# jhauret/vibravox

Hardware: AMD Instinct MI355X
Metric: EBEN train-step audio-seconds/sec (gen+disc) (higher is better)
Workload: dtype bf16

## Files before the change

### include/eben_hip.h

```cpp
#ifndef EBEN_HIP_H
#define EBEN_HIP_H

#include <stddef.h>
#include <stdint.h>

#if defined(EBEN_BUILDING)
#define EBEN_API __attribute__((visibility("default")))
#else
#define EBEN_API
#endif

#ifdef __cplusplus
extern "C" {
#endif

#define EBEN_OK 0
#define EBEN_EINVAL (-1)
#define EBEN_EWORKSPACE (-2)
#define EBEN_EUNSUPPORTED (-3)

#define EBEN_PAD_ZERO 0
#define EBEN_PAD_REFLECT 1

#define EBEN_MATH_F32 0
#define EBEN_MATH_BF16 1
#define EBEN_MATH_BF16X2 2
#define EBEN_MATH_BF16X3 3
#define EBEN_MATH_BF16X6 4
#define EBEN_LAYOUT_BL 0x100

typedef struct EbenConv1dDesc {
  int32_t batch;
  int32_t c_in, c_out;
  int32_t l_in, l_out;
  int32_t ksize, stride, dilation, groups;
  int32_t pad_l, pad_r;
  int32_t pad_mode;
  int32_t transposed;
  float in_slope;
  float out_slope;
  int32_t math;
} EbenConv1dDesc;

EBEN_API const char* eben_last_error(void);
#define EBEN_ABI_VERSION 5
EBEN_API int eben_version(void);
EBEN_API int eben_device_info(char* name, size_t name_bytes);

EBEN_API int eben_wn_scale(const float* g, const float* v, int rows, int cols, float* scale, float* norm, void* stream);
EBEN_API int eben_wn_bwd(const float* dw_slabs, int nslab, size_t slab_stride, int rows, int cols, int row_stride,
                const float* g, const float* v, const float* norm, float* dg, float* dv, float* dbias, void* stream);

typedef struct EbenWnScaleItem {
  const float* g; const float* v; float* scale; float* norm;
  int32_t rows, cols;
} EbenWnScaleItem;
typedef struct EbenWnBwdItem {
  const float* slabs;
  const float* g; const float* v; const float* norm;
  float* dg; float* dv; float* dbias;
  int64_t slab_stride;
  int32_t nslab, rows, cols, row_stride;
  int32_t col_perm_k, pad_;
} EbenWnBwdItem;
EBEN_API int eben_wn_scale_multi(const EbenWnScaleItem* items, int n, void* stream);
EBEN_API int eben_wn_bwd_multi(const EbenWnBwdItem* items, int n, void* stream);

EBEN_API size_t eben_conv1d_packed_floats(const EbenConv1dDesc* d, int which);
typedef struct EbenPackJob {
  EbenConv1dDesc desc;
  const float* v; const float* scale;
  float* wp_fwd; float* wp_bwd;
} EbenPackJob;
EBEN_API int eben_conv1d_pack_multi(const EbenPackJob* jobs, int n, void* stream);
EBEN_API int eben_conv1d_kernel_generation(const EbenConv1dDesc* d, int which);
#define EBEN_VARIANT_TAP3 1
#define EBEN_VARIANT_THIN_BL 2
#define EBEN_VARIANT_TAP4 3
EBEN_API int eben_conv1d_variant(const EbenConv1dDesc* d, int which, int mask_on_load, int* out, int n);
EBEN_API int eben_conv1d_pack(const EbenConv1dDesc* d, const float* v, const float* scale, float* wp_fwd, float* wp_bwd, void* stream);
EBEN_API int eben_conv1d_fwd(const EbenConv1dDesc* d, const float* x, const float* wp_fwd, const float* bias,
                    const float* residual, float* y, void* stream);
EBEN_API int eben_conv1d_fwd_res(const EbenConv1dDesc* d, const float* x, const float* wp_fwd, const float* bias,
                        const float* residual, float res_slope, float* y, void* stream);
EBEN_API size_t eben_conv1d_bwd_dx_workspace(const EbenConv1dDesc* d);
EBEN_API size_t eben_conv1d_bwd_dw_workspace(const EbenConv1dDesc* d, int* nslab, int* row_stride);
EBEN_API int eben_conv1d_bwd_dx(const EbenConv1dDesc* d, const float* dy, const float* y, const float* wp_bwd,
                       const float* x, float* dx, int accumulate, void* workspace, size_t ws_bytes, void* stream);
EBEN_API int eben_conv1d_bwd_dx_res(const EbenConv1dDesc* d, const float* dy, const float* y, const float* wp_bwd, const float* x,
                           const float* res_pre, const float* res_post, float* dx, void* workspace, size_t ws_bytes, void* stream);
EBEN_API int eben_conv1d_bwd_dx_ex(const EbenConv1dDesc* d, const float* g, const float* wp_bwd, const float* res, int res_rows,
                          const float* mask, float mask_slope, int seg, const int* seg_map, float* dx, void* stream);
EBEN_API int eben_conv1d_bwd_dx_fm(const EbenConv1dDesc* d, const float* g, const float* wp_bwd, const float* ref, int fm_rows,
                          const float* fm_sums, float fm_gs, const float* mask, float mask_slope, int seg, const int* seg_map,
                          float* dx, void* stream);
EBEN_API int eben_conv1d_bwd_dw(const EbenConv1dDesc* d, const float* dy, const float* y, const float* x, int has_bias,
                       float* slabs, size_t ws_bytes, void* stream);

EBEN_API int eben_bl_from_f32(const float* x, int batch, int channels, int length, void* hi, void* lo , void* stream);
EBEN_API int eben_bl_to_f32(const void* hi, const void* lo , int batch, int channels, int length, float* x, void* stream);
EBEN_API int eben_bl_conv1d_fwd(const EbenConv1dDesc* d, const void* x_hi, const void* x_lo, const float* wp_fwd, const float* bias,
                       void* y_hi, void* y_lo, void* stream);
EBEN_API int eben_bl_conv1d_bwd_dx(const EbenConv1dDesc* d, const void* g_hi, const float* wp_bwd, const void* act_hi, const void* act_lo,
                          float mask_slope, int seg, const int* seg_map, int fm_rows, int ref_row_offset, const float* fm_sums,
                          float fm_gs, void* dx_hi, void* dx_lo , void* stream);

EBEN_API int eben_bl_dx_pr_desc(const EbenConv1dDesc* d, EbenConv1dDesc* primed);
EBEN_API int eben_bl_dx_pr_weights(const EbenConv1dDesc* d, const float* v, const float* scale, float* w_primed, void* stream);
EBEN_API int eben_bl_conv1d_bwd_dx_pr(const EbenConv1dDesc* d, const void* g_hi, const float* wp_primed_fwd, const void* act_hi, const void* act_lo,
                                      float mask_slope, int seg, const int* seg_map, int fm_rows, int ref_row_offset, const float* fm_sums,
                                      float fm_gs, void* dx_hi, void* dx_lo, void* stream);
EBEN_API int eben_bl_conv1d_bwd_dx_c(const EbenConv1dDesc* d, const void* g_hi, const float* wp_bwd, const void* act_hi, const void* act_lo,
                            const void* fm_codes, float mask_slope, int seg, const int* seg_map, int fm_rows, int ref_row_offset,
                            const float* fm_sums, float fm_gs, void* dx_hi, void* dx_lo , void* stream);
EBEN_API int eben_bl_conv1d_bwd_dx_pr_c(const EbenConv1dDesc* d, const void* g_hi, const float* wp_primed_fwd, const void* act_hi, const void* act_lo,
                               const void* fm_codes, float mask_slope, int seg, const int* seg_map, int fm_rows, int ref_row_offset,
                               const float* fm_sums, float fm_gs, void* dx_hi, void* dx_lo , void* stream);
EBEN_API size_t eben_bl_conv1d_bwd_dw_workspace(const EbenConv1dDesc* d, int* nslab, int* row_stride, int* col_perm_k);
EBEN_API int eben_bl_conv1d_bwd_dw(const EbenConv1dDesc* d, const void* dy_hi, const void* x_hi, int has_bias, float* slabs, size_t ws_bytes,
                          void* stream);
EBEN_API int eben_bl_conv1d_bwd_dw_multi(const EbenConv1dDesc* const* descs, const void* const* dy_hi, const void* const* x_hi, int has_bias,
                                float* const* slabs, const size_t* ws_bytes, int n, void* stream);
EBEN_API int eben_bl_conv1d_bwd_dw_variant(const EbenConv1dDesc* d, int* out, int n);
typedef struct EbenBlHeadJob {
  const float* x;
  const float* v; const float* scale;
  const float* bias;
  void* y_hi; void* y_lo;
  int32_t c_in, c_out, l_in, l_out, ksize, dilation, pad, reflect_pad;
  float out_slope; int32_t pad_;
} EbenBlHeadJob;
EBEN_API int eben_bl_head_fwd(const EbenBlHeadJob* jobs, int njobs, int batch, void* stream);
EBEN_API int eben_bl_head_dx(const EbenBlHeadJob* jobs, int njobs, int rows, float* dx, void* stream);
EBEN_API size_t eben_bl_head_dw_workspace(const EbenBlHeadJob* job, int rows, int* nslab, int* row_stride);
EBEN_API int eben_bl_head_dw(const EbenBlHeadJob* job, int rows, float* slabs, size_t ws_bytes, void* stream);
EBEN_API int eben_bl_tail_fwd(const void* x_hi, const void* x_lo, int batch, int channels, int length, int ksize, int pad, const float* v,
                     const float* scale, const float* bias, float out_slope, float* y, void* stream);
EBEN_API int eben_bl_tail_dx(const float* seeds, int rows, int channels, int length, int ksize, int pad, const float* v, const float* scale,
                    const void* act_hi, const void* act_lo, float mask_slope, int seg, const int* seg_map, int fm_rows,
                    int ref_row_offset, const float* fm_sums, float fm_gs, void* g_hi, void* g_lo , void* stream);
EBEN_API size_t eben_bl_tail_dw_workspace(int rows, int channels, int l_out, int ksize, int nbranch, int* nslab, int* row_stride);
EBEN_API int eben_bl_tail_dw(const float* seeds, const void* x_hi, const void* x_lo, int rows, int nbranch, int channels, int length, int ksize, int pad,
                    float* slabs, size_t ws_bytes, void* stream);
EBEN_API size_t eben_bl_fm_sums_workspace(int npairs);
EBEN_API int eben_bl_fm_sums(const void* const* planes, const int64_t* units, int npairs, float* partial_ws, size_t ws_bytes, float* sums,
                    void* stream);
EBEN_API int eben_bl_fm_sums_codes(const void* const* planes, const int64_t* units, void* const* codes, int npairs, float* partial_ws,
                                   size_t ws_bytes, float* sums, void* stream);

EBEN_API size_t eben_ru_packed_floats(int channels);
EBEN_API int eben_ru_pack(int channels, const float* v_dil, const float* scale_dil, const float* v_pw, const float* scale_pw, float* wimg,
                 void* stream);
EBEN_API int eben_ru_fwd(int batch, int channels, int length, int dilation, const float* x, float in_slope, float out_slope,
                const float* wimg, float* y, float* h, float* u, void* stream);
EBEN_API int eben_ru_pack_bwd(int channels, const float* v_dil, const float* scale_dil, const float* v_pw, const float* scale_pw,
                     float* wimg_bwd, void* stream);
EBEN_API int eben_ru_bwd(int batch, int channels, int length, int dilation, const float* gy, const float* u, float out_slope,
                const float* x, float in_slope, const float* post, const float* wimg_bwd, float* gx, float* gh, void* stream);

EBEN_API size_t eben_ru_packed_floats_ex(int channels, int math);
EBEN_API int eben_ru_supported(int channels, int dilation, int math);
EBEN_API int eben_ru_pack_ex(int channels, int math, int which, const float* v_dil, const float* scale_dil, const float* v_pw,
                    const float* scale_pw, float* wimg, void* stream);
typedef struct EbenRuPackJob {
  int32_t channels, math, which, pad_;
  const float* v_dil; const float* scale_dil; const float* v_pw; const float* scale_pw; float* wimg;
} EbenRuPackJob;
EBEN_API int eben_ru_pack_multi(const EbenRuPackJob* jobs, int n, void* stream);
EBEN_API int eben_ru_fwd_ex(int math, int batch, int channels, int length, int dilation, const float* x, float in_slope, float out_slope,
                   const float* wimg, float* y, float* h, float* u, void* stream);
EBEN_API int eben_ru_bwd_ex(int math, int batch, int channels, int length, int dilation, const float* gy, const float* u, float out_slope,
                   const float* x, float in_slope, const float* post, const float* wimg_bwd, float* gx, float* gh, void* stream);

EBEN_API int eben_ru_dw_slabs(int batch, int channels, int length);
EBEN_API int eben_ru_dw(int math, int batch, int channels, int length, int dilation, const float* gy, const float* u, float out_slope,
               const float* h, const float* gh, const float* x, float in_slope, float* slabs_pw, float* slabs_dil, void* stream);

EBEN_API int eben_rubl_supported(int channels, int dilation);
EBEN_API int eben_rubl_fwd(int math, int batch, int channels, int length, int dilation, const float* x, float in_slope, float out_slope,
                           const float* wimg, float* y, void* xb, void* hb, void* umask, void* stream);
EBEN_API int eben_rubl_bwd(int batch, int channels, int length, int dilation, const float* gy, const void* umask, float out_slope, const float* x,
                           float in_slope, const float* post, const float* wimg_bwd, float* gx, void* gzb, void* ghb, void* stream);
EBEN_API int eben_rubl_dw_slabs(int batch, int channels, int length);
EBEN_API int eben_rubl_dw(int batch, int channels, int length, int dilation, const void* gzb, const void* hb, const void* ghb, const void* xb,
                          float* slabs_pw, float* slabs_dil, void* stream);

EBEN_API int eben_fir_decimate(const float* x, const float* w, float* y, int batch, int lx, int ly, int bands, int ntaps,
                      int stride, int off0, void* stream);
EBEN_API int eben_fir_interp_sum(const float* y, const float* w, float* x, int batch, int lx, int ly, int bands, int ntaps,
                        int stride, int off0, void* stream);

EBEN_API int eben_lrelu_fwd(const float* x, float* y, size_t n, float slope, void* stream);
EBEN_API int eben_lrelu_bwd(const float* dy, const float* x_or_y, float* dx, size_t n, float slope, void* stream);
EBEN_API size_t eben_gemm_packed_floats(int math, int groups, int m, int k);
EBEN_API int eben_gemm_pack(int math, int groups, int m, int k, const float* w, float* wp, void* stream);
EBEN_API int eben_gemm_fwd(int math, int groups, int m, int k, long long n, const float* x, const float* wp, float* y, void* stream);
EBEN_API int eben_space_to_depth(const float* x, const float* mask, float mask_slope, float* out, int rows, int L, int S, int off, int Lq,
                        int reflect, void* stream);
EBEN_API int eben_add(const float* a, const float* b, float* out, size_t n, void* stream);
EBEN_API int eben_axpby(const float* a, float alpha, const float* b, float beta, float* out, size_t n, void* stream);
EBEN_API int eben_tanh_lift_fwd(const float* x, const float* lift, float* out, int batch, int channels, int c_lift, int length, void* stream);
EBEN_API int eben_tanh_bwd(const float* dout, const float* out, float* dx, size_t n, void* stream);
EBEN_API int eben_reflect_pad_fwd(const float* x, float* y, int rows, int lx, int pad_l, int pad_r, void* stream);
EBEN_API int eben_reflect_pad_bwd(const float* dy, float* dx, int rows, int lx, int pad_l, int pad_r, void* stream);

EBEN_API int eben_fm_sums(const void* const* ptrs, const int64_t* numel, int npairs, float* partial_ws, size_t ws_bytes,
                 float* sums, void* stream);
EBEN_API size_t eben_fm_sums_workspace(int npairs);
EBEN_API int eben_fm_bwd(const void* const* ptrs, void* const* da_ptrs, const int64_t* numel, int npairs, const float* sums,
                const float* gout, float inv_count, void* stream);
EBEN_API int eben_hinge_fwd(const float* x, size_t n, float target, float* out, void* stream);
EBEN_API size_t eben_last_conv_norms_workspace(int batch);
EBEN_API int eben_last_conv_norms(const void* const* seeds, int n, const float* bands, const float* pre, int batch, int c_in, int c_out, int length,
                                  int ksize, int pad, float* workspace, size_t ws_bytes, float* norms, void* stream);
EBEN_API int eben_balance(const void* const* norms, const void* const* losses, int n, float* old, int init, int ema, float beta,
                 float one_minus_beta, float* lambdas, float* backprop, void* stream);
EBEN_API int eben_weighted_sum(const void* const* tensors, const float* weights, int n, size_t numel, float* out, void* stream);
EBEN_API int eben_disc_losses(const float* fm_sums, int npairs, float inv_count, const float* hinge, int nchains, float* out, void* stream);
EBEN_API int eben_stft_loss_total(const void* const* sums, const float* inv_counts, int n, int rows, float* out, void* stream);
EBEN_API int eben_hinge_fwd_multi(const void* const* xs, const int64_t* numel, const float* targets, int n, float* out, void* stream);
EBEN_API int eben_hinge_bwd(const float* x, size_t n, float target, const float* gout, float scale, float* dx, void* stream);
EBEN_API int eben_hinge_bwd_stacked(const float* enhanced_logits, const float* reference_logits, size_t per, const float* gout, float scale_adv,
                                    float scale_fake, float scale_real, float* seeds, void* stream);
EBEN_API int eben_stft_loss_sums(const float* spec_x, const float* spec_y, int rows, int bins, int bins_pad, int frames,
                        float eps, float* partial_ws, size_t ws_bytes, float* out, void* stream);
EBEN_API size_t eben_stft_loss_sums_workspace(int rows);
EBEN_API int eben_stft_loss_bwd(const float* spec_x, const float* spec_y, int rows, int bins, int bins_pad, int frames,
                       float eps, const float* sums, const float* gout, float scale, float* dspec_x, void* stream);

EBEN_API int eben_overlap_add(const float* frames_buf, float* x, int batch, int lx, int win, int frames, int hop, int pad,
                     int reflect, int accumulate, void* stream);

EBEN_API int eben_stft_frames(const float* sig, float* out, int rows, int t, int win, int hop, int pad, int frames, void* stream);
EBEN_API int eben_stft_frames_folded(const float* sig, float* out, int rows, int t, int win, int hop, int pad, int frames, int split,
                            void* stream);
EBEN_API int eben_split3(const float* in, float* out, int groups, int rows_per_group, long long cols, void* stream);
EBEN_API int eben_overlap_add_folded_tiled(int lx, int win, int hop, int pad);
EBEN_API int eben_overlap_add_folded(const float* frames_buf, float* x, int batch, int lx, int win, int frames, int hop, int pad,
                            int accumulate, long long row_stride, long long j_stride, void* stream);
EBEN_API int eben_stft_loss_sums_ex(const float* spec_x, const float* spec_y, int rows, int bins, int frames, long long row_stride,
                           long long bin_stride, long long im_off, float eps, float* partial_ws, size_t ws_bytes, float* out,
                           void* stream);
EBEN_API int eben_stft_loss_bwd_ex(const float* spec_x, const float* spec_y, int rows, int bins, int frames, long long row_stride,
                          long long bin_stride, long long im_off, float eps, const float* sums, const float* gout, float scale,
                          float* dspec_x, long long out_row_stride, long long out_bin_stride, long long out_im_off, void* stream);
EBEN_API int eben_overlap_add_ex(const float* frames_buf, float* x, int batch, int lx, int win, int frames, int hop, int pad,
                        int reflect, int accumulate, long long row_stride, long long j_stride, void* stream);

EBEN_API size_t eben_stft_terms_workspace(int rows);
EBEN_API int eben_stft_terms_fwd(const float* spec, int rows, int bins, int frames, float eps, int n_out, const int* fb_lo, const int* fb_off,
                                 const float* fb_w, int terms, int l2, float* mags, float* partial_ws, size_t ws_bytes, float* sums,
                                 void* stream);
EBEN_API int eben_stft_terms_bwd(const float* spec, int rows, int bins, int frames, float eps, int n_out, const int* bin_m, const float* bin_w,
                                 const float* mags, int terms, int l2, float w_sc, float w_log, float w_lin, const float* sums,
                                 const float* gout, float scale, float* dspec, void* stream);
EBEN_API int eben_stft_terms_total(const void* const* sums, const float* inv_counts, int n, int rows, int terms, float w_sc, float w_log,
                                   float w_lin, float* out, void* stream);

typedef struct EbenAdamTensor {
  float* param;
  const float* grad;
  float* exp_avg;
  float* exp_avg_sq;
  int64_t numel;
} EbenAdamTensor;
EBEN_API int eben_adam_step(const EbenAdamTensor* table, int ntensors, int64_t max_numel, float lr, float beta1, float beta2,
                   float eps, float weight_decay, int step, float grad_scale, void* stream);

typedef struct EbenCollateItem {
  const float* speech;
  const float* airborne;
  const float* noise;
  int64_t length;
  int64_t noise_start;
  int64_t shift;
} EbenCollateItem;
EBEN_API int eben_noisy_collate(const EbenCollateItem* items, int nitems, int samples, float* body_conducted, float* airborne, void* stream);

EBEN_API int eben_time_mask(float* x, long long rows, int t, int first, int count, void* stream);
EBEN_API int eben_phase_vocoder(const float* spec, float* out, int rows, int bins, int frames, int frames_out, double rate, float hop,
                       void* stream);
EBEN_API int eben_resample(const float* x, const float* kernels, float* out, int rows, int t_in, int t_out, int orig, int nw,
                  int width, void* stream);

EBEN_API int eben_multirate_down(const float* x, const float* tables, const int* widths, float* const* outs, int rows, int t_in,
                                 int scales, void* stream);
EBEN_API int eben_multirate_down_adjoint(const float* g0, const float* const* gs, const float* tables, const int* widths, float* dx,
                                         int rows, int t_in, int scales, void* stream);
EBEN_API int eben_resample_adjoint(const float* g, const float* kernels, float* dx, int rows, int t_in, int t_out, int orig, int nw,
                                   int width, int accumulate, void* stream);

EBEN_API int eben_l2norm(const float* x, size_t n, float* out, void* stream);

EBEN_API int eben_si_sdr(const float* preds, const float* target, int rows, int t, float* out, void* stream);
EBEN_API size_t eben_stoi_workspace(int rows, int t, int fs);
EBEN_API int eben_stoi(const float* clean, const float* processed, int rows, int t, int fs, const float* resample_table, int taps,
              void* workspace, size_t ws_bytes, float* out, void* stream);

#ifdef __cplusplus
}
#endif
#endif
```

### vibravox_amd/_lib.py

```python
from __future__ import annotations

import ctypes
import os
from ctypes import POINTER, c_char_p, c_float, c_int, c_int32, c_int64, c_size_t, c_void_p
from typing import Optional

import torch

_HERE = os.path.dirname(os.path.abspath(__file__))
LIB_PATH = os.path.join(_HERE, "lib", "libeben_hip.so")


class EbenError(RuntimeError):
    pass


class EbenConv1dDesc(ctypes.Structure):
    _fields_ = [
        ("batch", c_int32),
        ("c_in", c_int32),
        ("c_out", c_int32),
        ("l_in", c_int32),
        ("l_out", c_int32),
        ("ksize", c_int32),
        ("stride", c_int32),
        ("dilation", c_int32),
        ("groups", c_int32),
        ("pad_l", c_int32),
        ("pad_r", c_int32),
        ("pad_mode", c_int32),
        ("transposed", c_int32),
        ("in_slope", c_float),
        ("out_slope", c_float),
        ("math", c_int32),
    ]


class EbenPackJob(ctypes.Structure):
    _fields_ = [("desc", EbenConv1dDesc), ("v", c_void_p), ("scale", c_void_p), ("wp_fwd", c_void_p), ("wp_bwd", c_void_p)]


class EbenRuPackJob(ctypes.Structure):
    _fields_ = [("channels", c_int32), ("math", c_int32), ("which", c_int32), ("pad_", c_int32),
                ("v_dil", c_void_p), ("scale_dil", c_void_p), ("v_pw", c_void_p), ("scale_pw", c_void_p), ("wimg", c_void_p)]


class EbenWnScaleItem(ctypes.Structure):
    _fields_ = [("g", c_void_p), ("v", c_void_p), ("scale", c_void_p), ("norm", c_void_p), ("rows", c_int32), ("cols", c_int32)]


class EbenWnBwdItem(ctypes.Structure):
    _fields_ = [("slabs", c_void_p), ("g", c_void_p), ("v", c_void_p), ("norm", c_void_p), ("dg", c_void_p), ("dv", c_void_p),
                ("dbias", c_void_p), ("slab_stride", c_int64), ("nslab", c_int32), ("rows", c_int32), ("cols", c_int32),
                ("row_stride", c_int32), ("col_perm_k", c_int32), ("pad_", c_int32)]


class EbenBlHeadJob(ctypes.Structure):
    _fields_ = [("x", c_void_p), ("v", c_void_p), ("scale", c_void_p), ("bias", c_void_p), ("y_hi", c_void_p), ("y_lo", c_void_p),
                ("c_in", c_int32), ("c_out", c_int32), ("l_in", c_int32), ("l_out", c_int32), ("ksize", c_int32), ("dilation", c_int32),
                ("pad", c_int32), ("reflect_pad", c_int32), ("out_slope", c_float), ("pad_", c_int32)]


class EbenAdamTensor(ctypes.Structure):
    _fields_ = [
        ("param", c_void_p),
        ("grad", c_void_p),
        ("exp_avg", c_void_p),
        ("exp_avg_sq", c_void_p),
        ("numel", c_int64),
    ]


class EbenCollateItem(ctypes.Structure):
    _fields_ = [("speech", c_void_p), ("airborne", c_void_p), ("noise", c_void_p), ("length", c_int64), ("noise_start", c_int64),
                ("shift", c_int64)]


_P = c_void_p
_D = POINTER(EbenConv1dDesc)

SIGNATURES = {
    "eben_last_error": (c_char_p, []),
    "eben_version": (c_int, []),
    "eben_device_info": (c_int, [ctypes.c_char_p, c_size_t]),
    "eben_wn_scale": (c_int, [_P, _P, c_int, c_int, _P, _P, _P]),
    "eben_wn_bwd": (c_int, [_P, c_int, c_size_t, c_int, c_int, c_int, _P, _P, _P, _P, _P, _P, _P]),
    "eben_wn_scale_multi": (c_int, [POINTER(EbenWnScaleItem), c_int, _P]),
    "eben_wn_bwd_multi": (c_int, [POINTER(EbenWnBwdItem), c_int, _P]),
    "eben_conv1d_packed_floats": (c_size_t, [_D, c_int]),
    "eben_conv1d_kernel_generation": (c_int, [_D, c_int]),
    "eben_conv1d_variant": (c_int, [_D, c_int, c_int, POINTER(c_int), c_int]),
    "eben_conv1d_pack": (c_int, [_D, _P, _P, _P, _P, _P]),
    "eben_conv1d_pack_multi": (c_int, [POINTER(EbenPackJob), c_int, _P]),
    "eben_conv1d_fwd": (c_int, [_D, _P, _P, _P, _P, _P, _P]),
    "eben_conv1d_fwd_res": (c_int, [_D, _P, _P, _P, _P, c_float, _P, _P]),
    "eben_conv1d_bwd_dx_res": (c_int, [_D, _P, _P, _P, _P, _P, _P, _P, _P, c_size_t, _P]),
    "eben_conv1d_bwd_dx_workspace": (c_size_t, [_D]),
    "eben_conv1d_bwd_dw_workspace": (c_size_t, [_D, POINTER(c_int), POINTER(c_int)]),
    "eben_conv1d_bwd_dx": (c_int, [_D, _P, _P, _P, _P, _P, c_int, _P, c_size_t, _P]),
    "eben_conv1d_bwd_dx_ex": (c_int, [_D, _P, _P, _P, c_int, _P, c_float, c_int, POINTER(c_int), _P, _P]),
    "eben_conv1d_bwd_dx_fm": (c_int, [_D, _P, _P, _P, c_int, _P, c_float, _P, c_float, c_int, POINTER(c_int), _P, _P]),
    "eben_conv1d_bwd_dw": (c_int, [_D, _P, _P, _P, c_int, _P, c_size_t, _P]),
    "eben_bl_from_f32": (c_int, [_P, c_int, c_int, c_int, _P, _P, _P]),
    "eben_bl_to_f32": (c_int, [_P, _P, c_int, c_int, c_int, _P, _P]),
    "eben_bl_conv1d_fwd": (c_int, [_D, _P, _P, _P, _P, _P, _P, _P]),
    "eben_bl_conv1d_bwd_dx": (c_int, [_D, _P, _P, _P, _P, c_float, c_int, POINTER(c_int), c_int, c_int, _P, c_float, _P, _P, _P]),
    "eben_bl_dx_pr_desc": (c_int, [_D, _D]),
    "eben_bl_dx_pr_weights": (c_int, [_D, _P, _P, _P, _P]),
    "eben_bl_conv1d_bwd_dx_pr": (c_int, [_D, _P, _P, _P, _P, c_float, c_int, POINTER(c_int), c_int, c_int, _P, c_float, _P, _P, _P]),
    "eben_bl_conv1d_bwd_dx_c": (c_int, [_D, _P, _P, _P, _P, _P, c_float, c_int, POINTER(c_int), c_int, c_int, _P, c_float, _P, _P, _P]),
    "eben_bl_conv1d_bwd_dx_pr_c": (c_int, [_D, _P, _P, _P, _P, _P, c_float, c_int, POINTER(c_int), c_int, c_int, _P, c_float, _P, _P, _P]),
    "eben_bl_conv1d_bwd_dw_workspace": (c_size_t, [_D, POINTER(c_int), POINTER(c_int), POINTER(c_int)]),
    "eben_bl_conv1d_bwd_dw": (c_int, [_D, _P, _P, c_int, _P, c_size_t, _P]),
    "eben_bl_conv1d_bwd_dw_multi": (c_int, [POINTER(_D), POINTER(_P), POINTER(_P), c_int, POINTER(_P), POINTER(c_size_t), c_int, _P]),
    "eben_bl_conv1d_bwd_dw_variant": (c_int, [_D, POINTER(c_int), c_int]),
    "eben_bl_head_fwd": (c_int, [POINTER(EbenBlHeadJob), c_int, c_int, _P]),
    "eben_bl_head_dx": (c_int, [POINTER(EbenBlHeadJob), c_int, c_int, _P, _P]),
    "eben_bl_head_dw_workspace": (c_size_t, [POINTER(EbenBlHeadJob), c_int, POINTER(c_int), POINTER(c_int)]),
    "eben_bl_head_dw": (c_int, [POINTER(EbenBlHeadJob), c_int, _P, c_size_t, _P]),
    "eben_bl_tail_fwd": (c_int, [_P, _P, c_int, c_int, c_int, c_int, c_int, _P, _P, _P, c_float, _P, _P]),
    "eben_bl_tail_dx": (c_int, [_P, c_int, c_int, c_int, c_int, c_int, _P, _P, _P, _P, c_float, c_int, POINTER(c_int), c_int, c_int, _P, c_float,
                                _P, _P, _P]),
    "eben_bl_tail_dw_workspace": (c_size_t, [c_int, c_int, c_int, c_int, c_int, POINTER(c_int), POINTER(c_int)]),
    "eben_bl_tail_dw": (c_int, [_P, _P, _P, c_int, c_int, c_int, c_int, c_int, c_int, _P, c_size_t, _P]),
    "eben_bl_fm_sums_workspace": (c_size_t, [c_int]),
    "eben_bl_fm_sums": (c_int, [POINTER(c_void_p), POINTER(c_int64), c_int, _P, c_size_t, _P, _P]),
    "eben_bl_fm_sums_codes": (c_int, [POINTER(c_void_p), POINTER(c_int64), POINTER(c_void_p), c_int, _P, c_size_t, _P, _P]),
    "eben_ru_packed_floats": (c_size_t, [c_int]),
    "eben_ru_pack": (c_int, [c_int, _P, _P, _P, _P, _P, _P]),
    "eben_ru_fwd": (c_int, [c_int, c_int, c_int, c_int, _P, c_float, c_float, _P, _P, _P, _P, _P]),
    "eben_ru_pack_bwd": (c_int, [c_int, _P, _P, _P, _P, _P, _P]),
    "eben_ru_bwd": (c_int, [c_int, c_int, c_int, c_int, _P, _P, c_float, _P, c_float, _P, _P, _P, _P, _P]),
    "eben_ru_packed_floats_ex": (c_size_t, [c_int, c_int]),
    "eben_ru_supported": (c_int, [c_int, c_int, c_int]),
    "eben_ru_pack_ex": (c_int, [c_int, c_int, c_int, _P, _P, _P, _P, _P, _P]),
    "eben_ru_pack_multi": (c_int, [POINTER(EbenRuPackJob), c_int, _P]),
    "eben_ru_fwd_ex": (c_int, [c_int, c_int, c_int, c_int, c_int, _P, c_float, c_float, _P, _P, _P, _P, _P]),
    "eben_ru_bwd_ex": (c_int, [c_int, c_int, c_int, c_int, c_int, _P, _P, c_float, _P, c_float, _P, _P, _P, _P, _P]),
    "eben_ru_dw_slabs": (c_int, [c_int, c_int, c_int]),
    "eben_ru_dw": (c_int, [c_int, c_int, c_int, c_int, c_int, _P, _P, c_float, _P, _P, _P, c_float, _P, _P, _P]),
    "eben_rubl_supported": (c_int, [c_int, c_int]),
    "eben_rubl_fwd": (c_int, [c_int, c_int, c_int, c_int, c_int, _P, c_float, c_float, _P, _P, _P, _P, _P, _P]),
    "eben_rubl_bwd": (c_int, [c_int, c_int, c_int, c_int, _P, _P, c_float, _P, c_float, _P, _P, _P, _P, _P, _P]),
    "eben_rubl_dw_slabs": (c_int, [c_int, c_int, c_int]),
    "eben_rubl_dw": (c_int, [c_int, c_int, c_int, c_int, _P, _P, _P, _P, _P, _P, _P]),
    "eben_fir_decimate": (c_int, [_P, _P, _P, c_int, c_int, c_int, c_int, c_int, c_int, c_int, _P]),
    "eben_fir_interp_sum": (c_int, [_P, _P, _P, c_int, c_int, c_int, c_int, c_int, c_int, c_int, _P]),
    "eben_lrelu_fwd": (c_int, [_P, _P, c_size_t, c_float, _P]),
    "eben_lrelu_bwd": (c_int, [_P, _P, _P, c_size_t, c_float, _P]),
    "eben_space_to_depth": (c_int, [_P, _P, c_float, _P, c_int, c_int, c_int, c_int, c_int, c_int, _P]),
    "eben_gemm_packed_floats": (c_size_t, [c_int, c_int, c_int, c_int]),
    "eben_gemm_pack": (c_int, [c_int, c_int, c_int, c_int, _P, _P, _P]),
    "eben_gemm_fwd": (c_int, [c_int, c_int, c_int, c_int, ctypes.c_longlong, _P, _P, _P, _P]),
    "eben_add": (c_int, [_P, _P, _P, c_size_t, _P]),
    "eben_axpby": (c_int, [_P, c_float, _P, c_float, _P, c_size_t, _P]),
    "eben_tanh_lift_fwd": (c_int, [_P, _P, _P, c_int, c_int, c_int, c_int, _P]),
    "eben_tanh_bwd": (c_int, [_P, _P, _P, c_size_t, _P]),
    "eben_reflect_pad_fwd": (c_int, [_P, _P, c_int, c_int, c_int, c_int, _P]),
    "eben_reflect_pad_bwd": (c_int, [_P, _P, c_int, c_int, c_int, c_int, _P]),
    "eben_fm_sums": (c_int, [POINTER(c_void_p), POINTER(c_int64), c_int, _P, c_size_t, _P, _P]),
    "eben_fm_sums_workspace": (c_size_t, [c_int]),
    "eben_fm_bwd": (c_int, [POINTER(c_void_p), POINTER(c_void_p), POINTER(c_int64), c_int, _P, _P, c_float, _P]),
    "eben_hinge_fwd": (c_int, [_P, c_size_t, c_float, _P, _P]),
    "eben_hinge_fwd_multi": (c_int, [POINTER(c_void_p), POINTER(c_int64), POINTER(c_float), c_int, _P, _P]),
    "eben_disc_losses": (c_int, [_P, c_int, c_float, _P, c_int, _P, _P]),
    "eben_stft_loss_total": (c_int, [POINTER(c_void_p), POINTER(c_float), c_int, c_int, _P, _P]),
    "eben_last_conv_norms_workspace": (c_size_t, [c_int]),
    "eben_last_conv_norms": (c_int, [POINTER(c_void_p), c_int, _P, _P, c_int, c_int, c_int, c_int, c_int, c_int, _P, c_size_t, _P, _P]),
    "eben_balance": (c_int, [POINTER(c_void_p), POINTER(c_void_p), c_int, _P, c_int, c_int, c_float, c_float, _P, _P, _P]),
    "eben_weighted_sum": (c_int, [POINTER(c_void_p), _P, c_int, c_size_t, _P, _P]),
    "eben_hinge_bwd": (c_int, [_P, c_size_t, c_float, _P, c_float, _P, _P]),
    "eben_hinge_bwd_stacked": (c_int, [_P, _P, c_size_t, _P, c_float, c_float, c_float, _P, _P]),
    "eben_stft_loss_sums": (c_int, [_P, _P, c_int, c_int, c_int, c_int, c_float, _P, c_size_t, _P, _P]),
    "eben_stft_loss_sums_workspace": (c_size_t, [c_int]),
    "eben_stft_loss_bwd": (c_int, [_P, _P, c_int, c_int, c_int, c_int, c_float, _P, _P, c_float, _P, _P]),
    "eben_overlap_add": (c_int, [_P, _P, c_int, c_int, c_int, c_int, c_int, c_int, c_int, c_int, _P]),
    "eben_time_mask": (c_int, [_P, c_int64, c_int, c_int, c_int, _P]),
    "eben_phase_vocoder": (c_int, [_P, _P, c_int, c_int, c_int, c_int, ctypes.c_double, c_float, _P]),
    "eben_resample": (c_int, [_P, _P, _P, c_int, c_int, c_int, c_int, c_int, c_int, _P]),
    "eben_stft_frames": (c_int, [_P, _P, c_int, c_int, c_int, c_int, c_int, c_int, _P]),
    "eben_stft_frames_folded": (c_int, [_P, _P, c_int, c_int, c_int, c_int, c_int, c_int, c_int, _P]),
    "eben_split3": (c_int, [_P, _P, c_int, c_int, c_int64, _P]),
    "eben_overlap_add_folded_tiled": (c_int, [c_int, c_int, c_int, c_int]),
    "eben_overlap_add_folded": (c_int, [_P, _P, c_int, c_int, c_int, c_int, c_int, c_int, c_int, c_int64, c_int64, _P]),
    "eben_stft_loss_sums_ex": (c_int, [_P, _P, c_int, c_int, c_int, c_int64, c_int64, c_int64, c_float, _P, c_size_t, _P, _P]),
    "eben_stft_loss_bwd_ex": (c_int, [_P, _P, c_int, c_int, c_int, c_int64, c_int64, c_int64, c_float, _P, _P, c_float, _P, c_int64, c_int64,
                                      c_int64, _P]),
    "eben_overlap_add_ex": (c_int, [_P, _P, c_int, c_int, c_int, c_int, c_int, c_int, c_int, c_int, c_int64, c_int64, _P]),
    "eben_stft_terms_workspace": (c_size_t, [c_int]),
    "eben_stft_terms_fwd": (c_int, [_P, c_int, c_int, c_int, c_float, c_int, _P, _P, _P, c_int, c_int, _P, _P, c_size_t, _P, _P]),
    "eben_stft_terms_bwd": (c_int, [_P, c_int, c_int, c_int, c_float, c_int, _P, _P, _P, c_int, c_int, c_float, c_float, c_float, _P, _P,
                                    c_float, _P, _P]),
    "eben_stft_terms_total": (c_int, [POINTER(c_void_p), POINTER(c_float), c_int, c_int, c_int, c_float, c_float, c_float, _P, _P]),
    "eben_adam_step": (c_int, [POINTER(EbenAdamTensor), c_int, c_int64, c_float, c_float, c_float, c_float, c_float, c_int, c_float, _P]),
    "eben_noisy_collate": (c_int, [POINTER(EbenCollateItem), c_int, c_int, _P, _P, _P]),
    "eben_l2norm": (c_int, [_P, c_size_t, _P, _P]),
    "eben_si_sdr": (c_int, [_P, _P, c_int, c_int, _P, _P]),
    "eben_stoi_workspace": (c_size_t, [c_int, c_int, c_int]),
    "eben_stoi": (c_int, [_P, _P, c_int, c_int, c_int, _P, c_int, _P, c_size_t, _P, _P]),
    "eben_multirate_down": (c_int, [_P, _P, POINTER(c_int), POINTER(c_void_p), c_int, c_int, c_int, _P]),
    "eben_multirate_down_adjoint": (c_int, [_P, POINTER(c_void_p), _P, POINTER(c_int), _P, c_int, c_int, c_int, _P]),
    "eben_resample_adjoint": (c_int, [_P, _P, _P, c_int, c_int, c_int, c_int, c_int, c_int, c_int, _P]),
}

_lib: Optional[ctypes.CDLL] = None


ABI_VERSION = 5


def load(path: Optional[str] = None) -> ctypes.CDLL:
    global _lib
    if _lib is not None and path is None:
        return _lib
    p = path or os.environ.get("EBEN_HIP_LIB", LIB_PATH)
    if not os.path.exists(p):
        raise EbenError(
            f"{p} not found: build it with `python -c 'import __graft_entry__ as g; g.build()'` "
            f"or `vibravox_amd/csrc/build.sh` (there is no CPU fallback)."
        )
    lib = ctypes.CDLL(p)
    for name, (res, args) in SIGNATURES.items():
        fn = getattr(lib, name)
        fn.restype = res
        fn.argtypes = args
    have = lib.eben_version()
    if have != ABI_VERSION:
        raise EbenError(f"{p} reports ABI version {have}, this package binds version {ABI_VERSION} (include/eben_hip.h EBEN_ABI_VERSION): rebuild it "
                        f"with vibravox_amd/csrc/build.sh")
    if path is None:
        _lib = lib
    return lib


def check(rc: int, what: str = "") -> None:
    if rc != 0:
        msg = load().eben_last_error()
        raise EbenError(f"{what or 'libeben_hip'} failed (code {rc}): {msg.decode() if msg else '?'}")


def ptr(t: Optional[torch.Tensor]) -> Optional[int]:
    if t is None:
        return None
    if not t.is_cuda:
        raise EbenError(
            f"vibravox_amd ops run only on an MI355X HIP device (got a tensor on '{t.device}'); "
            "there is no CPU path -- the CPU oracle lives under oracle/ and is test-only."
        )
    if t.dtype is not torch.float32 or not t.is_contiguous():
        raise EbenError(f"expected a contiguous float32 tensor, got {t.dtype} contiguous={t.is_contiguous()}")
    return t.data_ptr()


def stream() -> int:
    return torch._C._cuda_getCurrentRawStream(torch._C._cuda_getDevice())
```

### vibravox_amd/csrc/common.h

```cpp
#pragma once
#include <hip/hip_runtime.h>

#include <atomic>

#include <cstdarg>
#include <cstdio>
#include <cstring>

#include "eben_hip.h"

namespace eben {

char* tls_error_buffer();
inline int fail(int code, const char* fmt, ...) {
  va_list ap;
  va_start(ap, fmt);
  vsnprintf(tls_error_buffer(), 512, fmt, ap);
  va_end(ap);
  return code;
}
inline int hip_fail(hipError_t e, const char* what) {
  snprintf(tls_error_buffer(), 512, "%s: %s", what, hipGetErrorString(e));
  return (int)e;
}

struct LdsAttrOnce { std::atomic<unsigned long long> devices{0ull}; };
inline int current_device_ordinal() {
  int dev = 0;
  if (hipGetDevice(&dev) != hipSuccess || dev < 0) dev = 0;
  return dev;
}
inline hipError_t lds_attr_once(LdsAttrOnce& once, const void* kern) {
  const unsigned long long bit = 1ull << (current_device_ordinal() & 63);
  if (once.devices.load(std::memory_order_acquire) & bit) return hipSuccess;
  const hipError_t e = hipFuncSetAttribute(kern, hipFuncAttributeMaxDynamicSharedMemorySize, 160 * 1024);
  if (e == hipSuccess) once.devices.fetch_or(bit, std::memory_order_release);
  return e;
}
inline int device_cus() {
  static std::atomic<int> cache[64];
  const int dev = current_device_ordinal() & 63;
  int n = cache[dev].load(std::memory_order_relaxed);
  if (n <= 0) {
    if (hipDeviceGetAttribute(&n, hipDeviceAttributeMultiprocessorCount, dev) != hipSuccess || n <= 0) n = 256;
    cache[dev].store(n, std::memory_order_relaxed);
  }
  return n;
}
#define EBEN_CHECK_LAUNCH(what)                         \
  do {                                                  \
    hipError_t e__ = hipGetLastError();                 \
    if (e__ != hipSuccess) return hip_fail(e__, what);  \
  } while (0)
#define EBEN_REQUIRE(cond, ...) \
  do {                          \
    if (!(cond)) return fail(EBEN_EINVAL, __VA_ARGS__); \
  } while (0)

inline hipStream_t as_stream(void* s) { return reinterpret_cast<hipStream_t>(s); }

inline int ceil_div(int a, int b) { return (a + b - 1) / b; }
inline int round_up(int a, int b) { return ceil_div(a, b) * b; }
inline size_t ceil_div_z(size_t a, size_t b) { return (a + b - 1) / b; }

__device__ __forceinline__ float lrelu(float v, float slope) { return v > 0.f ? v : v * slope; }
__device__ __forceinline__ float dlrelu(float ref, float slope) { return ref > 0.f ? 1.f : slope; }

__device__ __forceinline__ unsigned xcd_remap(unsigned bid, unsigned nblocks) {
  const unsigned nx = 8;
  const unsigned q = nblocks / nx, r = nblocks % nx;
  const unsigned xcd = bid % nx, idx = bid / nx;
  const unsigned start = xcd < r ? xcd * (q + 1) : r * (q + 1) + (xcd - r) * q;
  return start + idx;
}

__device__ __forceinline__ float wave_sum(float v) {
  float a = v, b = v;
  asm volatile("s_nop 1\n\tv_permlane32_swap_b32 %0, %1" : "+v"(a), "+v"(b));
  v = a + b;
  a = v; b = v;
  asm volatile("s_nop 1\n\tv_permlane16_swap_b32 %0, %1" : "+v"(a), "+v"(b));
  v = a + b;
#define EBEN_ROW_ROR_ADD(N)                                                                                                   \
  v += __builtin_bit_cast(float, __builtin_amdgcn_update_dpp(0, __builtin_bit_cast(int, v), 0x120 + (N), 0xf, 0xf, false));
  EBEN_ROW_ROR_ADD(8)
  EBEN_ROW_ROR_ADD(4)
  EBEN_ROW_ROR_ADD(2)
  EBEN_ROW_ROR_ADD(1)
#undef EBEN_ROW_ROR_ADD
  return v;
}
__device__ __forceinline__ float wave_sum_shfl(float v) {
#pragma unroll
  for (int o = 32; o > 0; o >>= 1) v += __shfl_xor(v, o, 64);
  return v;
}

__device__ __forceinline__ float block_sum_256(float v, float* red ) {
  v = wave_sum(v);
  const int lane = threadIdx.x & 63, w = threadIdx.x >> 6;
  __syncthreads();
  if (lane == 0) red[w] = v;
  __syncthreads();
  return red[0] + red[1] + red[2] + red[3];
}

typedef float f32x4 __attribute__((ext_vector_type(4)));

struct Canon {
  int B, Cin, Cout, Lin, Lout, k, s, d, g, pl, pr, reflect;
  int bf16;
  int xsplit_dir;
  int np;
  int bl;
};
int canon_from_desc(const EbenConv1dDesc* d, Canon* c);

struct TapIO {
  const float* x; const float* xmask; int in_mode; float in_slope;
  const float* wp; const float* bias; const float* res; float res_slope;
  const float* emask; float emask_slope; float out_slope; float* y; int accumulate;
  int res_rows; int em_seg; int em_map[4];
  const float* fm_sums; float fm_gs;
  const void* xh; const void* xl; void* yh; void* yl; const void* eh; const void* el; int bl_ref_off;
  const void* ec;
  int pr_S, pr_cbg, pr_Ly, pr_CBy, pr_order;
};

struct PhaseGeom { int J, off0, minoff, nt, oo, k0; };
__host__ __device__ inline PhaseGeom phase_geom(int mode, int ph, int J0, int off0_gs, int nt_gs, int dstep, int OS,
                                                int ps_pad, int ps_k, int ps_d, int ps_kstep, int Ly) {
  PhaseGeom q;
  q.J = J0; q.off0 = off0_gs; q.nt = nt_gs; q.oo = 0; q.k0 = 0;
  if (mode == 1) {
    int k0 = -1;
    for (int c = 0; c < ps_kstep; ++c) {
      int v = (ph + ps_pad - c * ps_d) % OS;
      if (v < 0) v += OS;
      if (v == 0) { k0 = c; break; }
    }
    if (k0 >= 0 && k0 < ps_k) {
      q.J = (ps_k - 1 - k0) / ps_kstep + 1;
      q.off0 = (ph + ps_pad - k0 * ps_d) / OS;
    } else {
      q.J = 0;
      q.off0 = 0;
    }
    q.k0 = k0;
    q.nt = ph < Ly ? (Ly - ph + OS - 1) / OS : 0;
    q.oo = ph;
  }
  q.minoff = (dstep >= 0 || q.J == 0) ? q.off0 : q.off0 + (q.J - 1) * dstep;
  return q;
}

int tap2_applicable(const Canon& c, int dir);
size_t tap2_packed_floats(const Canon& c, int dir);
int tap2_pack(const Canon& c, int dir, const float* w, const float* scale, float* wp, hipStream_t st);
int tap2_launch(const Canon& c, int dir, const TapIO& io, int reflect, hipStream_t st);

int tap3_applicable(const Canon& c, int dir);
int tap3_is_big(const Canon& c, int dir);
size_t tap3_packed_floats(const Canon& c, int dir);
int tap3_pack(const Canon& c, int dir, const float* w, const float* scale, float* wp, hipStream_t st);
int tap3_pack_multi(const Canon* cs, const int* dirs, const float* const* ws, const float* const* scales, float* const* wps, int n, hipStream_t st);
int tap3_launch(const Canon& c, int dir, const TapIO& io, int reflect, hipStream_t st);

int gc_applicable(const Canon& c, int dir);
size_t gc_packed_floats(const Canon& c, int dir);
int gc_pack(const Canon& c, int dir, const float* w, const float* scale, float* wp, hipStream_t st);
int gc_launch(const Canon& c, int dir, const TapIO& io, hipStream_t st);

int thin_applicable(const Canon& c, int dir);
size_t thin_packed_floats(const Canon& c, int dir);
int thin_pack(const Canon& c, int dir, const float* w, const float* scale, float* wp, hipStream_t st);
int thin_launch(const Canon& c, int dir, const TapIO& io, int reflect, hipStream_t st);
int tap_generation(const Canon& c, int dir);

struct Dw2Args {
  const float* a; const float* amask; int a_mode; float a_slope;
  const float* x; const float* xmask; int x_mode; float x_slope;
  float* ap;
  float* slabs;
  int B, G, Cg, Mg, Ca, Cx, La, Lx;
  int S, d, off0, J, Ng, has_bias, row_stride, reflect;
  int nsplit, nct, nchunks, nnt, nmt, XSTR, nch_max;
  long long slab_stride;
};

int dw2_applicable(const Canon& c);
size_t dw2_workspace(const Canon& c, int* nslab, int* row_stride);
int dw2_launch(const Canon& c, Dw2Args a, float* workspace, size_t ws_bytes, hipStream_t st);


int dw3_applicable(const Canon& c);
size_t dw3_workspace(const Canon& c, int* nslab, int* row_stride);
int dw3_launch(const Canon& c, const float* a, const float* amask, float a_slope, const float* x, float x_slope, int has_bias, float* workspace,
               size_t ws_bytes, hipStream_t st);

}
```

### vibravox_amd/csrc/gen_conv.hip

```cpp
#include "common.h"

#include <cstdlib>
#include <type_traits>

namespace eben {

typedef float f32x16 __attribute__((ext_vector_type(16)));
typedef float f32x2 __attribute__((ext_vector_type(2)));
typedef __bf16 bf16x8 __attribute__((ext_vector_type(8)));
typedef __bf16 bf16x2 __attribute__((ext_vector_type(2)));
typedef unsigned u32x4 __attribute__((ext_vector_type(4)));

struct GcArgs {
  const float* x; float* y; const u32x4* wp; const float* bias; const float* res;
  int B, CX, LX, CY, LY, NU, S;
  int rpc_shift, off0, KSP, nkg;
  int nrt, nrg, ncb, nh;
  int reflect;
  float in_slope, out_slope, res_slope;
  long long w_rt, w_half;
  unsigned xq, xr;
};

__device__ __forceinline__ unsigned gc_pack2(float a, float b) {
  const f32x2 v = {a, b};
  return __builtin_bit_cast(unsigned, __builtin_convertvector(v, bf16x2));
}

template <int NP>
__device__ __forceinline__ void gc_split(const float (&v)[8], u32x4 (&pc)[NP]) {
  float t[8];
#pragma unroll
  for (int e = 0; e < 8; ++e) t[e] = v[e];
#pragma unroll
  for (int q = 0; q < NP; ++q) {
    u32x4 o;
    o[0] = gc_pack2(t[0], t[1]); o[1] = gc_pack2(t[2], t[3]); o[2] = gc_pack2(t[4], t[5]); o[3] = gc_pack2(t[6], t[7]);
    pc[q] = o;
    if (q + 1 < NP) {
#pragma unroll
      for (int e = 0; e < 4; ++e) {
        t[2 * e] -= __builtin_bit_cast(float, o[e] << 16);
        t[2 * e + 1] -= __builtin_bit_cast(float, o[e] & 0xffff0000u);
      }
    }
  }
}

#ifndef EBEN_GC_DBG
#define EBEN_GC_DBG 0
#endif

template <int FORM, int RT, int CT, int NP>
__global__ __launch_bounds__(256, 2) void gc_kernel(const GcArgs P) {
  constexpr int KC = (RT == 2 && CT == 2) ? 2 : 8 / RT;
  constexpr int RTU = KC * NP * 64;
  constexpr int SLOT = RT * RTU;
  __shared__ __attribute__((aligned(16))) u32x4 Ws[2 * SLOT];

  const int tid = threadIdx.x;
  const int lane = tid & 63;
  const int wave = __builtin_amdgcn_readfirstlane(tid >> 6);
  const int n = lane & 31, hk = lane >> 5;

  unsigned id;
  {
    const unsigned bid = blockIdx.x, xcd = bid & 7u, idx = bid >> 3;
    id = (xcd < P.xr ? xcd * (P.xq + 1) : P.xr * (P.xq + 1) + (xcd - P.xr) * P.xq) + idx;
  }
  const int rg = __builtin_amdgcn_readfirstlane((int)(id % (unsigned)P.nrg)); id /= (unsigned)P.nrg;
  const int h = __builtin_amdgcn_readfirstlane((int)(id % (unsigned)P.nh)); id /= (unsigned)P.nh;
  const int cb = __builtin_amdgcn_readfirstlane((int)(id % (unsigned)P.ncb));
  const int b = __builtin_amdgcn_readfirstlane((int)(id / (unsigned)P.ncb));

  const float* xb = P.x + (long long)b * P.CX * P.LX;
  const u32x4* wsrc = P.wp + (long long)h * P.w_half + (long long)(rg * RT) * P.w_rt;
  const int nch = P.KSP / KC;

  constexpr int WPT = SLOT / 256;
  typedef const __attribute__((address_space(1))) char* gptr_t;
  static_assert(SLOT % 256 == 0, "a slot is a whole number of block-wide pieces");
  u32x4 wreg[WPT];
  auto load_w = [&](int ch) {
    if (EBEN_GC_DBG & 4) return;
#pragma unroll
    for (int p = 0; p < WPT; ++p) {
      if constexpr (RTU % 256 == 0) {
        const u32x4* base = wsrc + (long long)((p * 256) / RTU) * P.w_rt + (long long)ch * RTU + (p * 256) % RTU;
        unsigned long long a = reinterpret_cast<unsigned long long>(base);
        asm volatile("" : "+s"(a));
        wreg[p] = *reinterpret_cast<const __attribute__((address_space(1))) u32x4*>(reinterpret_cast<gptr_t>(a) + (unsigned)tid * 16u);
      } else {
        const int idx = p * 256 + tid;
        const unsigned off = (unsigned)((idx / RTU) * (int)P.w_rt + idx % RTU) * 16u;
        unsigned long long a = reinterpret_cast<unsigned long long>(wsrc + (long long)ch * RTU);
        asm volatile("" : "+s"(a));
        wreg[p] = *reinterpret_cast<const __attribute__((address_space(1))) u32x4*>(reinterpret_cast<gptr_t>(a) + off);
      }
    }
  };
  auto store_w = [&](int ch) {
    if (EBEN_GC_DBG & 4) return;
#pragma unroll
    for (int p = 0; p < WPT; ++p) Ws[(ch & 1) * SLOT + p * 256 + tid] = wreg[p];
  };

  const int u0w = (cb * 4 + wave) * (32 * CT);
  int ucol[CT];
  bool fast[CT];
#pragma unroll
  for (int ct = 0; ct < CT; ++ct) {
    const int u0 = u0w + ct * 32;
    const int u = u0 + n;
    ucol[ct] = u < P.NU ? u : P.NU - 1;
    bool f = u0 + 31 < P.NU;
    if (FORM == 0) f = f && P.S * u0 + P.off0 >= 0 && P.S * (u0 + 31) + P.off0 + (8 << P.rpc_shift) <= P.LX;
    if (FORM == 1) f = f && P.S * u0 + P.off0 >= 0 && P.S * (u0 + 31) + P.off0 + 4 <= P.LX;
    if (FORM == 2) f = f && (h == 0 ? u0 >= 1 : u0 + 32 < P.LX);
    fast[ct] = f;
  }
  const bool act_in = P.in_slope != 1.f;
  const int ks_real = P.nkg >> 1;
  const int RKS = FORM == 0 ? (P.rpc_shift ? 1 : 2) : FORM == 1 ? 4 : 8;
  int loff[CT];
#pragma unroll
  for (int ct = 0; ct < CT; ++ct) {
    const int u = ucol[ct];
    if (FORM == 0) loff[ct] = (P.rpc_shift ? 8 * hk : hk * P.LX) + P.S * u + P.off0;
    else if (FORM == 1) loff[ct] = 2 * hk * P.LX + P.S * u + P.off0;
    else loff[ct] = 4 * hk * P.LX + u - 1 + h;
  }
  auto row_ptr = [&](int ks) -> gptr_t {
    const int kc = ks < ks_real ? ks : ks_real - 1;
    const float* rp = xb + (long long)(kc * RKS) * P.LX;
    unsigned long long a = reinterpret_cast<unsigned long long>(rp);
    asm volatile("" : "+s"(a));
    return reinterpret_cast<gptr_t>(a);
  };
  struct Slow { int off[8]; unsigned ok; };
  auto slow_init = [&](int ct, Slow& sl) {
    const int u = ucol[ct];
    sl.ok = 0;
#pragma unroll
    for (int e = 0; e < 8; ++e) {
      int crow, pos;
      if (FORM == 0) { crow = P.rpc_shift ? 0 : hk; pos = P.S * u + P.off0 + (P.rpc_shift ? 8 * hk : 0) + e; }
      else if (FORM == 1) { crow = 2 * hk + (e >> 2); pos = P.S * u + P.off0 + (e & 3); }
      else { crow = 4 * hk + (e >> 1); pos = u - 1 + h + (e & 1); }
      if (P.reflect) {
        pos = pos < 0 ? -pos : pos;
        pos = pos >= P.LX ? 2 * (P.LX - 1) - pos : pos;
      }
      const bool ok = pos >= 0 && pos < P.LX;
      sl.off[e] = crow * P.LX + (ok ? pos : 0);
      sl.ok |= (unsigned)ok << e;
    }
  };
  auto gather = [&](auto fast_tag, int ks, int ct, const Slow& sl, float (&v)[8]) {
    constexpr bool FAST = decltype(fast_tag)::value;
    if (EBEN_GC_DBG & 2) {
#pragma unroll
      for (int e = 0; e < 8; ++e) v[e] = 1.f;
      return;
    }
    const gptr_t rp = row_ptr(ks);
    typedef float f4u __attribute__((ext_vector_type(4), aligned(4)));
    typedef float f2u __attribute__((ext_vector_type(2), aligned(4)));
    typedef const __attribute__((address_space(1))) f4u* g4_t;
    typedef const __attribute__((address_space(1))) f2u* g2_t;
    typedef const __attribute__((address_space(1))) float* g1_t;
    if constexpr (FAST) {
      const unsigned o = (unsigned)loff[ct] * 4u;
      if (FORM == 0) {
        const f4u a0 = *reinterpret_cast<g4_t>(rp + o), a1 = *reinterpret_cast<g4_t>(rp + 16 + o);
#pragma unroll
        for (int e = 0; e < 4; ++e) { v[e] = a0[e]; v[4 + e] = a1[e]; }
      } else if (FORM == 1) {
        const f4u a0 = *reinterpret_cast<g4_t>(rp + o), a1 = *reinterpret_cast<g4_t>(rp + (long long)P.LX * 4 + o);
#pragma unroll
        for (int e = 0; e < 4; ++e) { v[e] = a0[e]; v[4 + e] = a1[e]; }
      } else {
#pragma unroll
        for (int r = 0; r < 4; ++r) {
          const f2u a = *reinterpret_cast<g2_t>(rp + (long long)r * P.LX * 4 + o);
          v[2 * r] = a[0]; v[2 * r + 1] = a[1];
        }
      }
    } else {
#pragma unroll
      for (int e = 0; e < 8; ++e) v[e] = *reinterpret_cast<g1_t>(rp + (unsigned)sl.off[e] * 4u);
    }
  };
  auto slow_mask = [&](const Slow& sl, float (&v)[8]) {
#pragma unroll
    for (int e = 0; e < 8; ++e) v[e] = (sl.ok >> e) & 1u ? v[e] : 0.f;
  };
  auto activate = [&](auto act_tag, float (&v)[8]) {
    if constexpr (decltype(act_tag)::value) {
#pragma unroll
      for (int e = 0; e < 8; ++e) v[e] = lrelu(v[e], P.in_slope);
    }
  };

  f32x16 acc[CT][RT];
#pragma unroll
  for (int ct = 0; ct < CT; ++ct)
#pragma unroll
    for (int i = 0; i < RT; ++i)
#pragma unroll
      for (int r = 0; r < 16; ++r) acc[ct][i][r] = 0.f;

  auto run = [&](auto fast_tag, auto act_tag) {
    constexpr bool FAST = decltype(fast_tag)::value;
    float v[KC][CT][8];
    Slow sl[CT];
    if constexpr (!FAST) {
#pragma unroll
      for (int ct = 0; ct < CT; ++ct) slow_init(ct, sl[ct]);
    }
    auto pieces = [&](int j, u32x4 (&out)[CT][NP]) {
#pragma unroll
      for (int ct = 0; ct < CT; ++ct) {
        if constexpr (!FAST) slow_mask(sl[ct], v[j][ct]);
        activate(act_tag, v[j][ct]);
        gc_split<NP>(v[j][ct], out[ct]);
      }
    };
    load_w(0);
#pragma unroll
    for (int ksl = 0; ksl < KC; ++ksl)
#pragma unroll
      for (int ct = 0; ct < CT; ++ct) gather(fast_tag, ksl, ct, sl[ct], v[ksl][ct]);
    store_w(0);
    u32x4 bq[CT][NP];
    pieces(0, bq);
#pragma unroll
    for (int ct = 0; ct < CT; ++ct) gather(fast_tag, KC, ct, sl[ct], v[0][ct]);
    __syncthreads();
    auto chunk = [&](int ch, auto more_tag) {
      constexpr bool MORE = decltype(more_tag)::value;
      if constexpr (MORE) load_w(ch + 1);
      const u32x4* wb = Ws + (ch & 1) * SLOT + lane;
#pragma unroll
      for (int ksl = 0; ksl < KC; ++ksl) {
        constexpr int VPM = (44 * CT + 6 * RT * CT - 1) / (6 * RT * CT);
        const int nx = (ksl + 1) % KC;
        const bool has_next = MORE || ksl + 1 < KC;
        u32x4 aq[NP][RT];
#pragma unroll
        for (int q = 0; q < NP; ++q)
#pragma unroll
          for (int i = 0; i < RT; ++i) aq[q][i] = wb[i * RTU + (ksl * NP + q) * 64];
        u32x4 bqn[CT][NP];
        if (has_next) pieces(nx, bqn);
        if constexpr (MORE) {
#pragma unroll
          for (int ct = 0; ct < CT; ++ct) gather(fast_tag, ch * KC + ksl + 1 + KC, ct, sl[ct], v[nx][ct]);
        }
#pragma unroll
        for (int lvl = NP - 1; lvl >= 0; --lvl)
#pragma unroll
          for (int qw = 0; qw < NP; ++qw) {
            const int qx = lvl - qw;
            if (qx < 0 || qx >= NP) continue;
#pragma unroll
            for (int ct = 0; ct < CT; ++ct)
#pragma unroll
              for (int i = 0; i < RT; ++i) {
                if (EBEN_GC_DBG & 1) acc[ct][i][0] += __builtin_bit_cast(float, aq[qw][i][0] ^ bq[ct][qx][1]);
                else acc[ct][i] = __builtin_amdgcn_mfma_f32_32x32x16_bf16(__builtin_bit_cast(bf16x8, aq[qw][i]), __builtin_bit_cast(bf16x8, bq[ct][qx]), acc[ct][i], 0, 0, 0);
              }
          }
        if (has_next) {
#pragma unroll
          for (int ct = 0; ct < CT; ++ct)
#pragma unroll
            for (int q = 0; q < NP; ++q) bq[ct][q] = bqn[ct][q];
        }
        if (!(EBEN_GC_DBG & 16)) {
          __builtin_amdgcn_sched_group_barrier(0x100, NP * RT, 0);
          __builtin_amdgcn_sched_group_barrier(0x002, VPM, 0);
#pragma unroll
          for (int m = 0; m < 6 * RT * CT; ++m) {
            __builtin_amdgcn_sched_group_barrier(0x008, 1, 0);
            __builtin_amdgcn_sched_group_barrier(0x002, VPM, 0);
          }
        }
        __builtin_amdgcn_sched_barrier(0);
      }
      if constexpr (MORE) {
        store_w(ch + 1);
        __syncthreads();
      }
    };
    for (int ch = 0; ch + 1 < nch; ++ch) chunk(ch, std::true_type{});
    chunk(nch - 1, std::false_type{});
  };
  bool allfast = true;
#pragma unroll
  for (int ct = 0; ct < CT; ++ct) allfast = allfast && fast[ct];
  if (allfast) {
    if (act_in) run(std::true_type{}, std::true_type{});
    else run(std::true_type{}, std::false_type{});
  } else {
    if (act_in) run(std::false_type{}, std::true_type{});
    else run(std::false_type{}, std::false_type{});
  }

  if (EBEN_GC_DBG & 8) {
    float s = 0.f;
#pragma unroll
    for (int ct = 0; ct < CT; ++ct)
#pragma unroll
      for (int i = 0; i < RT; ++i)
#pragma unroll
        for (int r = 0; r < 16; ++r) s += acc[ct][i][r];
    if (s == 1.2345f) P.y[0] = s;
    return;
  }
  float* yb = P.y + (long long)b * P.CY * P.LY;
  const float* rb = P.res ? P.res + (long long)b * P.CY * P.LY : nullptr;
#pragma unroll
  for (int ct = 0; ct < CT; ++ct) {
    const int u = u0w + ct * 32 + n;
    if (u >= P.NU) continue;
#pragma unroll
    for (int i = 0; i < RT; ++i) {
      const int mt = (rg * RT + i) * 32;
#pragma unroll
      for (int r4 = 0; r4 < 4; ++r4) {
        const int m = mt + 8 * r4 + 4 * hk;
        float o[4];
#pragma unroll
        for (int r = 0; r < 4; ++r) o[r] = acc[ct][i][4 * r4 + r];
        if (FORM != 2) {
#pragma unroll
          for (int r = 0; r < 4; ++r) {
            const float t = o[r] + (P.bias ? P.bias[m + r] : 0.f);
            const long long yi = (long long)(m + r) * P.LY + u;
            yb[yi] = lrelu(t, P.out_slope) + (rb ? lrelu(rb[yi], P.res_slope) : 0.f);
          }
        } else if (P.S == 8) {
          const int co = m >> 2;
          const float bv = P.bias ? P.bias[co] : 0.f;
          f32x4 t;
#pragma unroll
          for (int r = 0; r < 4; ++r) t[r] = lrelu(o[r] + bv, P.out_slope);
          const long long yi = (long long)co * P.LY + 8 * u + 4 * h;
          if (rb) {
            const f32x4 rv = *reinterpret_cast<const f32x4*>(rb + yi);
#pragma unroll
            for (int r = 0; r < 4; ++r) t[r] += lrelu(rv[r], P.res_slope);
          }
          *reinterpret_cast<f32x4*>(yb + yi) = t;
        } else if (P.S == 4) {
#pragma unroll
          for (int c2 = 0; c2 < 2; ++c2) {
            const int co = (m >> 1) + c2;
            const float bv = P.bias ? P.bias[co] : 0.f;
            f32x2 t;
            t[0] = lrelu(o[2 * c2] + bv, P.out_slope); t[1] = lrelu(o[2 * c2 + 1] + bv, P.out_slope);
            const long long yi = (long long)co * P.LY + 4 * u + 2 * h;
            if (rb) { t[0] += lrelu(rb[yi], P.res_slope); t[1] += lrelu(rb[yi + 1], P.res_slope); }
            *reinterpret_cast<f32x2*>(yb + yi) = t;
          }
        } else {
#pragma unroll
          for (int r = 0; r < 4; ++r) {
            const float t = o[r] + (P.bias ? P.bias[m + r] : 0.f);
            const long long yi = (long long)(m + r) * P.LY + 2 * u + h;
            yb[yi] = lrelu(t, P.out_slope) + (rb ? lrelu(rb[yi], P.res_slope) : 0.f);
          }
        }
      }
    }
  }
}

struct GcPackArgs {
  const float* w; const float* scale; u32x4* wp;
  int form, CX, CY, k, S, pad, rpc_shift, nkg, KSP, nrt, nh, np;
  long long total;
};

__global__ __launch_bounds__(256) void gc_pack_kernel(const GcPackArgs P) {
  const long long i = (long long)blockIdx.x * 256 + threadIdx.x;
  if (i >= P.total) return;
  const int lane = (int)(i & 63);
  long long r = i >> 6;
  const int q = (int)(r % P.np); r /= P.np;
  const int ks = (int)(r % P.KSP); r /= P.KSP;
  const int rt = (int)(r % P.nrt);
  const int h = (int)(r / P.nrt);
  const int mr = rt * 32 + (lane & 31);
  const int kg = 2 * ks + (lane >> 5);
  float v[8];
#pragma unroll
  for (int e = 0; e < 8; ++e) {
    float t = 0.f;
    if (kg < P.nkg) {
      if (P.form != 2) {
        const int chan = P.form == 0 ? kg >> P.rpc_shift : 2 * kg + (e >> 2);
        const int j = P.form == 0 ? 8 * (kg & ((1 << P.rpc_shift) - 1)) + e : (e & 3);
        if (j < P.k && chan < P.CX && mr < P.CY)
          t = P.w[((long long)mr * P.CX + chan) * P.k + j] * (P.scale ? P.scale[mr] : 1.f);
      } else {
        const int chan = 4 * kg + (e >> 1);
        const int hs = P.S >> 1;
        const int co = mr / hs, p = h * hs + mr % hs;
        const int du = h == 0 ? 1 - (e & 1) : -(e & 1);
        const int j = P.S * du + p + P.pad;
        if (j >= 0 && j < P.k && chan < P.CX && co < P.CY)
          t = P.w[((long long)chan * P.CY + co) * P.k + j] * (P.scale ? P.scale[chan] : 1.f);
      }
    }
    v[e] = t;
  }
  u32x4 o;
  for (int qq = 0;; ++qq) {
    o[0] = gc_pack2(v[0], v[1]); o[1] = gc_pack2(v[2], v[3]); o[2] = gc_pack2(v[4], v[5]); o[3] = gc_pack2(v[6], v[7]);
    if (qq == q) break;
#pragma unroll
    for (int u = 0; u < 4; ++u) {
      v[2 * u] -= __builtin_bit_cast(float, o[u] << 16);
      v[2 * u + 1] -= __builtin_bit_cast(float, o[u] & 0xffff0000u);
    }
  }
  P.wp[i] = o;
}

static int gc_env(const char* name, int dflt) {
  const char* s = getenv(name);
  return s ? atoi(s) : dflt;
}

struct GcPlan {
  int ok, form, np;
  int CX, LX, CY, LY, NU, S, k, pad, rpc_shift, nkg, KSP, rows, nrt, nh;
  int RT, CT, nrg, ncb;
};

static void gc_plan(const Canon& c, int dir, GcPlan* p) {
  static const int enabled = gc_env("EBEN_GC", 1);
  memset(p, 0, sizeof(*p));
  if (!enabled || c.bl || (c.np != 3 && c.np != 2) || c.g != 1 || c.d != 1 || c.xsplit_dir >= 0) return;
  p->np = c.np;
  p->S = c.s; p->k = c.k;
  if (dir == 0) {
    const bool enc = c.k == 2 * c.s && (c.s == 2 || c.s == 4 || c.s == 8);
    const bool lat = c.s == 1 && c.k >= 5 && c.k <= 8;
    if (!(enc || lat) || c.Cin % 16 || c.Cout % 32) return;
    if (c.reflect && (c.pl > c.Lin - 1 || c.pr > c.Lin - 1)) return;
    p->form = c.k <= 4 ? 1 : 0;
    p->CX = c.Cin; p->LX = c.Lin; p->CY = c.Cout; p->LY = c.Lout; p->NU = c.Lout;
    p->pad = c.pl;
    p->rpc_shift = c.k > 8 ? 1 : 0;
    p->nkg = p->form == 0 ? c.Cin << p->rpc_shift : c.Cin / 2;
    p->rows = c.Cout; p->nh = 1;
  } else {
    if (c.s != 2 && c.s != 4 && c.s != 8) return;
    if (c.k != 2 * c.s || c.pl != c.s / 2 || c.Lin != c.s * c.Lout) return;
    if (c.Cout % 16 || (c.Cin * (c.s / 2)) % 32) return;
    p->form = 2;
    p->CX = c.Cout; p->LX = c.Lout; p->CY = c.Cin; p->LY = c.Lin; p->NU = c.Lout;
    p->pad = c.pl;
    p->nkg = c.Cout / 4;
    p->rows = c.Cin * (c.s / 2); p->nh = 2;
  }
  p->KSP = round_up(ceil_div(p->nkg, 2), 8);
  p->nrt = p->rows / 32;
  static const int env_rt = gc_env("EBEN_GC_RT", 0), env_ct = gc_env("EBEN_GC_CT", 0);
  double best = 1e30;
  const int prod = p->np == 3 ? 6 : p->np == 2 ? 3 : 1;
  for (int rt : {2, 1}) {
    if (p->nrt % rt) continue;
    for (int ct : {2, 1}) {
      if (rt == 1 && ct == 2) continue;
      if ((env_rt && rt != env_rt && p->nrt % env_rt == 0) || (env_ct && ct != env_ct)) continue;
      const int ncb = ceil_div(p->NU, 128 * ct);
      const long long waves = 4ll * p->nh * (p->nrt / rt) * c.B * ncb;
      const double per_wave = (double)p->KSP * ct * (32.0 * prod * rt > 240.0 ? 32.0 * prod * rt : 240.0) + 2500.0 + 600.0 * rt * ct;
      const double t = (double)((waves + 1023) / 1024) * per_wave * (ct == 2 ? 1.05 : 1.0);
      if (t < best * 0.98) { best = t; p->RT = rt; p->CT = ct; }
    }
  }
  if (!p->RT) return;
  p->nrg = p->nrt / p->RT;
  p->ncb = ceil_div(p->NU, 128 * p->CT);
  p->ok = 1;
}

int gc_applicable(const Canon& c, int dir) {
  GcPlan p;
  gc_plan(c, dir, &p);
  return p.ok;
}

size_t gc_packed_floats(const Canon& c, int dir) {
  GcPlan p;
  gc_plan(c, dir, &p);
  return p.ok ? (size_t)p.nh * p.nrt * p.KSP * p.np * 64 * 4 : 0;
}

int gc_pack(const Canon& c, int dir, const float* w, const float* scale, float* wp, hipStream_t st) {
  GcPlan p;
  gc_plan(c, dir, &p);
  if (!p.ok) return fail(EBEN_EUNSUPPORTED, "gc_pack on a layer the direct-operand conv does not cover");
  GcPackArgs a{};
  a.w = w; a.scale = scale; a.wp = reinterpret_cast<u32x4*>(wp);
  a.form = p.form; a.CX = p.CX; a.CY = p.CY; a.k = p.k; a.S = p.S; a.pad = p.pad; a.rpc_shift = p.rpc_shift; a.nkg = p.nkg; a.KSP = p.KSP;
  a.nrt = p.nrt; a.nh = p.nh; a.np = p.np;
  a.total = (long long)p.nh * p.nrt * p.KSP * p.np * 64;
  hipLaunchKernelGGL(gc_pack_kernel, dim3((unsigned)((a.total + 255) / 256)), dim3(256), 0, st, a);
  EBEN_CHECK_LAUNCH("gc_pack_kernel");
  return EBEN_OK;
}

template <int FORM, int NP>
static void gc_launch_shape(const GcPlan& p, const GcArgs& a, unsigned grid, hipStream_t st) {
  if (p.RT == 2 && p.CT == 2) hipLaunchKernelGGL((gc_kernel<FORM, 2, 2, NP>), dim3(grid), dim3(256), 0, st, a);
  else if (p.RT == 2) hipLaunchKernelGGL((gc_kernel<FORM, 2, 1, NP>), dim3(grid), dim3(256), 0, st, a);
  else hipLaunchKernelGGL((gc_kernel<FORM, 1, 1, NP>), dim3(grid), dim3(256), 0, st, a);
}

int gc_launch(const Canon& c, int dir, const TapIO& io, hipStream_t st) {
  GcPlan p;
  gc_plan(c, dir, &p);
  if (!p.ok) return fail(EBEN_EUNSUPPORTED, "gc_launch on a layer the direct-operand conv does not cover");
  if (io.emask || io.in_mode || io.accumulate || io.res_rows || io.fm_sums) return fail(EBEN_EUNSUPPORTED, "direct-operand conv: forward launches only");
  GcArgs a{};
  a.x = io.x; a.y = io.y; a.wp = reinterpret_cast<const u32x4*>(io.wp); a.bias = io.bias; a.res = io.res;
  a.B = c.B; a.CX = p.CX; a.LX = p.LX; a.CY = p.CY; a.LY = p.LY; a.NU = p.NU; a.S = p.S;
  a.rpc_shift = p.rpc_shift; a.off0 = -p.pad; a.KSP = p.KSP; a.nkg = p.nkg;
  a.nrt = p.nrt; a.nrg = p.nrg; a.ncb = p.ncb; a.nh = p.nh;
  a.reflect = dir == 0 ? c.reflect : 0;
  a.in_slope = io.in_slope; a.out_slope = io.out_slope; a.res_slope = io.res_slope;
  a.w_rt = (long long)p.KSP * p.np * 64; a.w_half = a.w_rt * p.nrt;
  const unsigned grid = (unsigned)(p.nh * p.nrg * c.B * p.ncb);
  a.xq = grid / 8; a.xr = grid % 8;
  if (p.np == 2) {
    if (p.form == 0) gc_launch_shape<0, 2>(p, a, grid, st);
    else if (p.form == 1) gc_launch_shape<1, 2>(p, a, grid, st);
    else gc_launch_shape<2, 2>(p, a, grid, st);
  } else if (p.form == 0) gc_launch_shape<0, 3>(p, a, grid, st);
  else if (p.form == 1) gc_launch_shape<1, 3>(p, a, grid, st);
  else gc_launch_shape<2, 3>(p, a, grid, st);
  EBEN_CHECK_LAUNCH("gc_kernel");
  return EBEN_OK;
}

}
```

### vibravox_amd/csrc/ru_split.hip

```cpp
#include "common.h"

#include <cstdlib>

namespace eben {

#ifndef EBEN_RU_DBG
#define EBEN_RU_DBG 0
#endif

typedef float f32x16 __attribute__((ext_vector_type(16)));
typedef float f32x2 __attribute__((ext_vector_type(2)));
typedef __bf16 bf16x8 __attribute__((ext_vector_type(8)));
typedef __bf16 bf16x2 __attribute__((ext_vector_type(2)));
typedef unsigned u32x4 __attribute__((ext_vector_type(4)));

__device__ __forceinline__ unsigned rs_pack_bf16(float a, float b) {
  const f32x2 v = {a, b};
  return __builtin_bit_cast(unsigned, __builtin_convertvector(v, bf16x2));
}

template <int NP>
__device__ __forceinline__ void rs_split8(const float (&v)[8], u32x4 (&p)[NP]) {
  float r[8];
#pragma unroll
  for (int e = 0; e < 8; ++e) r[e] = v[e];
#pragma unroll
  for (int q = 0; q < NP; ++q) {
    u32x4 o;
#pragma unroll
    for (int e = 0; e < 4; ++e) o[e] = rs_pack_bf16(r[2 * e], r[2 * e + 1]);
    p[q] = o;
    if (q + 1 < NP) {
#pragma unroll
      for (int e = 0; e < 4; ++e) {
        r[2 * e] -= __builtin_bit_cast(float, o[e] << 16);
        r[2 * e + 1] -= __builtin_bit_cast(float, o[e] & 0xffff0000u);
      }
    }
  }
}

template <int NP, int CT>
__device__ __forceinline__ void rs_mma(const u32x4 (&a)[NP][CT], const u32x4 (&b)[NP], f32x16 (&acc)[CT]) {
#pragma unroll
  for (int lvl = NP - 1; lvl >= 0; --lvl)
#pragma unroll
    for (int q = 0; q <= lvl; ++q)
#pragma unroll
      for (int i = 0; i < CT; ++i) {
        if (EBEN_RU_DBG & 8) acc[i][0] += __builtin_bit_cast(float, a[q][i][0] ^ b[lvl - q][i & 3]);
        else acc[i] = __builtin_amdgcn_mfma_f32_32x32x16_bf16(__builtin_bit_cast(bf16x8, a[q][i]), __builtin_bit_cast(bf16x8, b[lvl - q]), acc[i], 0, 0, 0);
      }
}

constexpr int RS_DMAX = 9;

struct Ru3Args {
  const float* x; const u32x4* wimg; float* y; float* h; float* u;
  u32x4* xb; u32x4* hb; unsigned char* um;
  int B, L, d, ntt, vec;
  float in_slope, out_slope;
};

template <int CT, int NW, int NP, int KSC, bool BL = false>
__global__ __launch_bounds__(NW * 64, (NW == 4 && CT < 4) ? 2 : 1) void ru3_fwd_kernel(const Ru3Args P) {
  constexpr int NT = NW * 64, BN = NW * 32, C = 32 * CT;
  constexpr int XS = BN + 2 * RS_DMAX + 6;
  constexpr int KB = C / 16;
  constexpr int KS1 = 3 * KB, KS2 = KB;
  constexpr int U = NP * CT * 64;
  constexpr int WCHU = KSC * U;
  constexpr int NCH1 = KS1 / KSC, NCH2 = KS2 / KSC, NCHK = NCH1 + NCH2;
  static_assert(KS1 % KSC == 0 && KS2 % KSC == 0, "a chunk never straddles the two stages");
  static_assert(XS % 4 == 0 && WCHU % 64 == 0, "tile rows are float4-aligned, chunks are whole wave pieces");

  extern __shared__ __attribute__((aligned(16))) u32x4 rs_smem[];
  u32x4* Ws = rs_smem;
  float* Xs = reinterpret_cast<float*>(rs_smem + 2 * WCHU);

  const int tid = threadIdx.x, lane = tid & 63;
  const int wn = __builtin_amdgcn_readfirstlane(tid >> 6);
  const int tt = __builtin_amdgcn_readfirstlane(blockIdx.x % P.ntt);
  const int b = __builtin_amdgcn_readfirstlane(blockIdx.x / P.ntt);
  const int t0 = tt * BN, d = P.d, L = P.L;
  const int q0 = t0 - d;
  const int qa = q0 >= 0 ? (q0 & ~3) : q0;
  const int xshift = q0 - qa;
  const float* xrow = P.x + (long long)b * C * L;

  auto issue_w = [&](int ch) {
    const u32x4* src = P.wimg + (long long)ch * WCHU;
    u32x4* dst = Ws + (ch & 1) * WCHU;
#pragma unroll
    for (int p = 0; p * NT < WCHU; ++p) {
      const int idx = p * NT + tid;
      if (idx < WCHU)
        __builtin_amdgcn_global_load_lds((const __attribute__((address_space(1))) void*)(src + idx),
                                         (__attribute__((address_space(3))) void*)(dst + (idx & ~63)), 16, 0, 0);
    }
  };
  issue_w(0);

  const bool interior = P.vec && q0 >= 0 && qa + XS <= L;
  if (interior) {
    constexpr int x4 = XS >> 2, tot4 = C * x4;
    for (int base = 0; base < ((EBEN_RU_DBG & 4) ? 4 * NT : tot4); base += 4 * NT) {
      f32x4 v[4];
      int sl[4];
#pragma unroll
      for (int e = 0; e < 4; ++e) {
        const int i = base + tid + e * NT;
        const int c = i / x4;
        const int k4 = i - c * x4;
        const bool ok = i < tot4;
        v[e] = *reinterpret_cast<const f32x4*>(xrow + (ok ? (long long)c * L + qa + 4 * k4 : 0));
        sl[e] = ok ? c * XS + 4 * k4 : -1;
      }
#pragma unroll
      for (int e = 0; e < 4; ++e) {
        f32x4 t;
#pragma unroll
        for (int k = 0; k < 4; ++k) t[k] = lrelu(v[e][k], P.in_slope);
        if (sl[e] >= 0) *reinterpret_cast<f32x4*>(Xs + sl[e]) = t;
      }
    }
  } else {
    constexpr int tot = C * XS;
    for (int base = 0; base < tot; base += 8 * NT) {
      float v[8];
      int sl[8], ok[8];
#pragma unroll
      for (int e = 0; e < 8; ++e) {
        const int i = base + tid + e * NT;
        const int c = i / XS;
        const int p = i - c * XS;
        int q = qa + p;
        q = q < 0 ? -q : q;
        q = q >= L ? 2 * (L - 1) - q : q;
        ok[e] = (int)(i < tot) & (int)(q >= 0) & (int)(q < L);
        v[e] = xrow[ok[e] ? (long long)c * L + q : 0];
        sl[e] = i < tot ? c * XS + p : -1;
      }
#pragma unroll
      for (int e = 0; e < 8; ++e)
        if (sl[e] >= 0) Xs[sl[e]] = ok[e] ? lrelu(v[e], P.in_slope) : 0.f;
    }
  }
  __syncthreads();

  f32x16 acc1[CT], acc2[CT];
#pragma unroll
  for (int i = 0; i < CT; ++i)
#pragma unroll
    for (int r = 0; r < 16; ++r) { acc1[i][r] = 0.f; acc2[i][r] = 0.f; }

  const int col = wn * 32 + (lane & 31);
  const float* xb = Xs + (lane >> 5) * 8 * XS + xshift + col;
  const int t = t0 + col;
  const bool live = t < L;
  const long long ubase = (long long)b * (C / 8) * L + t;

#pragma nounroll
  for (int ch = 0; ch < NCH1; ++ch) {
    issue_w(ch + 1);
    const u32x4* wb = Ws + (ch & 1) * WCHU + lane;
#pragma unroll
    for (int kk = 0; kk < KSC; ++kk) {
      const int ks = ch * KSC + kk;
      const int j = ks / KB, cb = ks - j * KB;
      const float* xk = xb + cb * 16 * XS + j * d;
      float v[8];
#pragma unroll
      for (int e = 0; e < 8; ++e) v[e] = xk[e * XS];
      u32x4 a[NP][CT], bq[NP];
#pragma unroll
      for (int q = 0; q < NP; ++q)
#pragma unroll
        for (int i = 0; i < CT; ++i) a[q][i] = wb[kk * U + (q * CT + i) * 64];
      rs_split8<NP>(v, bq);
      if constexpr (BL) {
        if (j == 1 && live && (!(EBEN_RU_DBG & 2) || bq[0][0] == 0x12345u)) P.xb[ubase + (long long)(2 * cb + (lane >> 5)) * L] = bq[0];
      }
      rs_mma<NP, CT>(a, bq, acc1);
    }
    __syncthreads();
  }

  const long long lbase = (long long)b * C * L + t;
  if constexpr (BL) {
    if (live) {
      uint2* __restrict__ hu = reinterpret_cast<uint2*>(P.hb + ubase) + (lane >> 5);
#pragma unroll
      for (int i = 0; i < CT; ++i)
#pragma unroll
        for (int q = 0; q < 4; ++q) {
          uint2 v;
          v.x = rs_pack_bf16(acc1[i][4 * q], acc1[i][4 * q + 1]);
          v.y = rs_pack_bf16(acc1[i][4 * q + 2], acc1[i][4 * q + 3]);
          if (!(EBEN_RU_DBG & 2) || v.x == 0x12345u) hu[(long long)(4 * i + q) * L * 2] = v;
        }
    }
  } else if (P.h != nullptr && live) {
    float* __restrict__ hb = P.h + lbase;
#pragma unroll
    for (int i = 0; i < CT; ++i)
#pragma unroll
      for (int r = 0; r < 16; ++r) {
        const unsigned m = i * 32 + (r & 3) + 8 * (r >> 2) + 4 * (lane >> 5);
        hb[m * (unsigned)L] = acc1[i][r];
      }
  }

#pragma unroll
  for (int c2 = 0; c2 < NCH2; ++c2) {
    const int ch = NCH1 + c2;
    if (ch + 1 < NCHK) issue_w(ch + 1);
    const u32x4* wb = Ws + (ch & 1) * WCHU + lane;
#pragma unroll
    for (int kk = 0; kk < KSC; ++kk) {
      const int ks2 = c2 * KSC + kk;
      const int isrc = ks2 >> 1, s = ks2 & 1;
      float v[8];
#pragma unroll
      for (int e = 0; e < 8; ++e) v[e] = acc1[isrc][8 * s + e];
      u32x4 a[NP][CT], bq[NP];
#pragma unroll
      for (int q = 0; q < NP; ++q)
#pragma unroll
        for (int i = 0; i < CT; ++i) a[q][i] = wb[kk * U + (q * CT + i) * 64];
      rs_split8<NP>(v, bq);
      rs_mma<NP, CT>(a, bq, acc2);
    }
    if (c2 + 1 < NCH2) __syncthreads();
  }

  if constexpr (BL) {
    unsigned nlo = 0, nhi = 0;
#pragma unroll
    for (int i = 0; i < CT; ++i)
#pragma unroll
      for (int q = 0; q < 4; ++q) {
        unsigned nib = 0;
#pragma unroll
        for (int e = 0; e < 4; ++e) nib |= (acc2[i][4 * q + e] > 0.f ? 1u : 0u) << e;
        if (i < 2) nlo |= nib << (4 * (4 * i + q));
        else nhi |= nib << (4 * (4 * (i - 2) + q));
      }
    const unsigned olo = __shfl_xor(nlo, 32, 64), ohi = CT > 2 ? __shfl_xor(nhi, 32, 64) : 0u;
    const int hf = lane >> 5;
    const unsigned l0 = hf ? olo : nlo, l1 = hf ? nlo : olo, h0 = hf ? ohi : nhi, h1 = hf ? nhi : ohi;
    if (live) {
      unsigned char* __restrict__ ub8 = P.um + ubase;
#pragma unroll
      for (int g = 0; g < 4 * CT; g += 2) {
        const int gg = g + hf;
        const unsigned w0 = gg < 8 ? l0 : h0, w1 = gg < 8 ? l1 : h1;
        const int sh = 4 * (gg & 7);
        ub8[(long long)gg * L] = (unsigned char)(((w0 >> sh) & 15u) | (((w1 >> sh) & 15u) << 4));
      }
    }
  }

  if (!live) return;
  const float* xc = Xs + xshift + d + col;
  float* __restrict__ yb = P.y + lbase;
  float* __restrict__ ub = P.u + lbase;
  const bool keep_u = !BL && P.u != nullptr;
#pragma unroll
  for (int i = 0; i < CT; ++i)
#pragma unroll
    for (int r = 0; r < 16; ++r) {
      const unsigned m = i * 32 + (r & 3) + 8 * (r >> 2) + 4 * (lane >> 5);
      const unsigned off = m * (unsigned)L;
      const float uu = lrelu(acc2[i][r], P.out_slope);
      if (keep_u) ub[off] = uu;
      if (!(EBEN_RU_DBG & 1) || uu == 12345.f) yb[off] = xc[m * XS] + uu;
    }
}

__device__ __forceinline__ void ru3_pack_fwd_body(const float* __restrict__ vd, const float* __restrict__ sd, const float* __restrict__ vp,
                                                  const float* __restrict__ sp, u32x4* __restrict__ img, int CT, int NP, unsigned bid, unsigned nblk) {
  const int C = 32 * CT, KB = C / 16;
  const int total = 4 * KB * CT * 64;
  for (int t = bid * 256 + threadIdx.x; t < total; t += nblk * 256) {
    const int lane = t & 63;
    const int i = (t >> 6) % CT;
    const int ks = t / (64 * CT);
    const int m = 32 * i + (lane & 31), kh = lane >> 5;
    float w[8];
    if (ks < 3 * KB) {
      const int j = ks / KB, cb = ks - j * KB;
#pragma unroll
      for (int e = 0; e < 8; ++e) w[e] = vd[((long long)m * C + cb * 16 + 8 * kh + e) * 3 + j] * (sd ? sd[m] : 1.f);
    } else {
      const int ks2 = ks - 3 * KB, isrc = ks2 >> 1, s = ks2 & 1;
#pragma unroll
      for (int e = 0; e < 8; ++e) {
        const int chn = 32 * isrc + (e & 3) + 8 * (2 * s + (e >> 2)) + 4 * kh;
        w[e] = vp[(long long)m * C + chn] * (sp ? sp[m] : 1.f);
      }
    }
    float r[8];
#pragma unroll
    for (int e = 0; e < 8; ++e) r[e] = w[e];
    for (int q = 0; q < NP; ++q) {
      u32x4 o;
#pragma unroll
      for (int e = 0; e < 4; ++e) o[e] = rs_pack_bf16(r[2 * e], r[2 * e + 1]);
      img[((long long)(ks * NP + q) * CT + i) * 64 + lane] = o;
#pragma unroll
      for (int e = 0; e < 4; ++e) {
        r[2 * e] -= __builtin_bit_cast(float, o[e] << 16);
        r[2 * e + 1] -= __builtin_bit_cast(float, o[e] & 0xffff0000u);
      }
    }
  }
}

struct Ru3BwdArgs {
  const float* gy; const float* u; const u32x4* wimg; const float* xmask; const float* post; float* gx; float* gh;
  int B, L, d, ntt, BO, vec;
  float out_slope, in_slope;
};

template <int CT, int NW, int NP, int G>
__global__ __launch_bounds__(NW * 64, (NW == 4 && CT < 4) ? 2 : 1) void ru3_bwd_kernel(const Ru3BwdArgs P) {
  constexpr int NT = NW * 64, WN = NW * 32, C = 32 * CT;
  constexpr int GS = WN + 4;
  constexpr int U = NP * CT * 64;
  constexpr int EU = 2 * U;
  constexpr int WCHU = G * EU;
  static_assert(CT % G == 0, "an entry group never straddles a stage");

  extern __shared__ __attribute__((aligned(16))) u32x4 rs_smem[];
  u32x4* Ws = rs_smem;
  float* Gs = reinterpret_cast<float*>(rs_smem + 2 * WCHU);

  const int tid = threadIdx.x, lane = tid & 63;
  const int wn = __builtin_amdgcn_readfirstlane(tid >> 6);
  const int tt = __builtin_amdgcn_readfirstlane(blockIdx.x % P.ntt);
  const int b = __builtin_amdgcn_readfirstlane(blockIdx.x / P.ntt);
  const int d = P.d, L = P.L, BO = P.BO;
  const int t0 = tt * BO;
  const int w0 = t0 - d;
  const int wa = w0 >= 0 ? (w0 & ~3) : w0;
  const int xshift = w0 - wa;
  const long long rowbase = (long long)b * C * L;

  const bool fold_l = t0 <= d && L > 1;
  const bool fold_r = t0 + BO > L - 1 - d && t0 <= L - 2;
  const int NS = 4 * CT + (fold_l ? CT : 0) + (fold_r ? CT : 0);
  const int NSG = NS / G;
  auto img_entry = [&](int sq) -> int {
    if (sq < 4 * CT) return sq;
    sq -= 4 * CT;
    if (fold_l) { if (sq < CT) return CT + 2 * CT + sq; sq -= CT; }
    return CT + sq;
  };
  auto issue_w = [&](int sg) {
    u32x4* dst = Ws + (sg & 1) * WCHU;
#pragma unroll
    for (int g = 0; g < G; ++g) {
      const u32x4* src = P.wimg + (long long)img_entry(sg * G + g) * EU;
#pragma unroll
      for (int p = 0; p * NT < EU; ++p) {
        const int idx = p * NT + tid;
        if (idx < EU)
          __builtin_amdgcn_global_load_lds((const __attribute__((address_space(1))) void*)(src + idx),
                                           (__attribute__((address_space(3))) void*)(dst + g * EU + (idx & ~63)), 16, 0, 0);
      }
    }
  };
  issue_w(0);

  const float* gyr = P.gy + rowbase;
  const float* ur = P.u + rowbase;
  const bool interior = P.vec && w0 >= 0 && wa + GS <= L;
  if (interior) {
    constexpr int x4 = GS >> 2, tot4 = C * x4;
    for (int base = 0; base < tot4; base += 4 * NT) {
      f32x4 v[4], m[4];
      int sl[4];
#pragma unroll
      for (int e = 0; e < 4; ++e) {
        const int i = base + tid + e * NT;
        const int c = i / x4;
        const int k4 = i - c * x4;
        const bool ok = i < tot4;
        const long long o = ok ? (long long)c * L + wa + 4 * k4 : 0;
        v[e] = *reinterpret_cast<const f32x4*>(gyr + o);
        m[e] = *reinterpret_cast<const f32x4*>(ur + o);
        sl[e] = ok ? c * GS + 4 * k4 : -1;
      }
#pragma unroll
      for (int e = 0; e < 4; ++e) {
        f32x4 t;
#pragma unroll
        for (int k = 0; k < 4; ++k) t[k] = v[e][k] * dlrelu(m[e][k], P.out_slope);
        if (sl[e] >= 0) *reinterpret_cast<f32x4*>(Gs + sl[e]) = t;
      }
    }
  } else {
    constexpr int tot = C * GS;
    for (int base = 0; base < tot; base += 8 * NT) {
      float v[8], m[8];
      int sl[8], ok[8];
#pragma unroll
      for (int e = 0; e < 8; ++e) {
        const int i = base + tid + e * NT;
        const int c = i / GS;
        const int p = i - c * GS;
        const int q = wa + p;
        ok[e] = (int)(i < tot) & (int)(q >= 0) & (int)(q < L);
        const long long o = ok[e] ? (long long)c * L + q : 0;
        v[e] = gyr[o];
        m[e] = ur[o];
        sl[e] = i < tot ? c * GS + p : -1;
      }
#pragma unroll
      for (int e = 0; e < 8; ++e)
        if (sl[e] >= 0) Gs[sl[e]] = ok[e] ? v[e] * dlrelu(m[e], P.out_slope) : 0.f;
    }
  }
  __syncthreads();

  f32x16 acc1[CT], acc2[CT];
#pragma unroll
  for (int i = 0; i < CT; ++i)
#pragma unroll
    for (int r = 0; r < 16; ++r) { acc1[i][r] = 0.f; acc2[i][r] = 0.f; }

  const int wc = wn * 32 + (lane & 31);
  const float* gbA = Gs + (lane >> 5) * 8 * GS + xshift + wc;
  const float* gbB = Gs + (lane >> 5) * 8 * GS + xshift + (wc < BO ? wc : BO - 1);

  auto entry = [&](const u32x4* wslot, int cb, const float* gb, int off, f32x16 (&acc)[CT], bool sel) {
#pragma unroll
    for (int kk = 0; kk < 2; ++kk) {
      const float* xk = gb + (cb * 32 + kk * 16) * GS + off;
      float v[8];
#pragma unroll
      for (int e = 0; e < 8; ++e) v[e] = sel ? xk[e * GS] : 0.f;
      u32x4 a[NP][CT], bq[NP];
#pragma unroll
      for (int q = 0; q < NP; ++q)
#pragma unroll
        for (int i = 0; i < CT; ++i) a[q][i] = wslot[kk * U + (q * CT + i) * 64];
      rs_split8<NP>(v, bq);
      rs_mma<NP, CT>(a, bq, acc);
    }
  };

  int sg = 0;
#pragma nounroll
  for (int c0 = 0; c0 < CT; c0 += G, ++sg) {
    issue_w(sg + 1);
    const u32x4* wb = Ws + (sg & 1) * WCHU + lane;
#pragma unroll
    for (int g = 0; g < G; ++g) entry(wb + g * EU, c0 + g, gbA, 0, acc1, true);
    if (c0 + G >= CT) {
      const int q = w0 + wc;
      const bool own = wc >= d && wc < d + BO && q < L;
      float* __restrict__ ghb = P.gh + rowbase + (own ? q : 0);
#pragma unroll
      for (int i = 0; i < CT; ++i)
#pragma unroll
        for (int r = 0; r < 16; ++r) {
          const int m = i * 32 + (r & 3) + 8 * (r >> 2) + 4 * (lane >> 5);
          const float v = (q >= 0 && q < L) ? acc1[i][r] : 0.f;
          Gs[m * GS + xshift + wc] = v;
          if (own) ghb[(unsigned)m * (unsigned)L] = v;
        }
    }
    __syncthreads();
  }
#pragma nounroll
  for (int jj = 0; jj < 3; ++jj)
#pragma nounroll
    for (int c0 = 0; c0 < CT; c0 += G, ++sg) {
      if (sg + 1 < NSG) issue_w(sg + 1);
      const u32x4* wb = Ws + (sg & 1) * WCHU + lane;
#pragma unroll
      for (int g = 0; g < G; ++g) entry(wb + g * EU, c0 + g, gbB, jj * d, acc2, true);
      __syncthreads();
    }
  const int t = t0 + wc;
  if (fold_l) {
    const bool in = t >= 1 && t <= d && wc < BO;
    const int off = in ? (d - t - w0) - wc : 0;
#pragma nounroll
    for (int c0 = 0; c0 < CT; c0 += G, ++sg) {
      if (sg + 1 < NSG) issue_w(sg + 1);
      const u32x4* wb = Ws + (sg & 1) * WCHU + lane;
#pragma unroll
      for (int g = 0; g < G; ++g) entry(wb + g * EU, c0 + g, gbA, off, acc2, in);
      __syncthreads();
    }
  }
  if (fold_r) {
    const bool in = t >= L - 1 - d && t <= L - 2 && wc < BO;
    const int off = in ? (2 * (L - 1) - t - d - w0) - wc : 0;
#pragma nounroll
    for (int c0 = 0; c0 < CT; c0 += G, ++sg) {
      if (sg + 1 < NSG) issue_w(sg + 1);
      const u32x4* wb = Ws + (sg & 1) * WCHU + lane;
#pragma unroll
      for (int g = 0; g < G; ++g) entry(wb + g * EU, c0 + g, gbA, off, acc2, in);
      __syncthreads();
    }
  }

  if (wc >= BO || t >= L) return;
  const float* __restrict__ gyb = P.gy + rowbase + t;
  const float* __restrict__ xmb = P.xmask + rowbase + t;
  const float* __restrict__ pob = P.post + rowbase + t;
  float* __restrict__ gxb = P.gx + rowbase + t;
#pragma unroll
  for (int i = 0; i < CT; ++i) {
    float gv[16], xv[16], pv[16];
    unsigned off[16];
#pragma unroll
    for (int r = 0; r < 16; ++r) {
      off[r] = (unsigned)(i * 32 + (r & 3) + 8 * (r >> 2) + 4 * (lane >> 5)) * (unsigned)L;
      gv[r] = gyb[off[r]];
    }
    if (P.xmask) {
#pragma unroll
      for (int r = 0; r < 16; ++r) xv[r] = xmb[off[r]];
    }
    if (P.post) {
#pragma unroll
      for (int r = 0; r < 16; ++r) pv[r] = pob[off[r]];
    }
#pragma unroll
    for (int r = 0; r < 16; ++r) {
      float v = acc2[i][r] + gv[r];
      if (P.xmask) v *= dlrelu(xv[r], P.in_slope);
      if (P.post) v += pv[r];
      gxb[off[r]] = v;
    }
  }
}

__device__ __forceinline__ void ru3_pack_bwd_body(const float* __restrict__ vd, const float* __restrict__ sd, const float* __restrict__ vp,
                                                  const float* __restrict__ sp, u32x4* __restrict__ img, int CT, int NP, unsigned bid, unsigned nblk) {
  const int C = 32 * CT;
  const int total = 4 * CT * 2 * CT * 64;
  for (int t = bid * 256 + threadIdx.x; t < total; t += nblk * 256) {
    const int lane = t & 63;
    const int i = (t >> 6) % CT;
    const int kk = (t / (64 * CT)) & 1;
    const int en = t / (128 * CT);
    const int row = 32 * i + (lane & 31), kh = lane >> 5;
    float w[8];
#pragma unroll
    for (int e = 0; e < 8; ++e) {
      if (en < CT) {
        const int m = en * 32 + kk * 16 + 8 * kh + e;
        w[e] = vp[(long long)m * C + row] * (sp ? sp[m] : 1.f);
      } else {
        const int jj = (en - CT) / CT, cb = (en - CT) - jj * CT;
        const int m = cb * 32 + kk * 16 + 8 * kh + e;
        w[e] = vd[((long long)m * C + row) * 3 + (2 - jj)] * (sd ? sd[m] : 1.f);
      }
    }
    float r[8];
#pragma unroll
    for (int e = 0; e < 8; ++e) r[e] = w[e];
    for (int q = 0; q < NP; ++q) {
      u32x4 o;
#pragma unroll
      for (int e = 0; e < 4; ++e) o[e] = rs_pack_bf16(r[2 * e], r[2 * e + 1]);
      img[(((long long)(en * 2 + kk) * NP + q) * CT + i) * 64 + lane] = o;
#pragma unroll
      for (int e = 0; e < 4; ++e) {
        r[2 * e] -= __builtin_bit_cast(float, o[e] << 16);
        r[2 * e + 1] -= __builtin_bit_cast(float, o[e] & 0xffff0000u);
      }
    }
  }
}

__global__ __launch_bounds__(256) void ru3_pack_fwd_kernel(const float* vd, const float* sd, const float* vp, const float* sp, u32x4* img, int CT, int NP) {
  ru3_pack_fwd_body(vd, sd, vp, sp, img, CT, NP, blockIdx.x, gridDim.x);
}
__global__ __launch_bounds__(256) void ru3_pack_bwd_kernel(const float* vd, const float* sd, const float* vp, const float* sp, u32x4* img, int CT, int NP) {
  ru3_pack_bwd_body(vd, sd, vp, sp, img, CT, NP, blockIdx.x, gridDim.x);
}

constexpr int RU_PACK_MULTI = 48;
struct RuPackTable {
  int n;
  unsigned short first[RU_PACK_MULTI + 1];
  struct { const float* vd; const float* sd; const float* vp; const float* sp; u32x4* img; short CT, NP, which, pad; } job[RU_PACK_MULTI];
};
__global__ __launch_bounds__(256) void ru3_pack_multi_kernel(const RuPackTable T) {
  int j = 0;
#pragma unroll 1
  while (j + 1 < T.n && blockIdx.x >= T.first[j + 1]) ++j;
  const unsigned bid = blockIdx.x - T.first[j], nblk = T.first[j + 1] - T.first[j];
  if (T.job[j].which == 0) ru3_pack_fwd_body(T.job[j].vd, T.job[j].sd, T.job[j].vp, T.job[j].sp, T.job[j].img, T.job[j].CT, T.job[j].NP, bid, nblk);
  else ru3_pack_bwd_body(T.job[j].vd, T.job[j].sd, T.job[j].vp, T.job[j].sp, T.job[j].img, T.job[j].CT, T.job[j].NP, bid, nblk);
}

static int rs_pieces(int math) {
  switch (math) {
    case EBEN_MATH_BF16: return 1;
    case EBEN_MATH_BF16X3: return 2;
    case EBEN_MATH_BF16X6: return 3;
    default: return 0;
  }
}

template <int CT, int NW, int NP, int KSC, bool BL = false>
static int launch_ru3_fwd(const Ru3Args& a, hipStream_t st) {
  static LdsAttrOnce attr_once;
  auto kern = ru3_fwd_kernel<CT, NW, NP, KSC, BL>;
  constexpr int XS = NW * 32 + 2 * RS_DMAX + 6;
  const size_t lds = (size_t)2 * KSC * NP * CT * 64 * 16 + sizeof(float) * 32 * CT * XS;
  {
    const hipError_t e = lds_attr_once(attr_once, reinterpret_cast<const void*>(kern));
    if (e != hipSuccess) return hip_fail(e, "hipFuncSetAttribute(ru3_fwd)");
  }
  hipLaunchKernelGGL(kern, dim3(a.B * a.ntt), dim3(NW * 64), lds, st, a);
  EBEN_CHECK_LAUNCH("ru3_fwd_kernel");
  return EBEN_OK;
}

template <int CT, int NW, int NP, int G>
static int launch_ru3_bwd(const Ru3BwdArgs& a, hipStream_t st) {
  static LdsAttrOnce attr_once;
  auto kern = ru3_bwd_kernel<CT, NW, NP, G>;
  constexpr int GS = NW * 32 + 4;
  const size_t lds = (size_t)2 * G * 2 * NP * CT * 64 * 16 + sizeof(float) * 32 * CT * GS;
  {
    const hipError_t e = lds_attr_once(attr_once, reinterpret_cast<const void*>(kern));
    if (e != hipSuccess) return hip_fail(e, "hipFuncSetAttribute(ru3_bwd)");
  }
  hipLaunchKernelGGL(kern, dim3(a.B * a.ntt), dim3(NW * 64), lds, st, a);
  EBEN_CHECK_LAUNCH("ru3_bwd_kernel");
  return EBEN_OK;
}

static int rs_waves(int channels) {
  static const int w128 = getenv("EBEN_RU3_W128") ? atoi(getenv("EBEN_RU3_W128")) : 4;
  return channels == 128 ? (w128 == 4 ? 4 : 2) : 4;
}

int ru3_supported(int channels, int dilation, int math) {
  return (channels == 32 || channels == 64 || channels == 128) && dilation >= 1 && dilation <= RS_DMAX && rs_pieces(math) > 0;
}

size_t ru3_packed_floats(int channels, int math) {
  const int np = rs_pieces(math);
  if (np == 0 || (channels != 32 && channels != 64 && channels != 128)) return 0;
  return (size_t)2 * np * channels * channels;
}

int ru3_pack(int channels, int math, int which, const float* vd, const float* sd, const float* vp, const float* sp, float* wimg, hipStream_t st) {
  const int np = rs_pieces(math), CT = channels / 32;
  const int total = which == 0 ? 8 * CT * CT * 64 : 4 * CT * 2 * CT * 64;
  if (which == 0)
    hipLaunchKernelGGL(ru3_pack_fwd_kernel, dim3(ceil_div(total, 256)), dim3(256), 0, st, vd, sd, vp, sp, reinterpret_cast<u32x4*>(wimg), CT, np);
  else
    hipLaunchKernelGGL(ru3_pack_bwd_kernel, dim3(ceil_div(total, 256)), dim3(256), 0, st, vd, sd, vp, sp, reinterpret_cast<u32x4*>(wimg), CT, np);
  EBEN_CHECK_LAUNCH("ru3_pack_kernel");
  return EBEN_OK;
}

int ru3_fwd(int math, int batch, int channels, int length, int dilation, const float* x, float in_slope, float out_slope, const float* wimg,
            float* y, float* h, float* u, hipStream_t st) {
  Ru3Args a;
  a.x = x; a.wimg = reinterpret_cast<const u32x4*>(wimg); a.y = y; a.h = h; a.u = u;
  a.xb = nullptr; a.hb = nullptr; a.um = nullptr;
  a.B = batch; a.L = length; a.d = dilation;
  const int bn = rs_waves(channels) * 32;
  a.ntt = ceil_div(length, bn);
  a.in_slope = in_slope; a.out_slope = out_slope;
  a.vec = ((reinterpret_cast<uintptr_t>(x) & 15) == 0 && (length & 3) == 0) ? 1 : 0;
  if ((long long)a.B * a.ntt > 0x7fffffffLL) return fail(EBEN_EINVAL, "ResidualUnit grid too large");
  const int np = rs_pieces(math);
#define EBEN_RU3_FWD(NPV)                                                 \
  switch (channels / 32) {                                                \
    case 1: return launch_ru3_fwd<1, 4, NPV, 2>(a, st);                   \
    case 2: return launch_ru3_fwd<2, 4, NPV, 2>(a, st);                   \
    default: return rs_waves(128) == 4 ? launch_ru3_fwd<4, 4, NPV, 2>(a, st) : launch_ru3_fwd<4, 2, NPV, 1>(a, st); \
  }
  switch (np) {
    case 1: EBEN_RU3_FWD(1)
    case 2: EBEN_RU3_FWD(2)
    default: EBEN_RU3_FWD(3)
  }
#undef EBEN_RU3_FWD
}

int ru3_fwd_bl(int math, int batch, int channels, int length, int dilation, const float* x, float in_slope, float out_slope, const float* wimg,
               float* y, void* xb, void* hb, void* um, hipStream_t st) {
  Ru3Args a;
  a.x = x; a.wimg = reinterpret_cast<const u32x4*>(wimg); a.y = y; a.h = nullptr; a.u = nullptr;
  a.xb = static_cast<u32x4*>(xb); a.hb = static_cast<u32x4*>(hb); a.um = static_cast<unsigned char*>(um);
  a.B = batch; a.L = length; a.d = dilation;
  a.ntt = ceil_div(length, 128);
  a.in_slope = in_slope; a.out_slope = out_slope;
  a.vec = ((reinterpret_cast<uintptr_t>(x) & 15) == 0 && (length & 3) == 0) ? 1 : 0;
  if ((long long)a.B * a.ntt > 0x7fffffffLL) return fail(EBEN_EINVAL, "ResidualUnit grid too large");
  const int np = rs_pieces(math);
  if (np != 3 && np != 2) return fail(EBEN_EUNSUPPORTED, "eben_rubl_fwd: the forward computes in EBEN_MATH_BF16X6 or EBEN_MATH_BF16X3 (got %d)", math);
  if (np == 2) {
    switch (channels / 32) {
      case 1: return launch_ru3_fwd<1, 4, 2, 2, true>(a, st);
      case 2: return launch_ru3_fwd<2, 4, 2, 2, true>(a, st);
      default: return launch_ru3_fwd<4, 4, 2, 2, true>(a, st);
    }
  }
  switch (channels / 32) {
    case 1: return launch_ru3_fwd<1, 4, 3, 2, true>(a, st);
    case 2: return launch_ru3_fwd<2, 4, 3, 2, true>(a, st);
    default: return launch_ru3_fwd<4, 4, 3, 2, true>(a, st);
  }
}

int ru3_bwd(int math, int batch, int channels, int length, int dilation, const float* gy, const float* u, float out_slope, const float* x,
            float in_slope, const float* post, const float* wimg, float* gx, float* gh, hipStream_t st) {
  Ru3BwdArgs a;
  a.gy = gy; a.u = u; a.wimg = reinterpret_cast<const u32x4*>(wimg); a.xmask = in_slope != 1.f ? x : nullptr; a.post = post; a.gx = gx; a.gh = gh;
  a.B = batch; a.L = length; a.d = dilation;
  const int nw = rs_waves(channels);
  const int wn = nw * 32;
  a.BO = wn - 2 * dilation; a.ntt = ceil_div(length, a.BO);
  a.out_slope = out_slope; a.in_slope = in_slope;
  a.vec = (((reinterpret_cast<uintptr_t>(gy) | reinterpret_cast<uintptr_t>(u)) & 15) == 0 && (length & 3) == 0) ? 1 : 0;
  if ((long long)a.B * a.ntt > 0x7fffffffLL) return fail(EBEN_EINVAL, "ResidualUnit grid too large");
  const int np = rs_pieces(math);
  switch (np) {
    case 1:
      switch (channels / 32) {
        case 1: return launch_ru3_bwd<1, 4, 1, 1>(a, st);
        case 2: return launch_ru3_bwd<2, 4, 1, 2>(a, st);
        default: return nw == 4 ? launch_ru3_bwd<4, 4, 1, 2>(a, st) : launch_ru3_bwd<4, 2, 1, 2>(a, st);
      }
    case 2:
      switch (channels / 32) {
        case 1: return launch_ru3_bwd<1, 4, 2, 1>(a, st);
        case 2: return launch_ru3_bwd<2, 4, 2, 2>(a, st);
        default: return rs_waves(128) == 4 ? launch_ru3_bwd<4, 4, 2, 1>(a, st) : launch_ru3_bwd<4, 2, 2, 1>(a, st);
      }
    default:
      switch (channels / 32) {
        case 1: return launch_ru3_bwd<1, 4, 3, 1>(a, st);
        case 2: return launch_ru3_bwd<2, 4, 3, 1>(a, st);
        default: return rs_waves(128) == 4 ? launch_ru3_bwd<4, 4, 3, 1>(a, st) : launch_ru3_bwd<4, 2, 3, 1>(a, st);
      }
  }
}

}

using namespace eben;

extern "C" size_t eben_ru_packed_floats_ex(int channels, int math) {
  if (math == EBEN_MATH_F32) return eben_ru_packed_floats(channels);
  return ru3_packed_floats(channels, math);
}

extern "C" int eben_ru_supported(int channels, int dilation, int math) {
  if (math == EBEN_MATH_F32) return (channels == 32 || channels == 64 || channels == 128) && dilation >= 1 && dilation <= 16;
  return ru3_supported(channels, dilation, math);
}

extern "C" int eben_ru_pack_ex(int channels, int math, int which, const float* v_dil, const float* scale_dil, const float* v_pw,
                               const float* scale_pw, float* wimg, void* stream) {
  EBEN_REQUIRE(which == 0 || which == 1, "ru_pack_ex: which = 0 (forward image) or 1 (backward image)");
  if (math == EBEN_MATH_F32)
    return which == 0 ? eben_ru_pack(channels, v_dil, scale_dil, v_pw, scale_pw, wimg, stream)
                      : eben_ru_pack_bwd(channels, v_dil, scale_dil, v_pw, scale_pw, wimg, stream);
  EBEN_REQUIRE(ru3_supported(channels, 1, math), "fused ResidualUnit: 32, 64 or 128 channels and a known math mode (got %d, %d)", channels, math);
  EBEN_REQUIRE(v_dil && v_pw && wimg, "null pointer in ru_pack_ex");
  return ru3_pack(channels, math, which, v_dil, scale_dil, v_pw, scale_pw, wimg, as_stream(stream));
}

extern "C" int eben_ru_pack_multi(const EbenRuPackJob* jobs, int n, void* stream) {
  EBEN_REQUIRE(n >= 0 && (n == 0 || jobs != nullptr), "bad ru pack job list");
  for (int base = 0; base < n; base += RU_PACK_MULTI) {
    RuPackTable T;
    T.n = n - base < RU_PACK_MULTI ? n - base : RU_PACK_MULTI;
    T.first[0] = 0;
    for (int j = 0; j < T.n; ++j) {
      const EbenRuPackJob& jb = jobs[base + j];
      EBEN_REQUIRE(jb.math != EBEN_MATH_F32, "ru_pack_multi: the split-operand images only (pack the fp32 MFMA images with eben_ru_pack)");
      EBEN_REQUIRE(ru3_supported(jb.channels, 1, jb.math) && (jb.which == 0 || jb.which == 1) && jb.v_dil && jb.v_pw && jb.wimg, "bad ru pack job %d", base + j);
      const int CT = jb.channels / 32;
      T.job[j].vd = jb.v_dil; T.job[j].sd = jb.scale_dil; T.job[j].vp = jb.v_pw; T.job[j].sp = jb.scale_pw;
      T.job[j].img = reinterpret_cast<u32x4*>(jb.wimg);
      T.job[j].CT = (short)CT; T.job[j].NP = (short)rs_pieces(jb.math); T.job[j].which = (short)jb.which; T.job[j].pad = 0;
      T.first[j + 1] = (unsigned short)(T.first[j] + ceil_div(8 * CT * CT * 64, 256));
    }
    hipLaunchKernelGGL(ru3_pack_multi_kernel, dim3(T.first[T.n]), dim3(256), 0, as_stream(stream), T);
    EBEN_CHECK_LAUNCH("ru3_pack_multi_kernel");
  }
  return EBEN_OK;
}

extern "C" int eben_ru_fwd_ex(int math, int batch, int channels, int length, int dilation, const float* x, float in_slope, float out_slope,
                              const float* wimg, float* y, float* h, float* u, void* stream) {
  if (math == EBEN_MATH_F32) return eben_ru_fwd(batch, channels, length, dilation, x, in_slope, out_slope, wimg, y, h, u, stream);
  EBEN_REQUIRE(ru3_supported(channels, dilation, math), "fused ResidualUnit (split bf16): 32 / 64 / 128 channels, dilation 1..%d (got %d, %d)",
               RS_DMAX, channels, dilation);
  EBEN_REQUIRE(batch > 0 && length > 0 && dilation < length, "bad ResidualUnit geometry");
  EBEN_REQUIRE(x && wimg && y, "null pointer in ru_fwd_ex");
  return ru3_fwd(math, batch, channels, length, dilation, x, in_slope, out_slope, wimg, y, h, u, as_stream(stream));
}

extern "C" int eben_ru_bwd_ex(int math, int batch, int channels, int length, int dilation, const float* gy, const float* u, float out_slope,
                              const float* x, float in_slope, const float* post, const float* wimg_bwd, float* gx, float* gh, void* stream) {
  if (math == EBEN_MATH_F32) return eben_ru_bwd(batch, channels, length, dilation, gy, u, out_slope, x, in_slope, post, wimg_bwd, gx, gh, stream);
  EBEN_REQUIRE(ru3_supported(channels, dilation, math), "fused ResidualUnit (split bf16): 32 / 64 / 128 channels, dilation 1..%d (got %d, %d)",
               RS_DMAX, channels, dilation);
  EBEN_REQUIRE(batch > 0 && length > 0 && dilation < length, "bad ResidualUnit geometry");
  EBEN_REQUIRE(gy && u && wimg_bwd && gx && gh, "null pointer in ru_bwd_ex");
  EBEN_REQUIRE(in_slope == 1.f || x, "x is required to differentiate the fused input activation");
  return ru3_bwd(math, batch, channels, length, dilation, gy, u, out_slope, x, in_slope, post, wimg_bwd, gx, gh, as_stream(stream));
}

extern "C" int eben_rubl_fwd(int math, int batch, int channels, int length, int dilation, const float* x, float in_slope, float out_slope,
                             const float* wimg, float* y, void* xb, void* hb, void* umask, void* stream) {
  EBEN_REQUIRE(ru3_supported(channels, dilation, math), "fused ResidualUnit (split bf16): 32 / 64 / 128 channels, dilation 1..%d (got %d, %d)",
               RS_DMAX, channels, dilation);
  EBEN_REQUIRE(batch > 0 && length > 0 && dilation < length, "bad ResidualUnit geometry");
  EBEN_REQUIRE(x && wimg && y && xb && hb && umask, "null pointer in rubl_fwd");
  return ru3_fwd_bl(math, batch, channels, length, dilation, x, in_slope, out_slope, wimg, y, xb, hb, umask, as_stream(stream));
}
```

### vibravox_amd/csrc/tapconv.hip

```cpp
#include "common.h"
#include "tap3.h"

#include <cstdlib>

namespace eben {

struct TapArgs {
  const float* x;
  const float* xmask;
  const float* wp;
  const float* bias;
  const float* res;
  const float* emask;
  float* y;
  int B, G, Cg, Mg, Mp, Cx, Cy, Lx, Ly;
  int S, OS, dstep, J, KCpad, CI_T, ncc;
  int mode;
  int off0, nt;
  int ps_pad, ps_k, ps_d, ps_kstep;
  int reflect, in_mode;
  float in_slope, out_slope, res_slope, emask_slope;
  int accumulate;
  int res_rows, em_seg, em_map[4];
  int PLEN, CSTRIDE;
// ... 283 lines not shown

struct TapPlan {
  int mode;
  int Cg, Mg, G, CI_T, ncc, J, KCpad, Mp, cfg, BM, BN;
  int S, OS, dstep, kstep, nph, PLEN, CSTRIDE;
  int Lx, Ly, Cx, Cy, off0, nt, ps_pad;
  int ntt, nmt;
  size_t lds_bytes;
  long long phase_stride;
  size_t packed_floats;
};

constexpr int kTapBM = 16, kTapBN = 256;

static void make_plan(const Canon& c, int dir, TapPlan* p) {
  p->mode = dir;
  p->G = c.g;
  if (dir == 0) {
    p->Cg = c.Cin / c.g; p->Mg = c.Cout / c.g;
    p->S = c.s; p->OS = 1; p->dstep = c.d; p->kstep = 1; p->nph = 1; p->J = c.k;
    p->Lx = c.Lin; p->Ly = c.Lout; p->Cx = c.Cin; p->Cy = c.Cout;
    p->off0 = -c.pl; p->nt = c.Lout; p->ps_pad = 0;
  } else {
    p->Cg = c.Cout / c.g; p->Mg = c.Cin / c.g;
    p->S = 1; p->OS = c.s;
    p->kstep = c.s / gcd_i(c.s, c.d);
    p->dstep = -(c.d * p->kstep) / c.s;
    p->nph = c.s;
    p->J = ceil_div(c.k, p->kstep);
    p->Lx = c.Lout; p->Cx = c.Cout; p->Cy = c.Cin;
    p->Ly = c.reflect ? c.Lin + c.pl + c.pr : c.Lin;
    p->ps_pad = c.reflect ? 0 : c.pl;
    p->off0 = 0; p->nt = ceil_div(p->Ly, c.s);
  }
  p->cfg = 3;
  p->BM = kTapBM; p->BN = kTapBN;
  p->Mp = round_up(p->Mg, p->BM);
  p->nmt = p->Mp / p->BM;
  p->ntt = ceil_div(p->nt, p->BN);
  const int adstep = p->dstep >= 0 ? p->dstep : -p->dstep;
  const int KT = 4096 / p->BM;
  {
    const int maxd = ((p->J - 1) * adstep) / p->S + 1;
    p->PLEN = p->BN + maxd + 1;
    p->CSTRIDE = round_up(p->S * p->PLEN, 32) + 16;
  }
  static const int env_cap = getenv("EBEN_TAP_CI_CAP") ? atoi(getenv("EBEN_TAP_CI_CAP")) : 0;
  static const int env_kb = getenv("EBEN_TAP_X_KB") ? atoi(getenv("EBEN_TAP_X_KB")) : 0;
  int cap = (int)(((env_kb > 0 ? env_kb : 24) * 1024) / (4 * (size_t)p->CSTRIDE));
  if (cap > (env_cap > 0 ? env_cap : 16)) cap = env_cap > 0 ? env_cap : 16;
  if (cap < 1) cap = 1;
  int ci;
  if (p->Cg <= cap) ci = p->Cg;
  else {
    const int nch = ceil_div(p->Cg, cap);
    ci = ceil_div(p->Cg, nch);
  }
  for (;;) {
    p->CI_T = ci;
    p->KCpad = round_up(p->J * ci, 4);
    p->lds_bytes = 4ull * ((size_t)round_up(p->KCpad, KT) + (size_t)KT * (p->BM + 16) + (size_t)ci * p->CSTRIDE);
    if (p->lds_bytes <= 160 * 1024 || ci == 1) break;
    ci = ci / 2 > 0 ? ci / 2 : 1;
  }
  p->ncc = ceil_div(p->Cg, p->CI_T);
  p->phase_stride = (long long)p->G * p->ncc * p->KCpad * p->Mp;
  p->packed_floats = (size_t)p->phase_stride * p->nph;
}

struct PackArgs {
  const float* w;
  const float* scale;
  float* wp;
  int G, Cg, Mg, Mp, CI_T, ncc, KCpad, J, nph;
  int mode, k, s, d, kstep, ps_pad, Cin_g, Cout_g;
  long long phase_stride;
};

__global__ __launch_bounds__(256) void pack_kernel(const PackArgs P) {
  const long long total = P.phase_stride * P.nph;
  for (long long i = (long long)blockIdx.x * 256 + threadIdx.x; i < total; i += (long long)gridDim.x * 256) {
    long long r = i;
    const int m = r % P.Mp; r /= P.Mp;
    const int f = r % P.KCpad; r /= P.KCpad;
    const int cc = r % P.ncc; r /= P.ncc;
    const int g = r % P.G;
    const int ph = r / P.G;
    const int j = f / P.CI_T, cl = f - j * P.CI_T;
    const int chan = cc * P.CI_T + cl;
    float v = 0.f;
    if (m < P.Mg && chan < P.Cg && j < P.J) {
      if (P.mode == 0) {
        const int co = g * P.Cout_g + m;
        v = P.w[((long long)co * P.Cin_g + chan) * P.k + j];
        if (P.scale) v *= P.scale[co];
      } else {
        int k0 = -1;
        for (int c = 0; c < P.kstep; ++c) {
          int q = (ph + P.ps_pad - c * P.d) % P.s;
          if (q < 0) q += P.s;
          if (q == 0) { k0 = c; break; }
        }
        const int kk = k0 + j * P.kstep;
        if (k0 >= 0 && kk < P.k) {
          const int co = g * P.Cout_g + chan;
          v = P.w[((long long)co * P.Cin_g + m) * P.k + kk];
          if (P.scale) v *= P.scale[co];
        }
      }
    }
    P.wp[i] = v;
  }
}

static int launch_pack(const Canon& c, const TapPlan& p, const float* w, const float* scale, float* wp, hipStream_t st) {
  PackArgs a;
  a.w = w; a.scale = scale; a.wp = wp;
  a.G = p.G; a.Cg = p.Cg; a.Mg = p.Mg; a.Mp = p.Mp; a.CI_T = p.CI_T; a.ncc = p.ncc; a.KCpad = p.KCpad; a.J = p.J; a.nph = p.nph;
  a.mode = p.mode; a.k = c.k; a.s = c.s; a.d = c.d; a.kstep = p.kstep; a.ps_pad = p.ps_pad;
  a.Cin_g = c.Cin / c.g; a.Cout_g = c.Cout / c.g;
  a.phase_stride = p.phase_stride;
  const long long total = p.phase_stride * p.nph;
  int blocks = (int)((total + 255) / 256);
  if (blocks > 8192) blocks = 8192;
  if (blocks < 1) blocks = 1;
  hipLaunchKernelGGL(pack_kernel, dim3(blocks), dim3(256), 0, st, a);
  EBEN_CHECK_LAUNCH("pack_kernel");
  return EBEN_OK;
}

template <int WM, int WN, int FM, int FN>
static int launch_cfg(const TapArgs& a, int nblocks, size_t lds, hipStream_t st) {
  static LdsAttrOnce attr_once;
  auto kern = tapconv_kernel<WM, WN, FM, FN>;
  {
    const hipError_t e = lds_attr_once(attr_once, reinterpret_cast<const void*>(kern));
    if (e != hipSuccess) return hip_fail(e, "hipFuncSetAttribute(tapconv)");
  }
  hipLaunchKernelGGL(kern, dim3(nblocks), dim3(WM * WN * 64), lds, st, a);
  EBEN_CHECK_LAUNCH("tapconv_kernel");
  return EBEN_OK;
}

static int launch_tap(const Canon& c, const TapPlan& p, const TapIO& io, int reflect, hipStream_t st) {
  if (p.lds_bytes > 160 * 1024) return fail(EBEN_EUNSUPPORTED, "tapconv tile needs %zu B of LDS", p.lds_bytes);
  TapArgs a;
  a.x = io.x; a.xmask = io.xmask; a.wp = io.wp; a.bias = io.bias; a.res = io.res; a.emask = io.emask; a.y = io.y;
  a.B = c.B; a.G = p.G; a.Cg = p.Cg; a.Mg = p.Mg; a.Mp = p.Mp; a.Cx = p.Cx; a.Cy = p.Cy; a.Lx = p.Lx; a.Ly = p.Ly;
  a.S = p.S; a.OS = p.OS; a.dstep = p.dstep; a.J = p.J; a.KCpad = p.KCpad; a.CI_T = p.CI_T; a.ncc = p.ncc;
  a.mode = p.mode; a.off0 = p.off0; a.nt = p.nt;
  a.ps_pad = p.ps_pad; a.ps_k = c.k; a.ps_d = c.d; a.ps_kstep = p.kstep;
  a.reflect = reflect; a.in_mode = io.in_mode;
  a.in_slope = io.in_slope; a.out_slope = io.out_slope; a.res_slope = io.res_slope; a.emask_slope = io.emask_slope;
  a.accumulate = io.accumulate;
  a.res_rows = io.res_rows; a.em_seg = io.em_seg;
  for (int i = 0; i < 4; ++i) a.em_map[i] = io.em_map[i];
  a.PLEN = p.PLEN; a.CSTRIDE = p.CSTRIDE;
  a.s_magic = p.S > 1 ? (unsigned)((0x100000000ull + p.S - 1) / p.S) : 0u;
  a.ntt = p.ntt; a.nmt = p.nmt; a.nph = p.nph;
  a.phase_stride = p.phase_stride;
  const long long nb = (long long)p.ntt * c.B * p.nph * p.nmt * p.G;
  if (nb <= 0 || nb > 0x7fffffffLL) return fail(EBEN_EINVAL, "tapconv grid of %lld blocks", nb);
  return launch_cfg<1, 4, 1, 4>(a, (int)nb, p.lds_bytes, st);
}

__global__ __launch_bounds__(1024) void conv_m1_fwd_kernel(const float* __restrict__ x, const float* __restrict__ wp,
                                                           const float* __restrict__ bias, float* __restrict__ y, int C, int Lx,
                                                           int Ly, int J, int pad, int dil, int CI_T, int KCpad, int Mp,
                                                           float out_slope) {
  __shared__ float part[16][64];
  const int lane = threadIdx.x & 63, w = threadIdx.x >> 6;
  const int b = blockIdx.y, t = blockIdx.x * 64 + lane;
  const float* xb = x + (long long)b * C * Lx;
  float acc = 0.f;
  if (J == 3) {
    int q[3], ok[3];
#pragma unroll
    for (int j = 0; j < 3; ++j) {
      const int qq = t - pad + j * dil;
      ok[j] = (int)(qq >= 0) & (int)(qq < Lx);
      q[j] = ok[j] ? qq : 0;
    }
    int cc = w / CI_T, cl = w - cc * CI_T;
    for (int c = w; c < C; c += 64) {
      float xv[4][3], wv[4][3];
#pragma unroll
      for (int u = 0; u < 4; ++u) {
        const int cu = c + 16 * u;
        const bool live = cu < C;
        const float* xr = xb + (long long)(live ? cu : w) * Lx;
        const float* wc = wp + ((long long)cc * KCpad + cl) * Mp;
#pragma unroll
        for (int j = 0; j < 3; ++j) {
          xv[u][j] = xr[q[j]];
          wv[u][j] = live ? wc[(long long)j * CI_T * Mp] : 0.f;
          if (!ok[j]) xv[u][j] = 0.f;
        }
        cl += 16;
        while (cl >= CI_T) { cl -= CI_T; ++cc; }
      }
#pragma unroll
      for (int u = 0; u < 4; ++u)
#pragma unroll
        for (int j = 0; j < 3; ++j)
          if (c + 16 * u < C) acc = fmaf(wv[u][j], xv[u][j], acc);
    }
  } else {
    for (int c = w; c < C; c += 16) {
      const int cc = c / CI_T, cl = c - cc * CI_T;
      const float* xr = xb + (long long)c * Lx;
      const float* wc = wp + ((long long)cc * KCpad + cl) * Mp;
      for (int j = 0; j < J; ++j) {
        const int q = t - pad + j * dil;
        const float xv = (q >= 0 && q < Lx) ? xr[q] : 0.f;
        acc = fmaf(wc[(long long)j * CI_T * Mp], xv, acc);
      }
    }
  }
  part[w][lane] = acc;
  __syncthreads();
  if (w == 0 && t < Ly) {
    float s = bias ? bias[0] : 0.f;
#pragma unroll
    for (int i = 0; i < 16; ++i) s += part[i][lane];
    y[(long long)b * Ly + t] = lrelu(s, out_slope);
  }
}

__global__ __launch_bounds__(256) void fold_kernel(const float* __restrict__ D, const float* __restrict__ mask, float* __restrict__ dx,
                                                   long long rows, int L, int pl, int pr, float slope, int accumulate,
                                                   const float* __restrict__ pre, const float* __restrict__ post) {
  const int Lp = L + pl + pr;
  const long long total = rows * L;
  for (long long i = (long long)blockIdx.x * 256 + threadIdx.x; i < total; i += (long long)gridDim.x * 256) {
    const long long row = i / L;
    const int u = (int)(i - row * L);
    const float* d = D + row * Lp;
    float v = d[u + pl];
    if (u >= 1 && u <= pl) v += d[pl - u];
    if (u >= L - 1 - pr && u <= L - 2) v += d[pl + 2 * (L - 1) - u];
    if (pre) v += pre[i];
    if (mask) v *= dlrelu(mask[i], slope);
    if (post) v += post[i];
    if (accumulate) v += dx[i];
    dx[i] = v;
  }
}

}

using namespace eben;

namespace eben {
int tap_generation(const Canon& c, int dir) {
  static const int thin_first = getenv("EBEN_THIN_FIRST") ? atoi(getenv("EBEN_THIN_FIRST")) : 0;
  if (c.bl) return tap3_applicable(c, dir) ? 4 : 0;
  if (c.bf16 && tap3_applicable(c, dir)) return 4;
  const int t2 = tap2_applicable(c, dir), th = thin_applicable(c, dir);
  if (th && (thin_first || !t2)) return 3;
  if (t2) return 2;
  return 1;
}
}

extern "C" size_t eben_conv1d_packed_floats(const EbenConv1dDesc* d, int which) {
  Canon c;
  if (canon_from_desc(d, &c) != EBEN_OK) return 0;
  TapPlan p;
  const int dir = d->transposed ? 1 - which : which;
  if (which == 0 && gc_applicable(c, dir)) return gc_packed_floats(c, dir);
  const int gen = tap_generation(c, dir);
  if (gen == 2) return tap2_packed_floats(c, dir);
  if (gen == 3) return thin_packed_floats(c, dir);
  if (gen == 4) return tap3_packed_floats(c, dir);
  make_plan(c, dir, &p);
  return p.packed_floats;
}

extern "C" int eben_conv1d_kernel_generation(const EbenConv1dDesc* d, int which) {
  Canon c;
  if (canon_from_desc(d, &c) != EBEN_OK) return 0;
  if (which == 0 && gc_applicable(c, d->transposed ? 1 : 0)) return 5;
  const int dir = d->transposed ? 1 - which : which;
  const int gen = tap_generation(c, dir);
  return gen == 4 && tap3_is_big(c, dir) ? 6 : gen;
}

extern "C" int eben_conv1d_variant(const EbenConv1dDesc* d, int which, int mask_on_load, int* out, int n) {
  EBEN_REQUIRE(out && n >= 8 && (which == 0 || which == 1), "eben_conv1d_variant: which 0 / 1 and 8 output slots");
  EBEN_REQUIRE(!mask_on_load || which == 1, "eben_conv1d_variant: the mask is applied on load by input gradients only");
  Canon c;
  const int rc = canon_from_desc(d, &c);
  if (rc) return rc;
  for (int i = 0; i < 8; ++i) out[i] = 0;
  out[0] = eben_conv1d_kernel_generation(d, which);
  if (out[0] != 4 && out[0] != 6) return EBEN_OK;
  const int dir = d->transposed ? 1 - which : which;
  Tap3Call k{};
  k.bl = c.bl; k.in_mode = mask_on_load ? 1 : 0; k.reflect = which == 0 && c.reflect && !d->transposed;
  Tap3Variant v;
  if (const int e = tap3_plan_variant(c, dir, k, &v)) return e;
  out[1] = v.FM; out[2] = v.XRB; out[3] = v.IM; out[4] = v.NPW; out[5] = v.NPX; out[6] = v.BL; out[7] = v.kernel;
  return EBEN_OK;
}

extern "C" int eben_conv1d_pack(const EbenConv1dDesc* d, const float* v, const float* scale, float* wp_fwd, float* wp_bwd, void* stream) {
  Canon c;
  int rc = canon_from_desc(d, &c);
  if (rc) return rc;
  EBEN_REQUIRE(v != nullptr, "null weight");
  for (int which = 0; which < 2; ++which) {
    float* dst = which == 0 ? wp_fwd : wp_bwd;
    if (!dst) continue;
    const int dir = d->transposed ? 1 - which : which;
    if (which == 0 && gc_applicable(c, dir)) {
      if ((rc = gc_pack(c, dir, v, scale, dst, as_stream(stream)))) return rc;
      continue;
    }
    const int gen = tap_generation(c, dir);
    if (gen != 1) {
      rc = gen == 2 ? tap2_pack(c, dir, v, scale, dst, as_stream(stream))
         : gen == 4 ? tap3_pack(c, dir, v, scale, dst, as_stream(stream)) : thin_pack(c, dir, v, scale, dst, as_stream(stream));
      if (rc) return rc;
      continue;
    }
    TapPlan p;
    make_plan(c, dir, &p);
    rc = launch_pack(c, p, v, scale, dst, as_stream(stream));
    if (rc) return rc;
  }
  return EBEN_OK;
}

extern "C" int eben_conv1d_pack_multi(const EbenPackJob* jobs, int n, void* stream) {
  EBEN_REQUIRE(n >= 0 && (n == 0 || jobs != nullptr), "bad pack job list");
  constexpr int CAP = 512;
  static thread_local Canon cs[CAP];
  static thread_local int dirs[CAP];
  static thread_local const float* ws[CAP];
  static thread_local const float* scs[CAP];
  static thread_local float* wps[CAP];
  int m = 0;
  auto flush = [&]() -> int {
    const int rc = m ? tap3_pack_multi(cs, dirs, ws, scs, wps, m, as_stream(stream)) : EBEN_OK;
    m = 0;
    return rc;
  };
  for (int i = 0; i < n; ++i) {
    const EbenPackJob& jb = jobs[i];
    Canon c;
    int rc = canon_from_desc(&jb.desc, &c);
    if (rc) return rc;
    EBEN_REQUIRE(jb.v != nullptr, "null weight");
    for (int which = 0; which < 2; ++which) {
      float* dst = which == 0 ? jb.wp_fwd : jb.wp_bwd;
      if (!dst) continue;
      const int dir = jb.desc.transposed ? 1 - which : which;
      if (!(which == 0 && gc_applicable(c, dir)) && tap_generation(c, dir) == 4) {
        if (m == CAP && (rc = flush())) return rc;
        cs[m] = c; dirs[m] = dir; ws[m] = jb.v; scs[m] = jb.scale; wps[m] = dst;
        ++m;
      } else {
        rc = eben_conv1d_pack(&jb.desc, jb.v, jb.scale, which == 0 ? dst : nullptr, which == 1 ? dst : nullptr, stream);
        if (rc) return rc;
      }
    }
  }
  return flush();
}

static int conv1d_fwd_impl(const EbenConv1dDesc* d, const float* x, const float* wp_fwd, const float* bias,
                           const float* residual, float res_slope, float* y, void* stream) {
  Canon c;
  int rc = canon_from_desc(d, &c);
  if (rc) return rc;
  EBEN_REQUIRE(x && wp_fwd && y, "null pointer in conv1d_fwd");
  TapPlan p;
  make_plan(c, d->transposed ? 1 : 0, &p);
  if (!d->transposed && c.Cout == 1 && c.g == 1 && c.s == 1 && !c.reflect && d->in_slope == 1.f && !residual && tap_generation(c, 0) == 1) {
    hipLaunchKernelGGL(conv_m1_fwd_kernel, dim3(ceil_div(c.Lout, 64), c.B), dim3(1024), 0, as_stream(stream), x, wp_fwd, bias, y,
                       c.Cin, c.Lin, c.Lout, c.k, c.pl, c.d, p.CI_T, p.KCpad, p.Mp, d->out_slope);
    EBEN_CHECK_LAUNCH("conv_m1_fwd_kernel");
    return EBEN_OK;
  }
  TapIO io{};
  io.x = x; io.in_mode = 0; io.in_slope = d->in_slope; io.wp = wp_fwd; io.bias = bias;
  io.res = residual; io.res_slope = res_slope; io.emask = nullptr; io.emask_slope = 1.f;
  io.out_slope = d->out_slope; io.y = y; io.accumulate = 0;
  if (gc_applicable(c, d->transposed ? 1 : 0)) return gc_launch(c, d->transposed ? 1 : 0, io, as_stream(stream));
  const int fgen = tap_generation(c, d->transposed ? 1 : 0);
  if (fgen == 2) return tap2_launch(c, d->transposed ? 1 : 0, io, c.reflect && !d->transposed, as_stream(stream));
  if (fgen == 3) return thin_launch(c, d->transposed ? 1 : 0, io, c.reflect && !d->transposed, as_stream(stream));
  if (fgen == 4) return tap3_launch(c, d->transposed ? 1 : 0, io, c.reflect && !d->transposed, as_stream(stream));
  return launch_tap(c, p, io, c.reflect && !d->transposed, as_stream(stream));
}

extern "C" int eben_conv1d_fwd(const EbenConv1dDesc* d, const float* x, const float* wp_fwd, const float* bias,
                               const float* residual, float* y, void* stream) {
  return conv1d_fwd_impl(d, x, wp_fwd, bias, residual, 1.f, y, stream);
}

extern "C" int eben_conv1d_fwd_res(const EbenConv1dDesc* d, const float* x, const float* wp_fwd, const float* bias,
                                   const float* residual, float res_slope, float* y, void* stream) {
  EBEN_REQUIRE(residual != nullptr, "conv1d_fwd_res without a residual");
  return conv1d_fwd_impl(d, x, wp_fwd, bias, residual, res_slope, y, stream);
}

extern "C" size_t eben_conv1d_bwd_dx_workspace(const EbenConv1dDesc* d) {
  Canon c;
  if (canon_from_desc(d, &c) != EBEN_OK) return 0;
  if (!d->transposed && c.reflect) return sizeof(float) * (size_t)c.B * c.Cin * (c.Lin + c.pl + c.pr);
  return 0;
}

static int conv1d_bwd_dx_impl(const EbenConv1dDesc* d, const float* dy, const float* y, const float* wp_bwd, const float* x,
                              const float* res_pre, const float* res_post, float* dx, int accumulate, void* workspace, size_t ws_bytes,
                              void* stream) {
  Canon c;
  int rc = canon_from_desc(d, &c);
  if (rc) return rc;
  EBEN_REQUIRE(dy && wp_bwd && dx, "null pointer in conv1d_bwd_dx");
  EBEN_REQUIRE(d->out_slope == 1.f || y, "y is required to differentiate the fused output activation");
  EBEN_REQUIRE(d->in_slope == 1.f || x, "x is required to differentiate the fused input activation");
  hipStream_t st = as_stream(stream);
  TapPlan p;
  const int dir = d->transposed ? 0 : 1;
  const int gen = tap_generation(c, dir);
  make_plan(c, dir, &p);
  TapIO io{};
  io.x = dy; io.wp = wp_bwd; io.bias = nullptr; io.res = nullptr; io.res_slope = 1.f; io.out_slope = 1.f;
  if (d->out_slope != 1.f) { io.in_mode = 1; io.xmask = y; io.in_slope = d->out_slope; }
  else { io.in_mode = 0; io.in_slope = 1.f; }
  const bool fold = !d->transposed && c.reflect;
  if (!fold) {
    if (res_post) return fail(EBEN_EUNSUPPORTED, "bwd_dx: an addend behind the input-activation mask needs the reflect-fold pass");
    io.res = res_pre;
    io.emask = d->in_slope != 1.f ? x : nullptr; io.emask_slope = d->in_slope;
    io.y = dx; io.accumulate = accumulate;
    return gen == 2 ? tap2_launch(c, dir, io, 0, st) : gen == 3 ? thin_launch(c, dir, io, 0, st)
         : gen == 4 ? tap3_launch(c, dir, io, 0, st) : launch_tap(c, p, io, 0, st);
  }
  const size_t need = eben_conv1d_bwd_dx_workspace(d);
  if (!workspace || ws_bytes < need) return fail(EBEN_EWORKSPACE, "bwd_dx needs %zu workspace bytes, got %zu", need, ws_bytes);
  io.emask = nullptr; io.emask_slope = 1.f; io.y = static_cast<float*>(workspace); io.accumulate = 0;
  rc = gen == 2 ? tap2_launch(c, dir, io, 0, st) : gen == 3 ? thin_launch(c, dir, io, 0, st)
     : gen == 4 ? tap3_launch(c, dir, io, 0, st) : launch_tap(c, p, io, 0, st);
  if (rc) return rc;
  const long long rows = (long long)c.B * c.Cin;
  long long blocks = (rows * c.Lin + 255) / 256;
  if (blocks > 4096) blocks = 4096;
  hipLaunchKernelGGL(fold_kernel, dim3((unsigned)blocks), dim3(256), 0, st, static_cast<const float*>(workspace),
                     d->in_slope != 1.f ? x : nullptr, dx, rows, c.Lin, c.pl, c.pr, d->in_slope, accumulate, res_pre, res_post);
  EBEN_CHECK_LAUNCH("fold_kernel");
  return EBEN_OK;
}

extern "C" int eben_conv1d_bwd_dx(const EbenConv1dDesc* d, const float* dy, const float* y, const float* wp_bwd,
                                  const float* x, float* dx, int accumulate, void* workspace, size_t ws_bytes, void* stream) {
  return conv1d_bwd_dx_impl(d, dy, y, wp_bwd, x, nullptr, nullptr, dx, accumulate, workspace, ws_bytes, stream);
}

extern "C" int eben_conv1d_bwd_dx_res(const EbenConv1dDesc* d, const float* dy, const float* y, const float* wp_bwd, const float* x,
                                      const float* res_pre, const float* res_post, float* dx, void* workspace, size_t ws_bytes,
                                      void* stream) {
  return conv1d_bwd_dx_impl(d, dy, y, wp_bwd, x, res_pre, res_post, dx, 0, workspace, ws_bytes, stream);
}

static int bwd_dx_batched(const EbenConv1dDesc* d, const float* g, const float* wp_bwd, const float* res, int res_rows, const float* fm_sums,
                          float fm_gs, const float* mask, float mask_slope, int seg, const int* seg_map, float* dx, void* stream);
extern "C" int eben_conv1d_bwd_dx_ex(const EbenConv1dDesc* d, const float* g, const float* wp_bwd, const float* res, int res_rows,
                                     const float* mask, float mask_slope, int seg, const int* seg_map, float* dx, void* stream) {
  return bwd_dx_batched(d, g, wp_bwd, res, res_rows, nullptr, 0.f, mask, mask_slope, seg, seg_map, dx, stream);
}
extern "C" int eben_conv1d_bwd_dx_fm(const EbenConv1dDesc* d, const float* g, const float* wp_bwd, const float* ref, int fm_rows,
                                     const float* fm_sums, float fm_gs, const float* mask, float mask_slope, int seg, const int* seg_map,
                                     float* dx, void* stream) {
  EBEN_REQUIRE(ref && fm_sums && mask && fm_rows > 0, "bad feature-matching arguments in conv1d_bwd_dx_fm");
  return bwd_dx_batched(d, g, wp_bwd, ref, fm_rows, fm_sums, fm_gs, mask, mask_slope, seg, seg_map, dx, stream);
}
static int bwd_dx_batched(const EbenConv1dDesc* d, const float* g, const float* wp_bwd, const float* res, int res_rows, const float* fm_sums,
                          float fm_gs, const float* mask, float mask_slope, int seg, const int* seg_map, float* dx, void* stream) {
  Canon c;
  int rc = canon_from_desc(d, &c);
  if (rc) return rc;
  EBEN_REQUIRE(g && wp_bwd && dx, "null pointer in conv1d_bwd_dx_ex");
  EBEN_REQUIRE(!(c.reflect && !d->transposed), "bwd_dx_ex does not fold reflect padding (pad explicitly)");
  EBEN_REQUIRE(seg >= 0 && (seg == 0 || (seg_map && c.B <= 4 * seg)), "bad batch segment map");
  const int dir = d->transposed ? 0 : 1;
  TapIO io{};
  io.x = g; io.in_mode = 0; io.in_slope = 1.f; io.wp = wp_bwd; io.out_slope = 1.f;
  io.res = res; io.res_slope = 1.f; io.res_rows = res_rows;
  io.emask = mask; io.emask_slope = mask_slope; io.em_seg = mask ? seg : 0;
  for (int i = 0; i < 4; ++i) io.em_map[i] = (seg > 0 && seg_map) ? seg_map[i] : i;
  io.y = dx; io.accumulate = 0;
  const int gen = tap_generation(c, dir);
  io.fm_sums = fm_sums; io.fm_gs = fm_gs;
  if (fm_sums && gen != 3 && gen != 4) return fail(EBEN_EUNSUPPORTED, "conv1d_bwd_dx_fm: kernel generation %d has no feature-matching epilogue", gen);
  hipStream_t st = as_stream(stream);
  if (gen == 2) return tap2_launch(c, dir, io, 0, st);
  if (gen == 3) return thin_launch(c, dir, io, 0, st);
  if (gen == 4) return tap3_launch(c, dir, io, 0, st);
  TapPlan p;
  make_plan(c, dir, &p);
  return launch_tap(c, p, io, 0, st);
}

namespace eben {
struct PrGeom { int ok, S, umin, kq, Lq, fold, cbg, order; };

static int pr_floordiv(int a, int b) { int q = a / b; if ((a % b != 0) && ((a < 0) != (b < 0))) --q; return q; }

static PrGeom pr_geometry(const Canon& c, Canon* cp) {
  PrGeom g{};
  static const int min_s = getenv("EBEN_PR_MIN_STRIDE") ? atoi(getenv("EBEN_PR_MIN_STRIDE")) : 4;
  static const int max_d = getenv("EBEN_PR_MAX_DIL") ? atoi(getenv("EBEN_PR_MAX_DIL")) : 1;
  static const int s2_max_d = getenv("EBEN_PR2_S2_MAX_DIL") ? atoi(getenv("EBEN_PR2_S2_MAX_DIL")) : 2;
  const bool s2 = c.s == 2 && c.d <= s2_max_d;
  if (!c.bl || c.np != 1 || c.reflect || (c.d > max_d && !s2) || c.s < 2 || (c.s < min_s && !s2) || c.s > 8 || (c.k - 1) * c.d + 1 <= c.s || c.pl > (c.k - 1) * c.d) return g;
  const int Cg = c.Cin / c.g;
  if ((c.Cin & 7) || (c.Cout & 7)) return g;
  g.S = c.s;
  g.umin = -pr_floordiv((c.k - 1) * c.d - c.pl, c.s);
  const int umax = pr_floordiv(c.s - 1 + c.pl, c.s);
  g.kq = umax - g.umin + 1;
  g.Lq = ceil_div(c.Lin, c.s);
  g.fold = (Cg & 7) != 0;
  g.cbg = g.fold ? c.Cin / 8 : Cg / 8;
  Canon q = c;
  q.Cin = c.Cout; q.Cout = c.s * c.Cin; q.Lin = c.Lout; q.Lout = g.Lq;
  q.k = g.kq; q.s = 1; q.d = 1; q.g = g.fold ? 1 : c.g;
  q.pl = -g.umin;
  q.pr = g.Lq - c.Lout + g.kq - 1 - q.pl;
  if (q.pl < 0 || q.pr < 0) return g;
  q.reflect = 0; q.xsplit_dir = -1;
  static const int max_rows = getenv("EBEN_PR_MAX_ROWS") ? atoi(getenv("EBEN_PR_MAX_ROWS")) : 64;
  static const int big_pr = getenv("EBEN_PR_BIG") ? atoi(getenv("EBEN_PR_BIG")) : 1;
  static const int small_pr2 = getenv("EBEN_PR2_TAP3") ? atoi(getenv("EBEN_PR2_TAP3")) : 1;
  g.order = (big_pr && c.s == 4 && c.d == 1 && (tap3_is_big(q, 0) || (small_pr2 && (q.Cout / q.g) % 32 == 0))) ? 1 : 0;
  if (s2) {
    if (tap3_is_big(q, 0) || (q.Cout / q.g) % 16 != 0) return g;
    g.order = 1;
  }
  if (q.Cout / q.g > max_rows && !g.order) return g;
  if (!tap3_applicable(q, 0)) return g;
  if (cp) *cp = q;
  g.ok = 1;
  return g;
}

__global__ __launch_bounds__(256) void pr_weights_kernel(const float* __restrict__ v, const float* __restrict__ scale, float* __restrict__ wq,
                                                          int Cin, int Cout, int G, int k, int S, int pad, int umin, int kq, int fold, int dil, int order) {
  const int Cg = Cin / G, Mg = Cout / G;
  const int cin_q = fold ? Cout : Mg;
  const long long total = (long long)S * Cin * cin_q * kq;
  for (long long i = (long long)blockIdx.x * 256 + threadIdx.x; i < total; i += (long long)gridDim.x * 256) {
    const int ui = (int)(i % kq);
    long long r = i / kq;
    const int cq = (int)(r % cin_q);
    const int row = (int)(r / cin_q);
    int ph, ci, co;
    if (fold && order) { const int lb = row >> 3, cb = lb / S; ph = lb - cb * S; ci = cb * 8 + (row & 7); co = cq; }
    else if (fold) { ph = row / Cin; ci = row - ph * Cin; co = cq; }
    else if (order == 0) { const int g = row / (S * Cg), rr = row - g * S * Cg; ph = rr / Cg; ci = g * Cg + (rr - ph * Cg); co = g * Mg + cq; }
    else {
      const int g = row / (S * Cg), rr = row - g * S * Cg, lb = rr >> 3, cb = lb / S;
      ph = lb - cb * S; ci = g * Cg + cb * 8 + (rr & 7); co = g * Mg + cq;
    }
    const int off = ph + pad - S * (ui + umin);
    const int j = off / dil;
    float w = 0.f;
    if (off >= 0 && j * dil == off && j < k && co / Mg == ci / Cg) w = v[((long long)co * Cg + (ci % Cg)) * k + j] * (scale ? scale[co] : 1.f);
    wq[i] = w;
  }
}

static void pr_desc_from_canon(const EbenConv1dDesc* d, const Canon& q, EbenConv1dDesc* o) {
  *o = *d;
  o->c_in = q.Cin; o->c_out = q.Cout; o->l_in = q.Lin; o->l_out = q.Lout; o->ksize = q.k; o->stride = 1; o->dilation = 1; o->groups = q.g;
  o->pad_l = q.pl; o->pad_r = q.pr; o->pad_mode = EBEN_PAD_ZERO; o->transposed = 0; o->in_slope = 1.f; o->out_slope = 1.f;
}
}

extern "C" int eben_bl_dx_pr_desc(const EbenConv1dDesc* d, EbenConv1dDesc* primed) {
  Canon c, q;
  int rc = canon_from_desc(d, &c);
  if (rc) return rc;
  if (d->transposed || !pr_geometry(c, &q).ok) return fail(EBEN_EUNSUPPORTED, "eben_bl_dx_pr_desc: the layer's input gradient has no phases-as-rows form");
  EBEN_REQUIRE(primed != nullptr, "null output descriptor");
  pr_desc_from_canon(d, q, primed);
  return EBEN_OK;
}

extern "C" int eben_bl_dx_pr_weights(const EbenConv1dDesc* d, const float* v, const float* scale, float* w_primed, void* stream) {
  Canon c, q;
  int rc = canon_from_desc(d, &c);
  if (rc) return rc;
  const PrGeom g = d->transposed ? PrGeom{} : pr_geometry(c, &q);
  if (!g.ok) return fail(EBEN_EUNSUPPORTED, "eben_bl_dx_pr_weights: the layer's input gradient has no phases-as-rows form");
  EBEN_REQUIRE(v && w_primed, "null pointer in eben_bl_dx_pr_weights");
  const long long total = (long long)q.Cout * (q.Cin / q.g) * q.k;
  long long blocks = (total + 255) / 256;
  if (blocks > 4096) blocks = 4096;
  hipLaunchKernelGGL(pr_weights_kernel, dim3((unsigned)blocks), dim3(256), 0, as_stream(stream), v, scale, w_primed, c.Cin, c.Cout, c.g, c.k, c.s, c.pl,
                     g.umin, g.kq, g.fold, c.d, g.order);
  EBEN_CHECK_LAUNCH("pr_weights_kernel");
  return EBEN_OK;
// ... 73 lines not shown
```

### vibravox_amd/gen_engine.py

```python
from __future__ import annotations

import ctypes
import dataclasses
import contextlib
import os
from typing import Dict, List, Optional

import torch

from . import ops
from ._lib import check, load, ptr, stream

USE_FUSED_RU = os.environ.get("EBEN_RU_FUSED", "1") != "0"
USE_FUSED_RU_BWD = os.environ.get("EBEN_RU_FUSED_BWD", "1") != "0"
USE_FUSED_RU_DW = os.environ.get("EBEN_RU_FUSED_DW", "1") != "0"
USE_RU_BL = os.environ.get("EBEN_RU_BL", "1") != "0"
DEFER_MARK_READY = os.environ.get("EBEN_G_DEFER_READY", "1") != "0"
USE_GRAPHS = os.environ.get("EBEN_GEN_GRAPHS", "1") != "0"
BWD_GROUPS = os.environ.get("EBEN_GEN_BWD_GROUPS", "1,1,1,1,1,1,1")
_RU_MATH = {"f32": ops.MATH_F32, "bf16x6": ops.MATH_BF16X6, "bf16x3": ops.MATH_BF16X3, "bf16": ops.MATH_BF16}
RU_FWD_MATH = _RU_MATH[os.environ.get("EBEN_RU_FWD_MATH", "bf16x6")]
_ru_fwd_math = [RU_FWD_MATH]


def ru_forward_math() -> int:
    return _ru_fwd_math[0]


def set_ru_forward_math(name=None) -> None:
    _ru_fwd_math[0] = RU_FWD_MATH if name is None else _RU_MATH[name]
RU_BWD_F32_MATH = _RU_MATH[os.environ.get("EBEN_RU_BWD_F32_MATH", "bf16x6")]
CONV_FWD_MATH = _RU_MATH[os.environ.get("EBEN_GEN_CONV_FWD_MATH", "bf16x6")]
_conv_fwd_math = [CONV_FWD_MATH]


def conv_forward_math() -> int:
    return _conv_fwd_math[0]


def set_forward_math(name=None) -> None:
    set_ru_forward_math(name)
    _conv_fwd_math[0] = CONV_FWD_MATH if name is None else _RU_MATH[name]


@contextlib.contextmanager
def forward_math(name=None):
    saved = (_ru_fwd_math[0], _conv_fwd_math[0])
    set_forward_math(name)
    try:
        yield
    finally:
        _ru_fwd_math[0], _conv_fwd_math[0] = saved


S2D_MIN_STRIDE = int(os.environ.get("EBEN_GEN_S2D_MIN_STRIDE", "8"))


def _params(m):
    return ops.conv_params(m)


class _ConvRec:

    __slots__ = ("m", "spec", "d", "x", "y", "wp_bwd", "norm", "scale")

    def __init__(self, m, spec, d, x, y, wp_bwd, norm, scale=None):
        self.m, self.spec, self.d, self.x, self.y, self.wp_bwd, self.norm, self.scale = m, spec, d, x, y, wp_bwd, norm, scale


class GeneratorEngine:
    def __init__(self, gen):
        self.gen = gen
        self._spec_cache: Dict[tuple, ops.ConvSpec] = {}
        self._ru_images: Dict[int, ops.PackedWeights] = {}
        self._s2d_images: Dict[int, tuple] = {}
        self._fwd_graph = ops.ReplayedChain()
        self._dx_graphs: List[ops.ReplayedChain] = []
        self._dw_graphs: List[ops.ReplayedChain] = []
        self._static: Dict[tuple, torch.Tensor] = {}
        self._dwq: Optional[list] = None
        self._core_convs = self._core_units = None

    def _spec(self, m, in_slope=None, out_slope=None) -> ops.ConvSpec:
        if in_slope is None and out_slope is None:
            return m.spec
        key = (id(m), in_slope, out_slope)
        s = self._spec_cache.get(key)
        if s is None:
            kw = {}
            if in_slope is not None:
                kw["in_slope"] = float(in_slope)
            if out_slope is not None:
                kw["out_slope"] = float(out_slope)
            s = self._spec_cache[key] = dataclasses.replace(m.spec, **kw)
        return s

    def _pack(self, m, spec, batch, l_in, train):
        d = ops.conv_desc(spec, batch, l_in, conv_forward_math())
        d_bwd = ops.conv_desc(spec, batch, l_in, ops._backward_math[0])
        v, g = _params(m)
        pw = ops.pack_weights(m.spec, d, v.detach(), None if g is None else g.detach(), m._packed, train, d_bwd)
        return d, d_bwd, pw

    def _s2d_route(self, m, spec, batch: int, l_q: int, kq: int, math: int, c: int, rows_out: int, in_slope: float, out_slope: float, scale):
        lib = load()
        alt = self._spec_cache.get((id(m), "s2d", in_slope, out_slope))
        if alt is None:
            alt = self._spec_cache[(id(m), "s2d", in_slope, out_slope)] = ops.ConvSpec(
                c_in=c * spec.stride, c_out=rows_out, ksize=kq, in_slope=float(in_slope), out_slope=float(out_slope))
        d = ops.conv_desc(alt, batch, l_q, math)
        if lib.eben_conv1d_kernel_generation(ctypes.byref(d), 0) != 4:
            return None
        v, g = _params(m)
        key = ops.weights_key((v, g), batch, l_q, math)
        hit = self._s2d_images.get(id(m))
        if hit is None or hit[0] != key:
            vv = v.detach().view(rows_out, c, kq, spec.stride).permute(0, 1, 3, 2).reshape(rows_out, c * spec.stride, kq).contiguous()
            wp = torch.empty(lib.eben_conv1d_packed_floats(ctypes.byref(d), 0), dtype=torch.float32, device=v.device)
            ops.conv1d_pack(d, vv, scale, wp, None)
            hit = self._s2d_images[id(m)] = (key, wp, vv)
        return d, hit[1]

    @staticmethod
    def _s2d_wanted(spec, math: int) -> bool:
        return (S2D_MIN_STRIDE > 0 and spec.stride >= S2D_MIN_STRIDE and spec.ksize % spec.stride == 0 and spec.groups == 1
                and spec.dilation == 1 and math != ops.MATH_F32)

    def _conv(self, m, x, train, in_slope=None, recs=None):
        lib = load()
        spec = self._spec(m, in_slope=in_slope)
        b, _, l_in = x.shape
        d, d_bwd, pw = self._pack(m, spec, b, l_in, train)
        y = torch.empty((b, spec.c_out, d.l_out), dtype=torch.float32, device=x.device)
        route = None
        if not spec.transposed and self._s2d_wanted(spec, conv_forward_math()) and lib.eben_conv1d_kernel_generation(ctypes.byref(d), 0) not in (4, 5):
            kq = spec.ksize // spec.stride
            l_q = d.l_out + kq - 1
            route = self._s2d_route(m, spec, b, l_q, kq, conv_forward_math(), spec.c_in, spec.c_out, spec.in_slope, spec.out_slope, pw.scale)
        if route is not None:
            xq = torch.empty((b, spec.c_in * spec.stride, l_q), dtype=torch.float32, device=x.device)
            check(lib.eben_space_to_depth(ptr(x), None, 1.0, ptr(xq), b * spec.c_in, l_in, spec.stride, -spec.pad_l, l_q,
                                          1 if spec.reflect else 0, stream()), "space_to_depth")
            check(lib.eben_conv1d_fwd(ctypes.byref(route[0]), ptr(xq), ptr(route[1]), ptr(m.bias), None, ptr(y), stream()), "conv1d_fwd")
        else:
            check(lib.eben_conv1d_fwd(ctypes.byref(d), ptr(x), ptr(pw.wp_fwd), ptr(m.bias), None, ptr(y), stream()), "conv1d_fwd")
        if recs is not None:
            recs.append(_ConvRec(m, spec, d_bwd, x, y if spec.out_slope != 1.0 else None, pw.wp_bwd, pw.norm, pw.scale))
        return y

    @staticmethod
    def _ru_bwd_math() -> int:
        return ops.MATH_BF16 if ops._backward_math[0] != ops.MATH_F32 else RU_BWD_F32_MATH

    def _ru_cache(self, ru) -> ops.PackedWeights:
        c = self._ru_images.get(id(ru))
        if c is None:
            c = self._ru_images[id(ru)] = ops.PackedWeights()
        c.params = _params(ru.dilated_conv) + _params(ru.pointwise_conv)
        return c

    def _ru_image(self, ru, which: int = 0) -> torch.Tensor:
        c = self._ru_cache(ru)
        slot = ("fwd", ru_forward_math()) if which == 0 else ("bwd", self._ru_bwd_math())
        if not c.current(slot, ops.weights_key(c.params)):
            self._ru_rebuild(ru, c, slot)
        return c.images[slot][1]

    def _ru_rebuild(self, ru, c: ops.PackedWeights, slot) -> None:
        lib = load()
        vd, _, vp, _ = c.params
        vd, vp = vd.detach(), vp.detach()
        ch = vd.shape[0]
        key = ops.weights_key(c.params)
        fwd = ("fwd", ru_forward_math())
        slots = [slot]
        if not c.current(fwd, key):
            if not c.reuse:
                c.scale_key = None
                c.ensure_scale()
            old, c.images = c.images, {}
            bwd = [s for s in old if s[0] == "bwd"]
            slots = [fwd] + bwd + ([slot] if slot != fwd and slot not in bwd else [])
        else:
            old = c.images
        for s in slots:
            hit = old.get(s)
            img = c.buffer(None if hit is None else hit[1], lib.eben_ru_packed_floats_ex(ch, s[1]), vd)
            ops.ru_pack(ch, s[1], 0 if s[0] == "fwd" else 1, vd, c.scale[0], vp, c.scale[2], img)
            c.images[s] = (key, img)

    def image_caches(self) -> list:
        return [(c, lambda slot, ru=ru, c=c: self._ru_rebuild(ru, c, slot))
                for ru in self._units() if (c := self._ru_images.get(id(ru))) is not None and c.images]

    def _units(self) -> list:
        if self._core_units is None:
            self._core_units = [ru for blk in list(self.gen.encoder_blocks) + list(self.gen.decoder_blocks) for ru in blk.residuals]
        return self._core_units

    def _residual_unit(self, ru, x, in_slope, train, recs):
        lib = load()
        b, c, l = x.shape
        dil, pwc = ru.dilated_conv, ru.pointwise_conv
        if train:
            spec_d = self._spec(dil, in_slope=in_slope if in_slope != 1.0 else None)
            _, dd_bwd, pw_d = self._pack(dil, spec_d, b, l, True)
            _, dp_bwd, pw_p = self._pack(pwc, pwc.spec, b, l, True)
        fwd_math = ru_forward_math()
        fusable = dil.spec.ksize == 3 and dil.spec.reflect and lib.eben_ru_supported(c, dil.spec.dilation, fwd_math) == 1
        if (train and USE_RU_BL and USE_FUSED_RU and USE_FUSED_RU_BWD and USE_FUSED_RU_DW and fusable and fwd_math in (ops.MATH_BF16X6, ops.MATH_BF16X3)
                and self._ru_bwd_math() == ops.MATH_BF16 and lib.eben_rubl_supported(c, dil.spec.dilation) == 1 and self._ru_bl_params_ok(ru, l)):
            img = self._ru_image(ru)
            y = torch.empty_like(x)
            xb = torch.empty((b, c // 8, l, 8), dtype=torch.bfloat16, device=x.device)
            hb = torch.empty_like(xb)
            um = torch.empty((b, c // 8, l), dtype=torch.uint8, device=x.device)
            check(lib.eben_rubl_fwd(fwd_math, b, c, l, dil.spec.dilation, ptr(x), float(in_slope), float(pwc.spec.out_slope), ptr(img), ptr(y),
                                    xb.data_ptr(), hb.data_ptr(), um.data_ptr(), stream()), "rubl_fwd")
            recs.append((("bl", self._ru_image(ru, 1), xb, hb, um), _ConvRec(dil, spec_d, dd_bwd, x if in_slope != 1.0 else None, None, pw_d.wp_bwd, pw_d.norm),
                         _ConvRec(pwc, pwc.spec, dp_bwd, None, None, pw_p.wp_bwd, pw_p.norm)))
            return y
        if USE_FUSED_RU and fusable:
            img = self._ru_image(ru)
            y = torch.empty_like(x)
            h = torch.empty_like(x) if train else None
            u = torch.empty_like(x) if train else None
            check(lib.eben_ru_fwd_ex(fwd_math, b, c, l, dil.spec.dilation, ptr(x), float(in_slope), float(pwc.spec.out_slope), ptr(img), ptr(y),
                                     ptr(h), ptr(u), stream()), "ru_fwd")
        else:
            xin = x
            if in_slope != 1.0:
                xin = torch.empty_like(x)
                check(lib.eben_lrelu_fwd(ptr(x), ptr(xin), x.numel(), float(in_slope), stream()), "lrelu_fwd")
            h = self._conv(dil, xin, train)
            u = self._conv(pwc, h, train)
            y = torch.empty_like(x)
            check(lib.eben_add(ptr(xin), ptr(u), ptr(y), x.numel(), stream()), "add")
        if train:
            bm = self._ru_bwd_math()
            fused = USE_FUSED_RU_BWD and dil.spec.ksize == 3 and dil.spec.reflect and lib.eben_ru_supported(c, dil.spec.dilation, bm) == 1
            recs.append(((self._ru_image(ru, 1), bm) if fused else None, _ConvRec(dil, spec_d, dd_bwd, x, None, pw_d.wp_bwd, pw_d.norm),
                         _ConvRec(pwc, pwc.spec, dp_bwd, h, u, pw_p.wp_bwd, pw_p.norm)))
        return y

    def forward(self, cut_audio: torch.Tensor, train: bool):
        gen = self.gen
        lib = load()
        ops.join_prepack()
        slope = gen.nl.negative_slope
        first_bands = gen.pqmf(cut_audio, "analysis", bands=gen.p).detach()
        saved = {"enc": [], "dec": [], "misc": []} if train else None
        a = self._conv(gen.first_conv, first_bands, train, recs=saved["misc"] if train else None)
        skips = []
        for blk in gen.encoder_blocks:
            recs = [] if train else None
            cur = a
            for k, ru in enumerate(blk.residuals):
                cur = self._residual_unit(ru, cur, slope if k == 0 else 1.0, train, recs)
            a = self._conv(blk.conv, cur, train, recs=recs)
            skips.append(a)
            if train:
                saved["enc"].append(recs)
        lat = [] if train else None
        l1 = self._conv(gen.latent_conv[1], a, train, in_slope=slope, recs=lat)
        cur = self._conv(gen.latent_conv[3], l1, train, recs=lat)
        if train:
            saved["latent"] = lat
        for blk, skip in zip(gen.decoder_blocks, reversed(skips)):
            recs = [] if train else None
            s = torch.empty_like(cur)
            check(lib.eben_add(ptr(cur), ptr(skip), ptr(s), cur.numel(), stream()), "add")
            cur = self._conv(blk.conv_trans, s, train, recs=recs)
            for ru in blk.residuals:
                cur = self._residual_unit(ru, cur, 1.0, train, recs)
            if train:
                saved["dec"].append(recs)
        return cur, first_bands, saved

    def _dx(self, rec: _ConvRec, dy, res_pre=None, res_post=None):
        lib = load()
        d = rec.d
        spec = rec.spec
        if (spec.transposed and res_pre is None and res_post is None and spec.in_slope == 1.0 and spec.output_padding == 0
                and self._s2d_wanted(spec, d.math) and lib.eben_conv1d_kernel_generation(ctypes.byref(d), 1) != 4):
            b, c_dy, l_dy = dy.shape
            kq = spec.ksize // spec.stride
            l_q = rec.x.shape[2] + kq - 1
            route = self._s2d_route(rec.m, spec, b, l_q, kq, d.math, c_dy, spec.c_in, 1.0, 1.0, rec.scale)
            if route is not None:
                gq = torch.empty((b, c_dy * spec.stride, l_q), dtype=torch.float32, device=dy.device)
                check(lib.eben_space_to_depth(ptr(dy), ptr(rec.y) if spec.out_slope != 1.0 else None, spec.out_slope, ptr(gq), b * c_dy, l_dy,
                                              spec.stride, -spec.pad_l, l_q, 0, stream()), "space_to_depth")
                dx = torch.empty_like(rec.x)
                check(lib.eben_conv1d_fwd(ctypes.byref(route[0]), ptr(gq), ptr(route[1]), None, None, ptr(dx), stream()), "conv1d_fwd")
                return dx
        ws_bytes = getattr(d, "_dx_ws", None)
        if ws_bytes is None:
            ws_bytes = d._dx_ws = lib.eben_conv1d_bwd_dx_workspace(ctypes.byref(d))
        ws = ops._empty(ws_bytes, dy) if ws_bytes else None
        dx = torch.empty_like(rec.x)
        xmask = rec.x if rec.spec.in_slope != 1.0 else None
        check(lib.eben_conv1d_bwd_dx_res(ctypes.byref(d), ptr(dy), ptr(rec.y), ptr(rec.wp_bwd), ptr(xmask), ptr(res_pre), ptr(res_post), ptr(dx),
                                         ptr(ws), ws_bytes, stream()), "conv1d_bwd_dx_res")
        return dx

    def _dw(self, rec: _ConvRec, dy):
        if ops._skip_weight_grads[0]:
            return
        if self._dwq is not None:
            self._dwq.append(("conv", rec, dy))
            return
        if _params(rec.m)[0].requires_grad:
            self._accumulate(self._conv_grads(rec, dy))

    @staticmethod
    def _accumulate(pairs) -> None:
        for p, t in pairs:
            if p is not None and t is not None and p.requires_grad:
                p.grad = t if p.grad is None else p.grad.add_(t)
                for hook in list((getattr(p, "_post_accumulate_grad_hooks", None) or {}).values()):
                    hook(p)

    @staticmethod
    def _conv_grads(rec: _ConvRec, dy) -> list:
        v, g = _params(rec.m)
        grads = ops.weight_grads(rec.d, dy, rec.y, rec.x, v, g, rec.m.bias, rec.norm)
        return [(p, t) for p, t in zip((v, g, rec.m.bias), grads) if p is not None and t is not None]

    @staticmethod
    def _unit_pairs(dil: _ConvRec, pwc: _ConvRec, res) -> list:
        return list(zip(_params(pwc.m), res[0][:2])) + list(zip(_params(dil.m), res[1][:2]))

    def _unit_grads(self, dil: _ConvRec, pwc: _ConvRec, gy, gh, bm: int, trainable_only: bool) -> list:
        (vd, gd), (vp, gp) = _params(dil.m), _params(pwc.m)
        wanted = lambda *ps: not trainable_only or all(p.requires_grad for p in ps)
        if (USE_FUSED_RU_DW and gd is not None and gp is not None and dil.m.bias is None and pwc.m.bias is None and wanted(vd, vp, gd, gp)
                and bm in (ops.MATH_BF16, ops.MATH_BF16X6)):
            res = ops.weight_grads_ru(bm, dil.spec.dilation, gy, pwc.y, float(pwc.spec.out_slope), pwc.x, gh, dil.x, float(dil.spec.in_slope),
                                      (vp, gp, pwc.norm), (vd, gd, dil.norm))
            if res is not False:
                return self._unit_pairs(dil, pwc, res)
        return [pair for rec, dy in ((pwc, gy), (dil, gh)) if wanted(_params(rec.m)[0]) for pair in self._conv_grads(rec, dy)]

    def _unit_grads_bl(self, dil: _ConvRec, pwc: _ConvRec, gzb, hb, ghb, xb):
        (vd, gd), (vp, gp) = _params(dil.m), _params(pwc.m)
        res = ops.weight_grads_ru_bl(dil.spec.dilation, gzb, hb, ghb, xb, (vp, gp, pwc.norm), (vd, gd, dil.norm))
        return False if res is False else self._unit_pairs(dil, pwc, res)

    def _ru_dw(self, dil: _ConvRec, pwc: _ConvRec, gy, gh, bm: int) -> None:
        if ops._skip_weight_grads[0]:
            return
        if self._dwq is not None:
            self._dwq.append(("ru", dil, pwc, gy, gh, bm))
            return
        self._accumulate(self._unit_grads(dil, pwc, gy, gh, bm, trainable_only=True))

    @staticmethod
    def _ru_bl_params_ok(ru, length: int) -> bool:
        keys = []
        for m in (ru.dilated_conv, ru.pointwise_conv):
            v, g = _params(m)
            if g is None or m.bias is not None or not (v.requires_grad and g.requires_grad):
                return False
            keys.append((v.grad is None and g.grad is None, ops._no_grad_hooks(v) and ops._no_grad_hooks(g)))
        return keys[0] == keys[1] and ru.dilated_conv.spec.dilation < length

    def _ru_backward_bl(self, rec, gy, res_post=None):
        (_, img_b, xb, hb, um), dil, pwc = rec
        b, c, l = gy.shape
        gx = torch.empty_like(gy)
        gzb, ghb = torch.empty_like(xb), torch.empty_like(xb)
        ins = dil.spec.in_slope
        check(load().eben_rubl_bwd(b, c, l, dil.spec.dilation, ptr(gy), um.data_ptr(), float(pwc.spec.out_slope), ptr(dil.x) if ins != 1.0 else None,
                                   float(ins), ptr(res_post), ptr(img_b), ptr(gx), gzb.data_ptr(), ghb.data_ptr(), stream()), "rubl_bwd")
        if not ops._skip_weight_grads[0]:
            if self._dwq is not None:
                self._dwq.append(("rubl", dil, pwc, gzb, hb, ghb, xb))
            else:
                res = self._unit_grads_bl(dil, pwc, gzb, hb, ghb, xb)
                if res is False:
                    raise RuntimeError("bundle-layout ResidualUnit: the two convs' weight gradients are routed differently (one of them holds a gradient "
                                       "or a hook the other does not); set EBEN_RU_BL=0 for this pattern")
                self._accumulate(res)
        return gx

    def _ru_backward(self, rec, gy, res_post=None):
        fused, dil, pwc = rec
        if fused is not None and fused[0] == "bl":
            return self._ru_backward_bl(rec, gy, res_post)
        if fused is not None:
            b, c, l = gy.shape
            gx, gh = torch.empty_like(gy), torch.empty_like(gy)
            ins = dil.spec.in_slope
            img_b, bm = fused
            check(load().eben_ru_bwd_ex(bm, b, c, l, dil.spec.dilation, ptr(gy), ptr(pwc.y), float(pwc.spec.out_slope),
                                        ptr(dil.x) if ins != 1.0 else None, float(ins), ptr(res_post), ptr(img_b), ptr(gx), ptr(gh), stream()), "ru_bwd")
            self._ru_dw(dil, pwc, gy, gh, bm)
            return gx
        gh = self._dx(pwc, gy)
        self._dw(pwc, gy)
        gx = self._dx(dil, gh, res_pre=gy, res_post=res_post)
        self._dw(dil, gh)
        return gx

    def _n_segments(self, saved) -> int:
        return len(saved["dec"]) + 1 + len(saved["enc"])

    def _bwd_segment(self, saved, k: int, g: torch.Tensor, skip_grads: list) -> torch.Tensor:
        n_dec, n_enc = len(saved["dec"]), len(saved["enc"])
        if k < n_dec:
            recs = saved["dec"][n_dec - 1 - k]
            for rec in reversed(recs[1:]):
                g = self._ru_backward(rec, g)
            ct = recs[0]
            gs = self._dx(ct, g)
            self._dw(ct, g)
            skip_grads.append(gs)
            return gs
        if k == n_dec:
            c1, c2 = saved["latent"]
            gl1 = self._dx(c2, g)
            self._dw(c2, g)
            g = self._dx(c1, gl1, res_post=skip_grads[-1])
            self._dw(c1, gl1)
            return g
        i = n_enc - 1 - (k - n_dec - 1)
        recs = saved["enc"][i]
        conv = recs[-1]
        gy = self._dx(conv, g)
        self._dw(conv, g)
        for rec in reversed(recs[1:-1]):
            gy = self._ru_backward(rec, gy)
        post = skip_grads[i - 1] if i >= 1 else None
        g = self._ru_backward(recs[0], gy, res_post=post)
        if i == 0:
            self._dw(saved["misc"][0], g)
        return g

    @torch.no_grad()
    def backward(self, saved, g_pre: torch.Tensor) -> None:
        g = g_pre.contiguous()
        skip_grads: List[Optional[torch.Tensor]] = []
        for k in range(self._n_segments(saved)):
            g = self._bwd_segment(saved, k, g, skip_grads)

    @staticmethod
    def _graphs_usable() -> bool:
        return USE_GRAPHS and ops.ReplayedChain.enabled and not ops.ReplayedPrepack._multi_rank() and not ops._timers_enabled()

    def _static_buf(self, name: str, like: torch.Tensor) -> torch.Tensor:
        key = (name, tuple(like.shape), like.dtype, like.device)
        buf = self._static.get(key)
        if buf is None:
            if len(self._static) >= 8:
                self._static.pop(next(iter(self._static)))
            buf = self._static[key] = torch.empty_like(like, memory_format=torch.contiguous_format)
        return buf

    def _fwd_sig(self, buf: torch.Tensor) -> tuple:
        if self._core_convs is None:
            gen = self.gen
            from .torch_modules.utils import HipConv1d
            self._core_convs = [m for part in (gen.first_conv, gen.encoder_blocks, gen.latent_conv, gen.decoder_blocks)
                                for m in part.modules() if isinstance(m, HipConv1d)]
        parts = [buf.data_ptr(), tuple(buf.shape), ops._backward_math[0], conv_forward_math(), ru_forward_math()]
        parts += [m._packed.state() for m in self._core_convs]
        parts += [None if (c := self._ru_images.get(id(ru))) is None else c.state() for ru in self._units()]
        return tuple(parts)

    def forward_train(self, x: torch.Tensor):
        self._fwd_replayed = False
        self._serial = getattr(self, "_serial", 0) + 1
        if not self._graphs_usable() or self._replay_outstanding():
            return self.forward(x, True)
        ops.join_prepack()
        buf = self._static_buf("x", x)
        buf.copy_(x)
        out = self._fwd_graph.run(self._fwd_sig(buf), lambda: self.forward(buf, True), None)
        self._fwd_replayed = self._fwd_graph.graph is not None
        if self._fwd_replayed:
            self._graph_serial = self._serial
        return out

    def _replay_outstanding(self) -> bool:
        ref = getattr(self, "_outstanding", None)
        if ref is None:
            return False
        if ref() is None:
            self._outstanding = None
            return False
        return True

    def _note_ctx(self, ctx) -> None:
        import weakref
        ctx.serial = self._serial
        self._outstanding = weakref.ref(ctx) if self._fwd_replayed else None

    def _deferrable(self) -> bool:
        if not ops._side["enabled"] or ops._skip_weight_grads[0]:
            return False
        sink = ops._side["sink"]
        for m in self._core_convs:
            for p in _params(m) + (m.bias,):
                if p is None:
                    continue
                if not p.requires_grad:
                    return False
                if sink is not None:
                    if sink.grad_buffer(p) is None:
                        return False
                elif p.grad is not None or not ops._no_grad_hooks(p):
                    return False
        return True

    def _dw_body(self, queue: list, sink=None) -> list:
        jobs, assign = [], []
        with ops.collect_wn_jobs(jobs, sink):
            for kind, *item in queue:
                if kind == "conv":
                    assign += self._conv_grads(*item)
                elif kind == "rubl":
                    res = self._unit_grads_bl(*item)
                    assert res is not False
                    assign += res
                else:
                    assign += self._unit_grads(*item, trainable_only=False)
        ops.wn_bwd_multi(jobs)
        return assign

    @torch.no_grad()
    def backward_train(self, saved, g_pre: torch.Tensor, serial: Optional[int] = None) -> None:
        from_graph = self._fwd_graph.out is not None and saved is self._fwd_graph.out[2]
        if from_graph and serial is not None and serial != getattr(self, "_graph_serial", None):
            raise RuntimeError("EBEN generator engine: this forward's saved activations were rewritten by a later replayed forward (backward "
                               "through an old graph after a new training forward); set EBEN_GEN_GRAPHS=0 for that pattern")
        self._outstanding = None
        if not (self._graphs_usable() and getattr(self, "_fwd_replayed", False) and from_graph and self._deferrable()):
            return self.backward(saved, g_pre)
        gbuf = self._static_buf("g", g_pre)
        gbuf.copy_(g_pre)
        n = self._n_segments(saved)
        sizes = [int(t) for t in BWD_GROUPS.split(",")] if BWD_GROUPS else []
        if sum(sizes) != n:
            sizes = [1] * n
        bounds = [sum(sizes[:i]) for i in range(len(sizes) + 1)]
        while len(self._dx_graphs) < len(sizes):
            self._dx_graphs.append(ops.ReplayedChain())
            self._dw_graphs.append(ops.ReplayedChain())
        dev = gbuf.device
        main = torch.cuda.current_stream(dev)
        side = ops._side_stream(dev)
        g, skip_grads = gbuf, []
        for k in range(len(sizes)):
            def dx_body(k=k, g=g):
                self._dwq = []
                sk = list(skip_grads)
                try:
                    out = g
                    for seg in range(bounds[k], bounds[k + 1]):
                        out = self._bwd_segment(saved, seg, out, sk)
                finally:
                    queue, self._dwq = self._dwq, None
                return out, sk[len(skip_grads):], queue

            g, new_skips, queue = self._dx_graphs[k].run((self._fwd_graph.captures, gbuf.data_ptr(), ops._backward_math[0]), dx_body, None)
            skip_grads.extend(new_skips)
            if not queue:
                continue
            side.wait_stream(main)
            sink = ops._side["sink"]
            with torch.cuda.stream(side):
                if self._dx_graphs[k].graph is not None:
                    assign = self._dw_graphs[k].run((self._dx_graphs[k].captures, id(sink)), lambda: self._dw_body(queue, sink), side)
                else:
                    assign = self._dw_body(queue, sink)
                    ops._side["keep"].append(queue)
            if sink is None:
# ... 37 lines not shown
```

Measured before the change: 7510.

## Fuse decoder skip-add into residual unit epilogue and add K-split gen-conv path

Adds fwd_post variants of the fused residual-unit forward kernels that add the next decoder block's skip tensor in the epilogue. This removes a separate elementwise add launch and its full-tensor read/write in the decoder. The gen_conv kernel is also refactored into a body that gains a K-split variant: four waves split the reduction and sum through shared memory, with weights loaded straight into registers. A mixed boundary mode lets wavefronts with partial halo use vector loads for in-range lanes. The refactor adds template complexity and could raise register pressure.

```diff
diff --git a/include/eben_hip.h b/include/eben_hip.h
--- a/include/eben_hip.h
+++ b/include/eben_hip.h
@@ -78,6 +78,7 @@
 #define EBEN_VARIANT_THIN_BL 2
 #define EBEN_VARIANT_TAP4 3
 EBEN_API int eben_conv1d_variant(const EbenConv1dDesc* d, int which, int mask_on_load, int* out, int n);
+EBEN_API int eben_gc_plan_info(const EbenConv1dDesc* d, int which, int* out, int n);
 EBEN_API int eben_conv1d_pack(const EbenConv1dDesc* d, const float* v, const float* scale, float* wp_fwd, float* wp_bwd, void* stream);
 EBEN_API int eben_conv1d_fwd(const EbenConv1dDesc* d, const float* x, const float* wp_fwd, const float* bias,
                     const float* residual, float* y, void* stream);
@@ -171,6 +172,8 @@
                    const float* wimg, float* y, float* h, float* u, void* stream);
 EBEN_API int eben_ru_bwd_ex(int math, int batch, int channels, int length, int dilation, const float* gy, const float* u, float out_slope,
                    const float* x, float in_slope, const float* post, const float* wimg_bwd, float* gx, float* gh, void* stream);
+EBEN_API int eben_ru_fwd_post(int math, int batch, int channels, int length, int dilation, const float* x, float in_slope, float out_slope,
+                     const float* wimg, const float* post, float* y, float* h, float* u, void* stream);
 
 EBEN_API int eben_ru_dw_slabs(int batch, int channels, int length);
 EBEN_API int eben_ru_dw(int math, int batch, int channels, int length, int dilation, const float* gy, const float* u, float out_slope,
@@ -179,6 +182,8 @@
 EBEN_API int eben_rubl_supported(int channels, int dilation);
 EBEN_API int eben_rubl_fwd(int math, int batch, int channels, int length, int dilation, const float* x, float in_slope, float out_slope,
                            const float* wimg, float* y, void* xb, void* hb, void* umask, void* stream);
+EBEN_API int eben_rubl_fwd_post(int math, int batch, int channels, int length, int dilation, const float* x, float in_slope, float out_slope,
+                                const float* wimg, const float* post, float* y, void* xb, void* hb, void* umask, void* stream);
 EBEN_API int eben_rubl_bwd(int batch, int channels, int length, int dilation, const float* gy, const void* umask, float out_slope, const float* x,
                            float in_slope, const float* post, const float* wimg_bwd, float* gx, void* gzb, void* ghb, void* stream);
 EBEN_API int eben_rubl_dw_slabs(int batch, int channels, int length);
diff --git a/vibravox_amd/_lib.py b/vibravox_amd/_lib.py
--- a/vibravox_amd/_lib.py
+++ b/vibravox_amd/_lib.py
@@ -90,6 +90,7 @@
     "eben_conv1d_packed_floats": (c_size_t, [_D, c_int]),
     "eben_conv1d_kernel_generation": (c_int, [_D, c_int]),
     "eben_conv1d_variant": (c_int, [_D, c_int, c_int, POINTER(c_int), c_int]),
+    "eben_gc_plan_info": (c_int, [_D, c_int, POINTER(c_int), c_int]),
     "eben_conv1d_pack": (c_int, [_D, _P, _P, _P, _P, _P]),
     "eben_conv1d_pack_multi": (c_int, [POINTER(EbenPackJob), c_int, _P]),
     "eben_conv1d_fwd": (c_int, [_D, _P, _P, _P, _P, _P, _P]),
@@ -136,11 +137,13 @@
     "eben_ru_pack_ex": (c_int, [c_int, c_int, c_int, _P, _P, _P, _P, _P, _P]),
     "eben_ru_pack_multi": (c_int, [POINTER(EbenRuPackJob), c_int, _P]),
     "eben_ru_fwd_ex": (c_int, [c_int, c_int, c_int, c_int, c_int, _P, c_float, c_float, _P, _P, _P, _P, _P]),
+    "eben_ru_fwd_post": (c_int, [c_int, c_int, c_int, c_int, c_int, _P, c_float, c_float, _P, _P, _P, _P, _P, _P]),
     "eben_ru_bwd_ex": (c_int, [c_int, c_int, c_int, c_int, c_int, _P, _P, c_float, _P, c_float, _P, _P, _P, _P, _P]),
     "eben_ru_dw_slabs": (c_int, [c_int, c_int, c_int]),
     "eben_ru_dw": (c_int, [c_int, c_int, c_int, c_int, c_int, _P, _P, c_float, _P, _P, _P, c_float, _P, _P, _P]),
     "eben_rubl_supported": (c_int, [c_int, c_int]),
     "eben_rubl_fwd": (c_int, [c_int, c_int, c_int, c_int, c_int, _P, c_float, c_float, _P, _P, _P, _P, _P, _P]),
+    "eben_rubl_fwd_post": (c_int, [c_int, c_int, c_int, c_int, c_int, _P, c_float, c_float, _P, _P, _P, _P, _P, _P, _P]),
     "eben_rubl_bwd": (c_int, [c_int, c_int, c_int, c_int, _P, _P, c_float, _P, c_float, _P, _P, _P, _P, _P, _P]),
     "eben_rubl_dw_slabs": (c_int, [c_int, c_int, c_int]),
     "eben_rubl_dw": (c_int, [c_int, c_int, c_int, c_int, _P, _P, _P, _P, _P, _P, _P]),
diff --git a/vibravox_amd/csrc/common.h b/vibravox_amd/csrc/common.h
--- a/vibravox_amd/csrc/common.h
+++ b/vibravox_amd/csrc/common.h
@@ -167,6 +167,7 @@
 int tap3_launch(const Canon& c, int dir, const TapIO& io, int reflect, hipStream_t st);
 
 int gc_applicable(const Canon& c, int dir);
+int gc_plan_info(const Canon& c, int dir, int* out);
 size_t gc_packed_floats(const Canon& c, int dir);
 int gc_pack(const Canon& c, int dir, const float* w, const float* scale, float* wp, hipStream_t st);
 int gc_launch(const Canon& c, int dir, const TapIO& io, hipStream_t st);
diff --git a/vibravox_amd/csrc/gen_conv.hip b/vibravox_amd/csrc/gen_conv.hip
--- a/vibravox_amd/csrc/gen_conv.hip
+++ b/vibravox_amd/csrc/gen_conv.hip
@@ -22,6 +22,8 @@
   unsigned xq, xr;
 };
 
+constexpr int GC_KSPLIT = 4;
+
 __device__ __forceinline__ unsigned gc_pack2(float a, float b) {
   const f32x2 v = {a, b};
   return __builtin_bit_cast(unsigned, __builtin_convertvector(v, bf16x2));
@@ -51,12 +53,13 @@
 #define EBEN_GC_DBG 0
 #endif
 
-template <int FORM, int RT, int CT, int NP>
-__global__ __launch_bounds__(256, 2) void gc_kernel(const GcArgs P) {
+template <int FORM, int RT, int CT, int NP, bool KS>
+__device__ __forceinline__ void gc_body(const GcArgs& P) {
   constexpr int KC = (RT == 2 && CT == 2) ? 2 : 8 / RT;
   constexpr int RTU = KC * NP * 64;
   constexpr int SLOT = RT * RTU;
-  __shared__ __attribute__((aligned(16))) u32x4 Ws[2 * SLOT];
+  constexpr int NT = CT * RT;
+  __shared__ __attribute__((aligned(16))) u32x4 Ws[KS ? GC_KSPLIT * NT * 4 * 64 : 2 * SLOT];
 
   const int tid = threadIdx.x;
   const int lane = tid & 63;
@@ -76,6 +79,8 @@
   const float* xb = P.x + (long long)b * P.CX * P.LX;
   const u32x4* wsrc = P.wp + (long long)h * P.w_half + (long long)(rg * RT) * P.w_rt;
   const int nch = P.KSP / KC;
+  const int ch0 = KS ? __builtin_amdgcn_readfirstlane(wave * nch / GC_KSPLIT) : 0;
+  const int ch1 = KS ? __builtin_amdgcn_readfirstlane((wave + 1) * nch / GC_KSPLIT) : nch;
 
   constexpr int WPT = SLOT / 256;
   typedef const __attribute__((address_space(1))) char* gptr_t;
@@ -104,8 +109,20 @@
 #pragma unroll
     for (int p = 0; p < WPT; ++p) Ws[(ch & 1) * SLOT + p * 256 + tid] = wreg[p];
   };
-
-  const int u0w = (cb * 4 + wave) * (32 * CT);
+  auto load_wk = [&](int ks, u32x4 (&dst)[RT][NP]) {
+    if (EBEN_GC_DBG & 4) return;
+    const int kc = ks < ch1 * KC ? ks : ch1 * KC - 1;
+#pragma unroll
+    for (int i = 0; i < RT; ++i) {
+      unsigned long long a = reinterpret_cast<unsigned long long>(wsrc + (long long)i * P.w_rt + (long long)kc * (NP * 64));
+      asm volatile("" : "+s"(a));
+#pragma unroll
+      for (int q = 0; q < NP; ++q)
+        dst[i][q] = *reinterpret_cast<const __attribute__((address_space(1))) u32x4*>(reinterpret_cast<gptr_t>(a) + q * 1024 + (unsigned)lane * 16u);
+    }
+  };
+
+  const int u0w = (KS ? cb : cb * 4 + wave) * (32 * CT);
   int ucol[CT];
   bool fast[CT];
 #pragma unroll
@@ -137,16 +154,18 @@
     asm volatile("" : "+s"(a));
     return reinterpret_cast<gptr_t>(a);
   };
-  struct Slow { int off[8]; unsigned ok; };
+  struct Slow { int off[8]; unsigned ok; int voff; bool vec; };
   auto slow_init = [&](int ct, Slow& sl) {
     const int u = ucol[ct];
     sl.ok = 0;
+    sl.vec = true;
 #pragma unroll
     for (int e = 0; e < 8; ++e) {
       int crow, pos;
       if (FORM == 0) { crow = P.rpc_shift ? 0 : hk; pos = P.S * u + P.off0 + (P.rpc_shift ? 8 * hk : 0) + e; }
       else if (FORM == 1) { crow = 2 * hk + (e >> 2); pos = P.S * u + P.off0 + (e & 3); }
       else { crow = 4 * hk + (e >> 1); pos = u - 1 + h + (e & 1); }
+      sl.vec = sl.vec && pos >= 0 && pos < P.LX;
       if (P.reflect) {
         pos = pos < 0 ? -pos : pos;
         pos = pos >= P.LX ? 2 * (P.LX - 1) - pos : pos;
@@ -155,9 +174,18 @@
       sl.off[e] = crow * P.LX + (ok ? pos : 0);
       sl.ok |= (unsigned)ok << e;
     }
-  };
-  auto gather = [&](auto fast_tag, int ks, int ct, const Slow& sl, float (&v)[8]) {
-    constexpr bool FAST = decltype(fast_tag)::value;
+    sl.voff = loff[ct];
+  };
+  auto mixed_init = [&](int ct, Slow& sl) {
+    const unsigned long long inside = __ballot(sl.vec);
+    const int doff = __builtin_amdgcn_readlane(loff[ct], __builtin_ctzll(inside));
+#pragma unroll
+    for (int e = 0; e < 8; ++e) sl.off[e] = sl.vec ? doff : sl.off[e];
+    sl.voff = sl.vec ? sl.voff : doff;
+  };
+  auto gather = [&](auto mode_tag, int ks, int ct, const Slow& sl, float (&v)[8], float (&vd)[8]) {
+    constexpr int MODE = decltype(mode_tag)::value;
+    constexpr bool FAST = MODE == 0;
     if (EBEN_GC_DBG & 2) {
 #pragma unroll
       for (int e = 0; e < 8; ++e) v[e] = 1.f;
@@ -169,8 +197,8 @@
     typedef const __attribute__((address_space(1))) f4u* g4_t;
     typedef const __attribute__((address_space(1))) f2u* g2_t;
     typedef const __attribute__((address_space(1))) float* g1_t;
-    if constexpr (FAST) {
-      const unsigned o = (unsigned)loff[ct] * 4u;
+    if constexpr (MODE != 2) {
+      const unsigned o = (unsigned)(FAST ? loff[ct] : sl.voff) * 4u;
       if (FORM == 0) {
         const f4u a0 = *reinterpret_cast<g4_t>(rp + o), a1 = *reinterpret_cast<g4_t>(rp + 16 + o);
 #pragma unroll
@@ -186,7 +214,12 @@
           v[2 * r] = a[0]; v[2 * r + 1] = a[1];
         }
       }
-    } else {
+    }
+    if constexpr (MODE == 1) {
+#pragma unroll
+      for (int e = 0; e < 8; ++e) vd[e] = *reinterpret_cast<g1_t>(rp + (unsigned)sl.off[e] * 4u);
+    }
+    if constexpr (MODE == 2) {
 #pragma unroll
       for (int e = 0; e < 8; ++e) v[e] = *reinterpret_cast<g1_t>(rp + (unsigned)sl.off[e] * 4u);
     }
@@ -194,6 +227,13 @@
   auto slow_mask = [&](const Slow& sl, float (&v)[8]) {
 #pragma unroll
     for (int e = 0; e < 8; ++e) v[e] = (sl.ok >> e) & 1u ? v[e] : 0.f;
+  };
+  auto mixed_pick = [&](const Slow& sl, float (&v)[8], const float (&vd)[8]) {
+#pragma unroll
+    for (int e = 0; e < 8; ++e) {
+      const float a = v[e], b = vd[e];
+      v[e] = sl.vec ? a : ((sl.ok >> e) & 1u ? b : 0.f);
+    }
   };
   auto activate = [&](auto act_tag, float (&v)[8]) {
     if constexpr (decltype(act_tag)::value) {
@@ -211,35 +251,44 @@
       for (int r = 0; r < 16; ++r) acc[ct][i][r] = 0.f;
 
   auto run = [&](auto fast_tag, auto act_tag) {
-    constexpr bool FAST = decltype(fast_tag)::value;
+    constexpr int MODE = decltype(fast_tag)::value;
+    constexpr bool FAST = MODE == 0;
     float v[KC][CT][8];
+    float vd[MODE == 1 ? KC : 1][CT][8];
     Slow sl[CT];
     if constexpr (!FAST) {
 #pragma unroll
-      for (int ct = 0; ct < CT; ++ct) slow_init(ct, sl[ct]);
+      for (int ct = 0; ct < CT; ++ct) {
+        slow_init(ct, sl[ct]);
+        if constexpr (MODE == 1) mixed_init(ct, sl[ct]);
+      }
     }
     auto pieces = [&](int j, u32x4 (&out)[CT][NP]) {
 #pragma unroll
       for (int ct = 0; ct < CT; ++ct) {
-        if constexpr (!FAST) slow_mask(sl[ct], v[j][ct]);
+        if constexpr (MODE == 1) mixed_pick(sl[ct], v[j][ct], vd[j][ct]);
+        if constexpr (MODE == 2) slow_mask(sl[ct], v[j][ct]);
         activate(act_tag, v[j][ct]);
         gc_split<NP>(v[j][ct], out[ct]);
       }
     };
-    load_w(0);
+    const int k0 = ch0 * KC;
+    u32x4 wl[2][RT][NP];
+    if constexpr (KS) { load_wk(k0, wl[0]); load_wk(k0 + 1, wl[1]); }
+    else load_w(0);
 #pragma unroll
     for (int ksl = 0; ksl < KC; ++ksl)
 #pragma unroll
-      for (int ct = 0; ct < CT; ++ct) gather(fast_tag, ksl, ct, sl[ct], v[ksl][ct]);
-    store_w(0);
+      for (int ct = 0; ct < CT; ++ct) gather(fast_tag, k0 + ksl, ct, sl[ct], v[ksl][ct], vd[MODE == 1 ? ksl : 0][ct]);
+    if constexpr (!KS) store_w(0);
     u32x4 bq[CT][NP];
     pieces(0, bq);
 #pragma unroll
-    for (int ct = 0; ct < CT; ++ct) gather(fast_tag, KC, ct, sl[ct], v[0][ct]);
-    __syncthreads();
+    for (int ct = 0; ct < CT; ++ct) gather(fast_tag, k0 + KC, ct, sl[ct], v[0][ct], vd[0][ct]);
+    if constexpr (!KS) __syncthreads();
     auto chunk = [&](int ch, auto more_tag) {
       constexpr bool MORE = decltype(more_tag)::value;
-      if constexpr (MORE) load_w(ch + 1);
+      if constexpr (MORE && !KS) load_w(ch + 1);
       const u32x4* wb = Ws + (ch & 1) * SLOT + lane;
 #pragma unroll
       for (int ksl = 0; ksl < KC; ++ksl) {
@@ -250,12 +299,13 @@
 #pragma unroll
         for (int q = 0; q < NP; ++q)
 #pragma unroll
-          for (int i = 0; i < RT; ++i) aq[q][i] = wb[i * RTU + (ksl * NP + q) * 64];
+          for (int i = 0; i < RT; ++i) aq[q][i] = KS ? wl[ksl & 1][i][q] : wb[i * RTU + (ksl * NP + q) * 64];
+        if constexpr (KS) load_wk(ch * KC + ksl + 2, wl[ksl & 1]);
         u32x4 bqn[CT][NP];
         if (has_next) pieces(nx, bqn);
         if constexpr (MORE) {
 #pragma unroll
-          for (int ct = 0; ct < CT; ++ct) gather(fast_tag, ch * KC + ksl + 1 + KC, ct, sl[ct], v[nx][ct]);
+          for (int ct = 0; ct < CT; ++ct) gather(fast_tag, ch * KC + ksl + 1 + KC, ct, sl[ct], v[nx][ct], vd[MODE == 1 ? nx : 0][ct]);
         }
 #pragma unroll
         for (int lvl = NP - 1; lvl >= 0; --lvl)
@@ -278,7 +328,7 @@
             for (int q = 0; q < NP; ++q) bq[ct][q] = bqn[ct][q];
         }
         if (!(EBEN_GC_DBG & 16)) {
-          __builtin_amdgcn_sched_group_barrier(0x100, NP * RT, 0);
+          if (!KS) __builtin_amdgcn_sched_group_barrier(0x100, NP * RT, 0);
           __builtin_amdgcn_sched_group_barrier(0x002, VPM, 0);
 #pragma unroll
           for (int m = 0; m < 6 * RT * CT; ++m) {
@@ -288,23 +338,39 @@
         }
         __builtin_amdgcn_sched_barrier(0);
       }
-      if constexpr (MORE) {
+      if constexpr (MORE && !KS) {
         store_w(ch + 1);
         __syncthreads();
       }
     };
-    for (int ch = 0; ch + 1 < nch; ++ch) chunk(ch, std::true_type{});
-    chunk(nch - 1, std::false_type{});
+    for (int ch = ch0; ch + 1 < ch1; ++ch) chunk(ch, std::true_type{});
+    chunk(ch1 - 1, std::false_type{});
   };
   bool allfast = true;
 #pragma unroll
   for (int ct = 0; ct < CT; ++ct) allfast = allfast && fast[ct];
+  constexpr bool MIXED = CT == 1 && KC <= 4;
+  bool mixed = MIXED;
+  if constexpr (MIXED) {
+    const int u = ucol[0];
+    const int p0 = FORM == 2 ? u - 1 + h : P.S * u + P.off0 + (FORM == 0 && P.rpc_shift ? 8 * hk : 0);
+    const int span = FORM == 0 ? 8 : FORM == 1 ? 4 : 2;
+    mixed = __ballot(p0 >= 0 && p0 + span <= P.LX) != 0ull;
+  }
+  typedef std::integral_constant<int, 0> fast_t;
+  typedef std::integral_constant<int, 1> mixed_t;
+  typedef std::integral_constant<int, 2> slow_t;
   if (allfast) {
-    if (act_in) run(std::true_type{}, std::true_type{});
-    else run(std::true_type{}, std::false_type{});
+    if (act_in) run(fast_t{}, std::true_type{});
+    else run(fast_t{}, std::false_type{});
+  } else if (MIXED && mixed) {
+    if constexpr (MIXED) {
+      if (act_in) run(mixed_t{}, std::true_type{});
+      else run(mixed_t{}, std::false_type{});
+    }
   } else {
-    if (act_in) run(std::false_type{}, std::true_type{});
-    else run(std::false_type{}, std::false_type{});
+    if (act_in) run(slow_t{}, std::true_type{});
+    else run(slow_t{}, std::false_type{});
   }
 
   if (EBEN_GC_DBG & 8) {
@@ -318,6 +384,28 @@
     if (s == 1.2345f) P.y[0] = s;
     return;
   }
+  f32x4 ksum[CT][RT];
+  if constexpr (KS) {
+#pragma unroll
+    for (int ct = 0; ct < CT; ++ct)
+#pragma unroll
+      for (int i = 0; i < RT; ++i)
+#pragma unroll
+        for (int r4 = 0; r4 < 4; ++r4) {
+          const f32x4 t = {acc[ct][i][4 * r4], acc[ct][i][4 * r4 + 1], acc[ct][i][4 * r4 + 2], acc[ct][i][4 * r4 + 3]};
+          Ws[((wave * NT + ct * RT + i) * 4 + r4) * 64 + lane] = __builtin_bit_cast(u32x4, t);
+        }
+    __syncthreads();
+#pragma unroll
+    for (int ct = 0; ct < CT; ++ct)
+#pragma unroll
+      for (int i = 0; i < RT; ++i) {
+        f32x4 t = __builtin_bit_cast(f32x4, Ws[((ct * RT + i) * 4 + wave) * 64 + lane]);
+#pragma unroll
+        for (int part = 1; part < GC_KSPLIT; ++part) t += __builtin_bit_cast(f32x4, Ws[((part * NT + ct * RT + i) * 4 + wave) * 64 + lane]);
+        ksum[ct][i] = t;
+      }
+  }
   float* yb = P.y + (long long)b * P.CY * P.LY;
   const float* rb = P.res ? P.res + (long long)b * P.CY * P.LY : nullptr;
 #pragma unroll
@@ -328,11 +416,12 @@
     for (int i = 0; i < RT; ++i) {
       const int mt = (rg * RT + i) * 32;
 #pragma unroll
-      for (int r4 = 0; r4 < 4; ++r4) {
+      for (int r4i = 0; r4i < (KS ? 1 : 4); ++r4i) {
+        const int r4 = KS ? wave : r4i;
         const int m = mt + 8 * r4 + 4 * hk;
         float o[4];
 #pragma unroll
-        for (int r = 0; r < 4; ++r) o[r] = acc[ct][i][4 * r4 + r];
+        for (int r = 0; r < 4; ++r) o[r] = KS ? ksum[ct][i][r] : acc[ct][i][4 * r4i + r];
         if (FORM != 2) {
 #pragma unroll
           for (int r = 0; r < 4; ++r) {
@@ -375,6 +464,16 @@
       }
     }
   }
+}
+
+template <int FORM, int RT, int CT, int NP>
+__global__ __launch_bounds__(256, 2) void gc_kernel(const GcArgs P) {
+  gc_body<FORM, RT, CT, NP, false>(P);
+}
+
+template <int RT, int NP>
+__global__ __launch_bounds__(256, 2) void gc_ksplit_kernel(const GcArgs P) {
+  gc_body<0, RT, 1, NP, true>(P);
 }
 
 struct GcPackArgs {
@@ -438,6 +537,7 @@
   int ok, form, np;
   int CX, LX, CY, LY, NU, S, k, pad, rpc_shift, nkg, KSP, rows, nrt, nh;
   int RT, CT, nrg, ncb;
+  int ks;
 };
 
 static void gc_plan(const Canon& c, int dir, GcPlan* p) {
@@ -485,8 +585,23 @@
     }
   }
   if (!p->RT) return;
+  p->ks = 1;
+  static const int ksplit = gc_env("EBEN_GC_KSPLIT", 1);
+  const long long waves0 = 4ll * p->nh * (p->nrt / p->RT) * c.B * ceil_div(p->NU, 128 * p->CT);
+  if (ksplit && p->form == 0 && waves0 < 1024 && p->KSP >= 16 * GC_KSPLIT) {
+    int srt = 0;
+    double sbest = best;
+    for (int rt : {2, 1}) {
+      if (p->nrt % rt || (env_rt && rt != env_rt && p->nrt % env_rt == 0)) continue;
+      const long long waves = (long long)GC_KSPLIT * (p->nrt / rt) * c.B * ceil_div(p->NU, 32);
+      const double per_wave = (double)p->KSP / GC_KSPLIT * (32.0 * prod * rt > 240.0 ? 32.0 * prod * rt : 240.0) + 2500.0 + 600.0 * rt + 1500.0;
+      const double t = (double)((waves + 1023) / 1024) * per_wave;
+      if (t < sbest * 0.98) { sbest = t; srt = rt; }
+    }
+    if (srt) { p->RT = srt; p->CT = 1; p->ks = GC_KSPLIT; }
+  }
   p->nrg = p->nrt / p->RT;
-  p->ncb = ceil_div(p->NU, 128 * p->CT);
+  p->ncb = ceil_div(p->NU, (p->ks > 1 ? 32 : 128) * p->CT);
   p->ok = 1;
 }
 
@@ -494,6 +609,14 @@
   GcPlan p;
   gc_plan(c, dir, &p);
   return p.ok;
+}
+
+int gc_plan_info(const Canon& c, int dir, int* out) {
+  GcPlan p;
+  gc_plan(c, dir, &p);
+  if (!p.ok) return fail(EBEN_EUNSUPPORTED, "gc_plan_info on a layer the direct-operand conv does not cover");
+  out[0] = p.form; out[1] = p.RT; out[2] = p.CT; out[3] = p.np; out[4] = p.ks; out[5] = p.nh * p.nrg * c.B * p.ncb;
+  return EBEN_OK;
 }
 
 size_t gc_packed_floats(const Canon& c, int dir) {
@@ -518,6 +641,13 @@
 
 template <int FORM, int NP>
 static void gc_launch_shape(const GcPlan& p, const GcArgs& a, unsigned grid, hipStream_t st) {
+  if constexpr (FORM == 0) {
+    if (p.ks > 1) {
+      if (p.RT == 2) hipLaunchKernelGGL((gc_ksplit_kernel<2, NP>), dim3(grid), dim3(256), 0, st, a);
+      else hipLaunchKernelGGL((gc_ksplit_kernel<1, NP>), dim3(grid), dim3(256), 0, st, a);
+      return;
+    }
+  }
   if (p.RT == 2 && p.CT == 2) hipLaunchKernelGGL((gc_kernel<FORM, 2, 2, NP>), dim3(grid), dim3(256), 0, st, a);
   else if (p.RT == 2) hipLaunchKernelGGL((gc_kernel<FORM, 2, 1, NP>), dim3(grid), dim3(256), 0, st, a);
   else hipLaunchKernelGGL((gc_kernel<FORM, 1, 1, NP>), dim3(grid), dim3(256), 0, st, a);
diff --git a/vibravox_amd/csrc/ru_split.hip b/vibravox_amd/csrc/ru_split.hip
--- a/vibravox_amd/csrc/ru_split.hip
+++ b/vibravox_amd/csrc/ru_split.hip
@@ -58,12 +58,13 @@
 struct Ru3Args {
   const float* x; const u32x4* wimg; float* y; float* h; float* u;
   u32x4* xb; u32x4* hb; unsigned char* um;
+  const float* post;
   int B, L, d, ntt, vec;
   float in_slope, out_slope;
 };
 
-template <int CT, int NW, int NP, int KSC, bool BL = false>
-__global__ __launch_bounds__(NW * 64, (NW == 4 && CT < 4) ? 2 : 1) void ru3_fwd_kernel(const Ru3Args P) {
+template <int CT, int NW, int NP, int KSC, bool BL, bool POST>
+__device__ __forceinline__ void ru3_fwd_body(const Ru3Args& P) {
   constexpr int NT = NW * 64, BN = NW * 32, C = 32 * CT;
   constexpr int XS = BN + 2 * RS_DMAX + 6;
   constexpr int KB = C / 16;
@@ -211,6 +212,17 @@
       }
   }
 
+  float pv[POST ? CT * 16 : 1];
+  if constexpr (POST) {
+    if (live) {
+      const float* __restrict__ pb = P.post + lbase;
+#pragma unroll
+      for (int i = 0; i < CT; ++i)
+#pragma unroll
+        for (int r = 0; r < 16; ++r) pv[i * 16 + r] = pb[(unsigned)(i * 32 + (r & 3) + 8 * (r >> 2) + 4 * (lane >> 5)) * (unsigned)L];
+    }
+  }
+
 #pragma unroll
   for (int c2 = 0; c2 < NCH2; ++c2) {
     const int ch = NCH1 + c2;
@@ -274,8 +286,20 @@
       const unsigned off = m * (unsigned)L;
       const float uu = lrelu(acc2[i][r], P.out_slope);
       if (keep_u) ub[off] = uu;
-      if (!(EBEN_RU_DBG & 1) || uu == 12345.f) yb[off] = xc[m * XS] + uu;
-    }
+      float yv = xc[m * XS] + uu;
+      if constexpr (POST) yv += pv[i * 16 + r];
+      if (!(EBEN_RU_DBG & 1) || uu == 12345.f) yb[off] = yv;
+    }
+}
+
+template <int CT, int NW, int NP, int KSC, bool BL = false>
+__global__ __launch_bounds__(NW * 64, (NW == 4 && CT < 4) ? 2 : 1) void ru3_fwd_kernel(const Ru3Args P) {
+  ru3_fwd_body<CT, NW, NP, KSC, BL, false>(P);
+}
+
+template <int CT, int NW, int NP, int KSC, bool BL = false>
+__global__ __launch_bounds__(NW * 64, (NW == 4 && CT < 4) ? 2 : 1) void ru3_fwd_post_kernel(const Ru3Args P) {
+  ru3_fwd_body<CT, NW, NP, KSC, BL, true>(P);
 }
 
 __device__ __forceinline__ void ru3_pack_fwd_body(const float* __restrict__ vd, const float* __restrict__ sd, const float* __restrict__ vp,
@@ -614,10 +638,19 @@
 
 template <int CT, int NW, int NP, int KSC, bool BL = false>
 static int launch_ru3_fwd(const Ru3Args& a, hipStream_t st) {
+  constexpr int XS = NW * 32 + 2 * RS_DMAX + 6;
+  const size_t lds = (size_t)2 * KSC * NP * CT * 64 * 16 + sizeof(float) * 32 * CT * XS;
+  if (a.post) {
+    static LdsAttrOnce attr_once;
+    auto kern = ru3_fwd_post_kernel<CT, NW, NP, KSC, BL>;
+    const hipError_t e = lds_attr_once(attr_once, reinterpret_cast<const void*>(kern));
+    if (e != hipSuccess) return hip_fail(e, "hipFuncSetAttribute(ru3_fwd_post)");
+    hipLaunchKernelGGL(kern, dim3(a.B * a.ntt), dim3(NW * 64), lds, st, a);
+    EBEN_CHECK_LAUNCH("ru3_fwd_post_kernel");
+    return EBEN_OK;
+  }
   static LdsAttrOnce attr_once;
   auto kern = ru3_fwd_kernel<CT, NW, NP, KSC, BL>;
-  constexpr int XS = NW * 32 + 2 * RS_DMAX + 6;
-  const size_t lds = (size_t)2 * KSC * NP * CT * 64 * 16 + sizeof(float) * 32 * CT * XS;
   {
     const hipError_t e = lds_attr_once(attr_once, reinterpret_cast<const void*>(kern));
     if (e != hipSuccess) return hip_fail(e, "hipFuncSetAttribute(ru3_fwd)");
@@ -669,10 +702,10 @@
 }
 
 int ru3_fwd(int math, int batch, int channels, int length, int dilation, const float* x, float in_slope, float out_slope, const float* wimg,
-            float* y, float* h, float* u, hipStream_t st) {
+            const float* post, float* y, float* h, float* u, hipStream_t st) {
   Ru3Args a;
   a.x = x; a.wimg = reinterpret_cast<const u32x4*>(wimg); a.y = y; a.h = h; a.u = u;
-  a.xb = nullptr; a.hb = nullptr; a.um = nullptr;
+  a.xb = nullptr; a.hb = nullptr; a.um = nullptr; a.post = post;
   a.B = batch; a.L = length; a.d = dilation;
   const int bn = rs_waves(channels) * 32;
   a.ntt = ceil_div(length, bn);
@@ -695,9 +728,9 @@
 }
 
 int ru3_fwd_bl(int math, int batch, int channels, int length, int dilation, const float* x, float in_slope, float out_slope, const float* wimg,
-               float* y, void* xb, void* hb, void* um, hipStream_t st) {
+               const float* post, float* y, void* xb, void* hb, void* um, hipStream_t st) {
   Ru3Args a;
-  a.x = x; a.wimg = reinterpret_cast<const u32x4*>(wimg); a.y = y; a.h = nullptr; a.u = nullptr;
+  a.x = x; a.wimg = reinterpret_cast<const u32x4*>(wimg); a.y = y; a.h = nullptr; a.u = nullptr; a.post = post;
   a.xb = static_cast<u32x4*>(xb); a.hb = static_cast<u32x4*>(hb); a.um = static_cast<unsigned char*>(um);
   a.B = batch; a.L = length; a.d = dilation;
   a.ntt = ceil_div(length, 128);
@@ -808,7 +841,16 @@
                RS_DMAX, channels, dilation);
   EBEN_REQUIRE(batch > 0 && length > 0 && dilation < length, "bad ResidualUnit geometry");
   EBEN_REQUIRE(x && wimg && y, "null pointer in ru_fwd_ex");
-  return ru3_fwd(math, batch, channels, length, dilation, x, in_slope, out_slope, wimg, y, h, u, as_stream(stream));
+  return ru3_fwd(math, batch, channels, length, dilation, x, in_slope, out_slope, wimg, nullptr, y, h, u, as_stream(stream));
+}
+
+extern "C" int eben_ru_fwd_post(int math, int batch, int channels, int length, int dilation, const float* x, float in_slope, float out_slope,
+                                const float* wimg, const float* post, float* y, float* h, float* u, void* stream) {
+  EBEN_REQUIRE(math != EBEN_MATH_F32 && ru3_supported(channels, dilation, math),
+               "fused ResidualUnit with an output addend (split bf16 only): 32 / 64 / 128 channels, dilation 1..%d (got %d, %d)", RS_DMAX, channels, dilation);
+  EBEN_REQUIRE(batch > 0 && length > 0 && dilation < length, "bad ResidualUnit geometry");
+  EBEN_REQUIRE(x && wimg && post && y, "null pointer in ru_fwd_post");
+  return ru3_fwd(math, batch, channels, length, dilation, x, in_slope, out_slope, wimg, post, y, h, u, as_stream(stream));
 }
 
 extern "C" int eben_ru_bwd_ex(int math, int batch, int channels, int length, int dilation, const float* gy, const float* u, float out_slope,
@@ -828,5 +870,14 @@
                RS_DMAX, channels, dilation);
   EBEN_REQUIRE(batch > 0 && length > 0 && dilation < length, "bad ResidualUnit geometry");
   EBEN_REQUIRE(x && wimg && y && xb && hb && umask, "null pointer in rubl_fwd");
-  return ru3_fwd_bl(math, batch, channels, length, dilation, x, in_slope, out_slope, wimg, y, xb, hb, umask, as_stream(stream));
-}
+  return ru3_fwd_bl(math, batch, channels, length, dilation, x, in_slope, out_slope, wimg, nullptr, y, xb, hb, umask, as_stream(stream));
+}
+
+extern "C" int eben_rubl_fwd_post(int math, int batch, int channels, int length, int dilation, const float* x, float in_slope, float out_slope,
+                                  const float* wimg, const float* post, float* y, void* xb, void* hb, void* umask, void* stream) {
+  EBEN_REQUIRE(ru3_supported(channels, dilation, math), "fused ResidualUnit (split bf16): 32 / 64 / 128 channels, dilation 1..%d (got %d, %d)",
+               RS_DMAX, channels, dilation);
+  EBEN_REQUIRE(batch > 0 && length > 0 && dilation < length, "bad ResidualUnit geometry");
+  EBEN_REQUIRE(x && wimg && post && y && xb && hb && umask, "null pointer in rubl_fwd_post");
+  return ru3_fwd_bl(math, batch, channels, length, dilation, x, in_slope, out_slope, wimg, post, y, xb, hb, umask, as_stream(stream));
+}
diff --git a/vibravox_amd/csrc/tapconv.hip b/vibravox_amd/csrc/tapconv.hip
--- a/vibravox_amd/csrc/tapconv.hip
+++ b/vibravox_amd/csrc/tapconv.hip
@@ -609,6 +609,14 @@
   if (const int e = tap3_plan_variant(c, dir, k, &v)) return e;
   out[1] = v.FM; out[2] = v.XRB; out[3] = v.IM; out[4] = v.NPW; out[5] = v.NPX; out[6] = v.BL; out[7] = v.kernel;
   return EBEN_OK;
+}
+
+extern "C" int eben_gc_plan_info(const EbenConv1dDesc* d, int which, int* out, int n) {
+  EBEN_REQUIRE(out && n >= 6 && which == 0, "eben_gc_plan_info: which 0 (forward launches) and 6 output slots");
+  Canon c;
+  const int rc = canon_from_desc(d, &c);
+  if (rc) return rc;
+  return gc_plan_info(c, d->transposed ? 1 : 0, out);
 }
 
 extern "C" int eben_conv1d_pack(const EbenConv1dDesc* d, const float* v, const float* scale, float* wp_fwd, float* wp_bwd, void* stream) {
diff --git a/vibravox_amd/gen_engine.py b/vibravox_amd/gen_engine.py
--- a/vibravox_amd/gen_engine.py
+++ b/vibravox_amd/gen_engine.py
@@ -15,6 +15,7 @@
 USE_FUSED_RU_BWD = os.environ.get("EBEN_RU_FUSED_BWD", "1") != "0"
 USE_FUSED_RU_DW = os.environ.get("EBEN_RU_FUSED_DW", "1") != "0"
 USE_RU_BL = os.environ.get("EBEN_RU_BL", "1") != "0"
+USE_RU_POST = os.environ.get("EBEN_RU_POST", "1") != "0"
 DEFER_MARK_READY = os.environ.get("EBEN_G_DEFER_READY", "1") != "0"
 USE_GRAPHS = os.environ.get("EBEN_GEN_GRAPHS", "1") != "0"
 BWD_GROUPS = os.environ.get("EBEN_GEN_BWD_GROUPS", "1,1,1,1,1,1,1")
@@ -198,7 +199,7 @@
             self._core_units = [ru for blk in list(self.gen.encoder_blocks) + list(self.gen.decoder_blocks) for ru in blk.residuals]
         return self._core_units
 
-    def _residual_unit(self, ru, x, in_slope, train, recs):
+    def _residual_unit(self, ru, x, in_slope, train, recs, post=None):
         lib = load()
         b, c, l = x.shape
         dil, pwc = ru.dilated_conv, ru.pointwise_conv
@@ -215,8 +216,12 @@
             xb = torch.empty((b, c // 8, l, 8), dtype=torch.bfloat16, device=x.device)
             hb = torch.empty_like(xb)
             um = torch.empty((b, c // 8, l), dtype=torch.uint8, device=x.device)
-            check(lib.eben_rubl_fwd(fwd_math, b, c, l, dil.spec.dilation, ptr(x), float(in_slope), float(pwc.spec.out_slope), ptr(img), ptr(y),
-                                    xb.data_ptr(), hb.data_ptr(), um.data_ptr(), stream()), "rubl_fwd")
+            if post is None:
+                check(lib.eben_rubl_fwd(fwd_math, b, c, l, dil.spec.dilation, ptr(x), float(in_slope), float(pwc.spec.out_slope), ptr(img), ptr(y),
+                                        xb.data_ptr(), hb.data_ptr(), um.data_ptr(), stream()), "rubl_fwd")
+            else:
+                check(lib.eben_rubl_fwd_post(fwd_math, b, c, l, dil.spec.dilation, ptr(x), float(in_slope), float(pwc.spec.out_slope), ptr(img),
+                                             ptr(post), ptr(y), xb.data_ptr(), hb.data_ptr(), um.data_ptr(), stream()), "rubl_fwd_post")
             recs.append((("bl", self._ru_image(ru, 1), xb, hb, um), _ConvRec(dil, spec_d, dd_bwd, x if in_slope != 1.0 else None, None, pw_d.wp_bwd, pw_d.norm),
                          _ConvRec(pwc, pwc.spec, dp_bwd, None, None, pw_p.wp_bwd, pw_p.norm)))
             return y
@@ -225,8 +230,13 @@
             y = torch.empty_like(x)
             h = torch.empty_like(x) if train else None
             u = torch.empty_like(x) if train else None
-            check(lib.eben_ru_fwd_ex(fwd_math, b, c, l, dil.spec.dilation, ptr(x), float(in_slope), float(pwc.spec.out_slope), ptr(img), ptr(y),
-                                     ptr(h), ptr(u), stream()), "ru_fwd")
+            if post is not None and fwd_math != ops.MATH_F32:
+                check(lib.eben_ru_fwd_post(fwd_math, b, c, l, dil.spec.dilation, ptr(x), float(in_slope), float(pwc.spec.out_slope), ptr(img),
+                                           ptr(post), ptr(y), ptr(h), ptr(u), stream()), "ru_fwd_post")
+                post = None
+            else:
+                check(lib.eben_ru_fwd_ex(fwd_math, b, c, l, dil.spec.dilation, ptr(x), float(in_slope), float(pwc.spec.out_slope), ptr(img), ptr(y),
+                                         ptr(h), ptr(u), stream()), "ru_fwd")
         else:
             xin = x
             if in_slope != 1.0:
@@ -236,6 +246,10 @@
             u = self._conv(pwc, h, train)
             y = torch.empty_like(x)
             check(lib.eben_add(ptr(xin), ptr(u), ptr(y), x.numel(), stream()), "add")
+        if post is not None:
+            ysum = torch.empty_like(y)
+            check(lib.eben_add(ptr(y), ptr(post), ptr(ysum), y.numel(), stream()), "add")
+            y = ysum
         if train:
             bm = self._ru_bwd_math()
             fused = USE_FUSED_RU_BWD and dil.spec.ksize == 3 and dil.spec.reflect and lib.eben_ru_supported(c, dil.spec.dilation, bm) == 1
@@ -266,13 +280,20 @@
         cur = self._conv(gen.latent_conv[3], l1, train, recs=lat)
         if train:
             saved["latent"] = lat
-        for blk, skip in zip(gen.decoder_blocks, reversed(skips)):
+        rskips = skips[::-1]
+        added = False
+        for i, blk in enumerate(gen.decoder_blocks):
             recs = [] if train else None
-            s = torch.empty_like(cur)
-            check(lib.eben_add(ptr(cur), ptr(skip), ptr(s), cur.numel(), stream()), "add")
+            s = cur
+            if not added:
+                s = torch.empty_like(cur)
+                check(lib.eben_add(ptr(cur), ptr(rskips[i]), ptr(s), cur.numel(), stream()), "add")
             cur = self._conv(blk.conv_trans, s, train, recs=recs)
-            for ru in blk.residuals:
-                cur = self._residual_unit(ru, cur, 1.0, train, recs)
+            added = False
+            for k, ru in enumerate(blk.residuals):
+                post = rskips[i + 1] if USE_RU_POST and k == len(blk.residuals) - 1 and i + 1 < len(rskips) else None
+                cur = self._residual_unit(ru, cur, 1.0, train, recs, post=post)
+                added = post is not None
             if train:
                 saved["dec"].append(recs)
         return cur, first_bands, saved
```

New measurement: 7554 (median of 6 runs). No clear change (+0.6%).
